# ChicyChen/LOCO-Edit

Measured on AMD Instinct MI355X. Metric: edit-directions/sec (top-5 PMP-Jacobian SVD @256^2) + vT cos-sim vs ref, higher is better.
Workload: dtype bf16x3 (split-bf16 MFMA operands, fp32 accumulate + fp32 storage); 1 GPU; CelebA-HQ DDPM 256x256 top-5 local basis (l_eye-sized mask, L=2400), t=0.6T, 12 power iterations, one GPU; multi_gpu_form=single, probes_total=5, probes_per_gpu=5, kept=5, n_iter=12, mask_L=2400, weights=synthetic seed 0, streams=2

## Files before the change

### include/loco_hip_diag.h

```cpp
#ifndef LOCO_HIP_DIAG_H
#define LOCO_HIP_DIAG_H
#include "loco_hip.h"
#ifdef __cplusplus
extern "C" {
#endif

int  loco_bench_conv(loco_ctx* ctx, int32_t cin, int32_t cout, int32_t H, int32_t W, int32_t B, int32_t mode,
                     int32_t taps, int32_t tile, int32_t iters, float* ms_avg, void* stream);

typedef struct loco_conv_desc {
    int32_t struct_size;
    int32_t Cin, Cout, Hin, Win, B, taps;
    int32_t stride, upsample, zins, mode, cpg;
    int32_t transposed, accumulate, in_arena, pad;
    int32_t Cin2, cot_cpg;
    float   res_scale;
    int32_t reserved;
    const float *weight, *bias;
    const float *in, *bias2, *res;
    const float *prim, *sc, *sh, *mr, *gamma, *tst, *tc;
    const float *in2, *w2, *bias2nd;
    const float *cot_d, *cot_prim, *cot_sc, *cot_sh, *cot_mr, *cot_tc;
    float* out;
} loco_conv_desc;
int  loco_debug_conv(loco_ctx* ctx, const loco_conv_desc* desc, char* plan, int64_t cap, void* stream);

int64_t loco_debug_tensor(loco_ctx* ctx, const char* name, float* dst, int64_t cap, void* stream);

#ifdef __cplusplus
}
#endif
#endif
```

### loco-edit_amd/csrc/conv_bf16.hip

```cpp
#include "kernels.h"
#include <cstdio>
#include <cstdlib>

namespace loco {

enum : int { PR_BF16X3 = 0, PR_F16 = 1 };
template <int PR, int TAPS, int MODE> void launch_tile_b(const ConvArgs& a, hipStream_t st);
template <int PR, int MODE> void launch_kcat_b(const ConvArgs& a, hipStream_t st);
template <int PR, int MODE> void launch_pair_b(const ConvArgs& a, hipStream_t st);
void launch_conv_gemm(const ConvArgs& a, hipStream_t st);

template <int PR>
static void launch_lowp(const ConvArgs& a, int taps, hipStream_t st) {
#ifdef LOCO_DIAG
    if (a.cot_d && (taps != 1 || a.gemm || a.nsplit > 1 || a.Cin2 > 0 || (a.Cout % conv_bf16_tile_couts(a)) != 0 || a.st_kind == ST_TAN || a.st_kind == ST_COT)) {
        fprintf(stderr, "loco: ConvArgs::cot_d on a launch whose epilogue has no norm-cotangent term (taps %d, gemm %d, nsplit %d, Cout %d, st_kind %d)\n",
                taps, a.gemm, a.nsplit, a.Cout, a.st_kind);
        abort();
    }
#endif
    if constexpr (PR == PR_BF16X3) {
        if (taps == 1 && a.gemm) { launch_conv_gemm(a, st); return; }
    }
    if (taps == 9 && a.Cin2 > 0) {
        if (a.mode == CM_GN_SILU) launch_kcat_b<PR, CM_GN_SILU>(a, st);
        else if (a.mode == CM_GN_GELU) launch_kcat_b<PR, CM_GN_GELU>(a, st);
        else launch_kcat_b<PR, CM_TAN_SILU>(a, st);
        return;
    }
    if constexpr (PR == PR_BF16X3) {
        if (taps == 9 && a.pair) {
            switch (a.mode) {
                case CM_NONE: launch_pair_b<PR, CM_NONE>(a, st); break;
                case CM_GN_SILU: launch_pair_b<PR, CM_GN_SILU>(a, st); break;
                case CM_TAN_SILU: launch_pair_b<PR, CM_TAN_SILU>(a, st); break;
                default: launch_pair_b<PR, CM_COT_SILU>(a, st); break;
            }
            return;
        }
    }
    if (taps == 9) {
        switch (a.mode) {
            case CM_NONE: launch_tile_b<PR, 9, CM_NONE>(a, st); break;
            case CM_GN_SILU: launch_tile_b<PR, 9, CM_GN_SILU>(a, st); break;
            case CM_GN_GELU: launch_tile_b<PR, 9, CM_GN_GELU>(a, st); break;
            case CM_TAN_SILU: launch_tile_b<PR, 9, CM_TAN_SILU>(a, st); break;
            case CM_COT_SILU: launch_tile_b<PR, 9, CM_COT_SILU>(a, st); break;
            default: launch_tile_b<PR, 9, CM_GN>(a, st); break;
        }
    } else {
        switch (a.mode) {
            case CM_NONE: launch_tile_b<PR, 1, CM_NONE>(a, st); break;
            default: launch_tile_b<PR, 1, CM_GN>(a, st); break;
        }
    }
}
void launch_conv_bf16x3(const ConvArgs& a, int taps, hipStream_t st) { launch_lowp<PR_BF16X3>(a, taps, st); }
void launch_conv_f16(const ConvArgs& a, int taps, hipStream_t st) { launch_lowp<PR_F16>(a, taps, st); }

}
```

### loco-edit_amd/csrc/conv_bf16_kernel.h

```cpp
#pragma once
#include "kernels.h"
#include <cstdlib>
#include <type_traits>

namespace loco {


typedef float f32x16 __attribute__((ext_vector_type(16)));
typedef float f32x4 __attribute__((ext_vector_type(4)));
typedef f32x4 f32x4_u __attribute__((aligned(4)));
typedef float f32x2 __attribute__((ext_vector_type(2)));
typedef f32x2 f32x2_u __attribute__((aligned(4)));
typedef __bf16 bf16x8 __attribute__((ext_vector_type(8)));
typedef _Float16 f16x8 __attribute__((ext_vector_type(8)));
typedef short s16x8 __attribute__((ext_vector_type(8)));

enum : int { PR_BF16X3 = 0, PR_F16 = 1 };

constexpr int BKC = 16;
constexpr bool LIVE_MASK = true;
constexpr bool EARLY_W = true;
constexpr int NDUMMY = 8;

__device__ __forceinline__ float sigmoidf2_(float y) { return __builtin_amdgcn_rcpf(1.0f + __expf(-y)); }
// ... 257 lines not shown
            const int gl = lane & (LW - 1);
            if (gl < (1 << STEPS)) {
                int base = 0;
#pragma unroll
                for (int sb = 0; sb < STEPS; ++sb) base += ((gl >> sb) & 1) * (NV >> (sb + 1));
                const int ntile = (a.Hout * a.Wout) / NT;
                float* const sp = a.st_part + (long)b * a.Cout * ntile * 2;
#pragma unroll
                for (int i = 0; i < LEFT; ++i) {
                    const int idx = base + i, hq = idx >> 1;
                    const int h = hq / NTASK, q = hq - h * NTASK;
                    const int row = (q * NTHR + tid) / NQ;
                    const int co = co0 + ((row >> 5) * TM + h) * 32 + (row & 31);
                    sp[((long)co * ntile + tile_id) * 2 + (idx & 1)] = av[i];
                }
            }
        }
    }
}
template <int WM, int WN, int TM, int TN>
__device__ __forceinline__ void conv_lowp_epilogue_direct(const ConvArgs& a, f32x16 (&acc)[TM][TN], const int co0, const int oy0,
                                                          const int ox0, const int TW, const int b, const int split) {
    const int lane = threadIdx.x & 63, wave = threadIdx.x >> 6;
    const int l31 = lane & 31, khalf = lane >> 5, wm = wave / WN, wn = wave % WN;
    const long out_plane = (long)a.Hout * a.Wout;
    const bool full_co = false;
#pragma unroll
    for (int j = 0; j < TN; ++j) {
        int p = (wn * TN + j) * 32 + l31;
        int ty = p / TW, tx = p - ty * TW;
        int oy = oy0 + ty, ox = ox0 + tx;
        const unsigned pix = (unsigned)(oy * a.Wout + ox);
#pragma unroll
        for (int i = 0; i < TM; ++i) {
            const int cob = co0 + (wm * TM + i) * 32 + 4 * khalf;
            if (a.nsplit > 1) {
                float* pb = a.partial + (((long)split * a.B + b) * a.Cout) * out_plane;
#pragma unroll
                for (int r = 0; r < 16; ++r) {
                    int co = cob + (r & 3) + 8 * (r >> 2);
                    if (full_co || co < a.Cout) pb[(long)co * out_plane + pix] = acc[i][j][r];
                }
            } else {
                float* ob = a.out + (long)b * a.out_bs;
                const float* rb = a.res ? a.res + (long)b * a.res_bs : nullptr;
                const float* b2 = a.bias2 ? a.bias2 + (long)b * a.bias2_bs : nullptr;
                if (rb || a.accumulate) {
                    float rv[16];
#pragma unroll
                    for (int r = 0; r < 16; ++r) {
                        int co = cob + (r & 3) + 8 * (r >> 2);
                        const bool ok = full_co || co < a.Cout;
                        const long off = (long)(ok ? co : a.Cout - 1) * out_plane + pix;
                        float t = 0.f;
                        if (rb) t = a.res_scale * rb[off];
                        if (a.accumulate) t += ob[off];
                        rv[r] = t;
                    }
#pragma unroll
                    for (int r = 0; r < 16; ++r) {
                        int co = cob + (r & 3) + 8 * (r >> 2);
                        if (!(full_co || co < a.Cout)) continue;
                        float v = acc[i][j][r] + rv[r];
                        if (a.bias) v += a.bias[co];
                        if (b2) v += b2[co];
                        __builtin_nontemporal_store(v, &ob[(long)co * out_plane + pix]);
                    }
                } else {
#pragma unroll
                    for (int r = 0; r < 16; ++r) {
                        int co = cob + (r & 3) + 8 * (r >> 2);
                        if (!(full_co || co < a.Cout)) continue;
                        float v = acc[i][j][r];
                        if (a.bias) v += a.bias[co];
                        if (b2) v += b2[co];
                        __builtin_nontemporal_store(v, &ob[(long)co * out_plane + pix]);
                    }
                }
            }
        }
    }
}

template <int PR, int TAPS, int WM, int WN, int TM, int TN, int MODE, int STG, int PHASE = 0>
__device__ __forceinline__ void conv_lowp_body(const ConvArgs& a, f32x16 (&acc)[TM][TN]) {
    constexpr int NTHR = WM * WN * 64;
    constexpr int HP = halo_pitch<PR>();
    constexpr int RB = rec_bytes<PR>();
    constexpr int NPC = RB / 16;
    constexpr int MT = WM * TM * 32;
    constexpr int NT = WN * TN * 32;
    constexpr int KS = (TAPS == 9) ? 3 : 1;
    constexpr int NTS = KS;
    constexpr int NROW = (TAPS == 9) ? 3 : 1;
    constexpr bool NEEDP = (MODE == CM_TAN_SILU || MODE == CM_COT_SILU);
    constexpr bool GEN = (STG == 1 || STG == 2);
    constexpr int NITEM = GEN ? (2 * max_halo(NT, TAPS, STG == 2) + NTHR - 1) / NTHR : 1;
    constexpr int WTOT = NTS * MT * NPC;
    constexpr int NWV = (WTOT + NTHR - 1) / NTHR;
    constexpr bool XPF = (TAPS == 9 && STG != 2);
    constexpr int NWB = XPF ? 3 : 2;
    constexpr bool DEEP1 = (TAPS == 1 && STG == 1 && !NEEDP);
    constexpr int DEEP_D = 4;

    extern __shared__ __attribute__((aligned(16))) unsigned char smem_b[];
#ifdef LOCO_DUAL_STAMP
#define LP_STAMP(i) do { if (threadIdx.x == 0 && PHASE == 0) reinterpret_cast<unsigned long long*>(a.partial)[blockIdx.x * 8 + (i)] = __builtin_amdgcn_s_memtime(); } while (0)
#else
#define LP_STAMP(i) do { } while (0)
#endif
    LP_STAMP(0);
    constexpr int WBYTES = NTS * MT * RB;
    unsigned char* const Wsb = smem_b;
    unsigned char* Hsb;
    unsigned char* Ws = smem_b;
    unsigned char* Hs = smem_b;

    const int tid = threadIdx.x;
    const int lane = tid & 63;
    const int wave = tid >> 6;
    const int l31 = lane & 31;
    const int khalf = lane >> 5;
    const int wm = wave / WN, wn = wave % WN;

    const int S = a.stride;
    const int TW = (TAPS == 1 && PHASE == 0 && a.stride == 1 && !a.upsample && !a.zins && (a.Wout & (a.Wout - 1)) == 0)
                       ? (a.Wout < NT ? a.Wout : NT) : (a.Wout < 32 ? a.Wout : 32);
    const int TH = NT / TW;
    const int tiles_x = a.Wout / TW;
    int tile_id, cot_id, zid;
    {
        const int ntile = (a.Hout * a.Wout) / NT, ncot = (a.Cout + MT - 1) / MT, Z = a.B * a.nsplit;
        const int NTC = ntile * ncot, L = blockIdx.x;
        int T = 0;
        if ((ntile & 7) == 0) {
            int q = L >> 3, q2, t8;
            idivmod_small(q, ncot, q2, cot_id);
            idivmod_small(q2, Z, t8, zid);
            tile_id = t8 * 8 + (L & 7);
        } else {
            if ((NTC & 7) == 0) { int q = L >> 3, t8; idivmod_small(q, Z, t8, zid); T = t8 * 8 + (L & 7); }
            else idivmod_small(L, Z, T, zid);
            idivmod_small(T, ntile, cot_id, tile_id);
        }
        tile_id = __builtin_amdgcn_readfirstlane(tile_id);
        cot_id = __builtin_amdgcn_readfirstlane(cot_id);
        zid = __builtin_amdgcn_readfirstlane(zid);
    }
    int ty0_, tx0_;
    idivmod_small(tile_id, tiles_x, ty0_, tx0_);
    const int oy0 = __builtin_amdgcn_readfirstlane(ty0_ * TH);
    const int ox0 = __builtin_amdgcn_readfirstlane(tx0_ * TW);
    const int co0 = cot_id * MT;
    int zb_, zs_;
    idivmod_small(zid, a.nsplit, zb_, zs_);
    const int b = __builtin_amdgcn_readfirstlane(zb_);
    const int split = __builtin_amdgcn_readfirstlane(zs_);

    if constexpr (XPF && PHASE != 2 && EARLY_W) {
        const int nchunks_ = (a.Cin + BKC - 1) / BKC;
        const int cps_ = __builtin_amdgcn_readfirstlane((nchunks_ + a.nsplit - 1) / a.nsplit);
        const int cbeg_ = split * cps_;
        const int cend_ = (cbeg_ + cps_ < nchunks_) ? cbeg_ + cps_ : nchunks_;
        if (cend_ > cbeg_) {
            typedef __attribute__((address_space(3))) unsigned char lds_u8_;
            typedef const __attribute__((address_space(1))) unsigned char glb_u8_;
            const int wpitch_ = (a.Cout + 31) & ~31;
            const unsigned char* wbase0 = reinterpret_cast<const unsigned char*>(a.wb) +
                                          (unsigned)(cbeg_ * TAPS) * ((unsigned)wpitch_ * (unsigned)RB);
#pragma unroll
            for (int st_ = 0; st_ < 2; ++st_)
#pragma unroll
                for (int i = 0; i < NWV; ++i) {
                    int e = tid + i * NTHR;
                    if (e >= WTOT) e = WTOT - 1;
                    const int tap = e / (MT * NPC), rem = e - tap * (MT * NPC);
                    int rec = co0 + rem / NPC;
                    if (rec >= wpitch_) rec = wpitch_ - 1;
                    const unsigned rel = (unsigned)(((st_ * NTS + tap) * wpitch_ + rec) * NPC + (rem % NPC)) * 16u;
                    const int e0 = wave * 64 + i * NTHR;
                    if ((WTOT % NTHR) == 0 || e0 < WTOT)
                        __builtin_amdgcn_global_load_lds((glb_u8_*)(wbase0 + rel), (lds_u8_*)(smem_b + st_ * WBYTES + e0 * 16), 16, 0, 0);
                }
        }
    }
    const int halo_w = (TW - 1) * S + KS;
    const int halo_h = (TH - 1) * S + KS;
    const int halo_sz = halo_h * halo_w;
    const int HBYTES = (halo_sz + NDUMMY) * HP;
    Hsb = smem_b + NWB * WBYTES;

    const int LH = (a.upsample || a.zins) ? a.Hin * 2 : a.Hin;
    const int LW = (a.upsample || a.zins) ? a.Win * 2 : a.Win;
    const long in_plane = (long)a.Hin * a.Win;

    int ipos[NITEM], ioct[NITEM];
    unsigned ivoff[NITEM];
    bool ival[NITEM];
#pragma unroll
    for (int i = 0; i < NITEM; ++i) {
        int it = tid + i * NTHR;
        int oct, pos;
        idivmod_small(it, halo_sz, oct, pos);
        int off = -1;
        if (it < 2 * halo_sz) {
            int hy, hx;
            idivmod_small(pos, halo_w, hy, hx);
            int Y = oy0 * S - a.pad + hy, X = ox0 * S - a.pad + hx;
            if (Y >= 0 && Y < LH && X >= 0 && X < LW) {
                if (a.upsample) off = (Y >> 1) * a.Win + (X >> 1);
                else if (a.zins) off = ((Y | X) & 1) ? -1 : (Y >> 1) * a.Win + (X >> 1);
                else off = Y * a.Win + X;
            }
        } else {
            pos = -1; oct = 0;
        }
        ipos[i] = pos; ioct[i] = oct;
        ival[i] = off >= 0;
        ivoff[i] = (unsigned)(oct * 8 * (int)in_plane + (off >= 0 ? off : 0));
    }

    const int nseg = (halo_w + 3) >> 2;
    int v_q4 = 0, v_pos0 = -1, v_voff = 0, v_cnt = 0;
    unsigned v_pm = 0;
    int v_rec[4] = {0, 0, 0, 0};
    unsigned v_goff = 0;
    if constexpr (!GEN) {
        const int per_q = halo_h * nseg;
        const int nsg4 = (nseg + 3) >> 2, nhy2 = (halo_h + 1) >> 1;
        bool have = false;
        int hy = 0, sg = 0;
        if (32 * nsg4 * nhy2 <= NTHR) {
            const int hi = tid >> 5;
            v_q4 = (tid >> 3) & 3;
            int hq_, hr_;
            idivmod_small(hi, nsg4, hq_, hr_);
            sg = hr_ * 4 + (tid & 3);
            hy = hq_ * 2 + ((tid >> 2) & 1);
            have = hi < nsg4 * nhy2 && sg < nseg && hy < halo_h;
            if (!have) v_q4 = 0;
        } else if (tid < 4 * per_q) {
            int rem;
            idivmod_small(tid, per_q, v_q4, rem);
            idivmod_small(rem, nseg, hy, sg);
            have = true;
        }
        if (have) {
            int Y = oy0 - a.pad + hy, X0 = ox0 - a.pad + 4 * sg;
            bool rowok = (Y >= 0 && Y < a.Hin);
            v_pos0 = hy * halo_w + 4 * sg;
            v_cnt = halo_w - 4 * sg < 4 ? halo_w - 4 * sg : 4;
            v_voff = rowok ? Y * a.Win + X0 : 0;
#pragma unroll
            for (int pxi = 0; pxi < 4; ++pxi)
                if (rowok && X0 + pxi >= 0 && X0 + pxi < a.Win && pxi < v_cnt) v_pm |= 1u << pxi;
        }
#pragma unroll
        for (int pxi = 0; pxi < 4; ++pxi)
            v_rec[pxi] = (v_pos0 >= 0 && pxi < v_cnt) ? v_pos0 + pxi : halo_sz + (tid & (NDUMMY - 1));
        v_goff = (unsigned)(((long)v_q4 * 4 * in_plane + v_voff + 16) * 4);
    }

    int hoff[TN];
#pragma unroll
    for (int j = 0; j < TN; ++j) {
        int p = (wn * TN + j) * 32 + l31;
        int ty, tx;
        idivmod_small(p, TW, ty, tx);
        hoff[j] = ty * S * halo_w + tx * S;
    }
    int hbyte[TN];
#pragma unroll
    for (int j = 0; j < TN; ++j) hbyte[j] = hrec_off<PR>(hoff[j], khalf);
    int aoff_hi[TM], aoff_lo[TM];
#pragma unroll
    for (int i = 0; i < TM; ++i) {
        int p = (wm * TM + i) * 32 + l31;
        aoff_hi[i] = rec_off<PR>(p, khalf);
        aoff_lo[i] = PR == PR_F16 ? 0 : rec_off<PR>(p, 2 + khalf);
    }

    if constexpr (PHASE != 2) {
#pragma unroll
        for (int i = 0; i < TM; ++i)
#pragma unroll
            for (int j = 0; j < TN; ++j)
#pragma unroll
                for (int r = 0; r < 16; ++r) acc[i][j][r] = 0.0f;
    }

    const int nchunks = (a.Cin + BKC - 1) / BKC;
    const int cps = __builtin_amdgcn_readfirstlane((nchunks + a.nsplit - 1) / a.nsplit);
    const int cbeg = split * cps;
    const int cend = (cbeg + cps < nchunks) ? cbeg + cps : nchunks;

    const float* inb = a.in + (long)b * a.in_bs;
    const float2* sxb = NEEDP ? a.sx : nullptr;
    const float* scb = (MODE == CM_GN_SILU || MODE == CM_GN || MODE == CM_GN_GELU) ? a.sc + (long)b * a.scsh_bs : nullptr;
    const float* shb = (MODE == CM_GN_SILU || MODE == CM_GN || MODE == CM_GN_GELU) ? a.sh + (long)b * a.scsh_bs : nullptr;
    const int wpitch = (a.Cout + 31) & ~31;
    const uint4* wg = reinterpret_cast<const uint4*>(a.wb);

    float hv[NITEM][8];
    float2 pv[NEEDP ? NITEM : 1][8];
    float cA[(MODE == CM_NONE) ? 1 : 16], cB[(MODE == CM_NONE) ? 1 : 16];
    const float* tcb = NEEDP ? a.tc + (long)b * a.tc_bs : nullptr;

    constexpr int NPART = (!GEN && NROW == 3) ? 2 : 1;
    constexpr int KP = 4 / NPART;
    struct HaloRegs {
        f32x4 dq[GEN ? 1 : KP];
        f32x4 sq[(!GEN && NEEDP) ? KP : 1][2];
        f32x4 cq[(!GEN && MODE != CM_NONE) ? (KP == 4 ? 2 : 1) : 1];
    };
    auto cq_a = [&](const HaloRegs& R, int kk) -> float {
        if constexpr (GEN || MODE == CM_NONE) return 0.f;
        else if constexpr (NEEDP) { if constexpr (KP == 4) return R.cq[kk >> 1][(kk & 1) * 2]; else return R.cq[0][kk * 2]; }
        else return R.cq[0][kk];
    };
    auto cq_b = [&](const HaloRegs& R, int kk) -> float {
        if constexpr (GEN || MODE == CM_NONE) return 0.f;
        else if constexpr (NEEDP) { if constexpr (KP == 4) return R.cq[kk >> 1][(kk & 1) * 2 + 1]; else return R.cq[0][kk * 2 + 1]; }
        else if constexpr (KP == 4) return R.cq[1][kk];
        else return R.cq[0][2 + kk];
    };
    HaloRegs hr;
    bool pf_live = true, dma_live = true;
#ifdef LOCO_DUAL_STAMP
    const bool wi_halo = (a.no_deep & 2) != 0, wi_dma = (a.no_deep & 4) != 0, wi_novalu = (a.no_deep & 8) != 0;
#endif
    auto prefetch_hv = [&](HaloRegs& R, int chunk, int part) {
        const unsigned cb = (unsigned)chunk * ((unsigned)(BKC * 4) * (unsigned)in_plane);
        const char* pk = reinterpret_cast<const char*>(inb - 16) + cb;
        const char* sk = reinterpret_cast<const char*>(reinterpret_cast<const float*>(sxb) - 32) + 2u * cb;
        const unsigned pl = (unsigned)in_plane * 4u;
#pragma unroll
        for (int kk = 0; kk < KP; ++kk) {
#ifdef LOCO_DUAL_STAMP
            const unsigned po = (pf_live && !wi_halo) ? v_goff + (unsigned)(part * KP + kk) * pl : 64u;
#else
            const unsigned po = pf_live ? v_goff + (unsigned)(part * KP + kk) * pl : 64u;
#endif
            R.dq[kk] = *reinterpret_cast<const f32x4_u*>(pk + po);
            if constexpr (NEEDP) {
                R.sq[kk][0] = *reinterpret_cast<const f32x4_u*>(sk + 2u * po);
                R.sq[kk][1] = *reinterpret_cast<const f32x4_u*>(sk + 2u * po + 16);
            }
        }
        const int c0 = chunk * BKC + v_q4 * 4 + part * KP;
        if constexpr (MODE != CM_NONE) {
            if constexpr (NEEDP) {
                R.cq[0] = *reinterpret_cast<const f32x4_u*>(tcb + 2 * c0);
                if constexpr (KP == 4) R.cq[1] = *reinterpret_cast<const f32x4_u*>(tcb + 2 * c0 + 4);
            } else if constexpr (KP == 4) {
                R.cq[0] = *reinterpret_cast<const f32x4_u*>(scb + c0);
                R.cq[1] = *reinterpret_cast<const f32x4_u*>(shb + c0);
            } else {
                const f32x2 sa = *reinterpret_cast<const f32x2_u*>(scb + c0), sb = *reinterpret_cast<const f32x2_u*>(shb + c0);
                R.cq[0] = f32x4{sa[0], sa[1], sb[0], sb[1]};
            }
        }
    };
    auto stage_hv = [&](const HaloRegs& R, int part) {
#ifdef LOCO_DUAL_STAMP
        if (wi_novalu) return;
#endif
        const int oct = v_q4 >> 1, half = v_q4 & 1;
#pragma unroll
        for (int pxi = 0; pxi < 4; ++pxi) {
            float r[KP];
#pragma unroll
            for (int kk = 0; kk < KP; ++kk) {
                float d = R.dq[kk][pxi];
                float v = d;
                if constexpr (MODE == CM_GN_SILU) {
                    float y = fmaf(cq_a(R, kk), d, cq_b(R, kk));
                    v = y * sigmoidf2_(y);
                } else if constexpr (MODE == CM_GN_GELU) {
                    v = act_fwd(fmaf(cq_a(R, kk), d, cq_b(R, kk)), ACT_GELU);
                } else if constexpr (MODE == CM_GN) {
                    v = fmaf(cq_a(R, kk), d, cq_b(R, kk));
                } else if constexpr (NEEDP) {
                    const float Sv = R.sq[kk][pxi >> 1][(pxi & 1) * 2], xh = R.sq[kk][pxi >> 1][(pxi & 1) * 2 + 1];
                    if constexpr (MODE == CM_TAN_SILU) v = Sv * fmaf(-xh, cq_b(R, kk), d - cq_a(R, kk));
                    else v = fmaf(-xh, cq_b(R, kk), fmaf(Sv, d, -cq_a(R, kk)));
                }
                r[kk] = ((v_pm >> pxi) & 1u) ? v : 0.0f;
            }
            unsigned char* dst = Hs + hrec_off<PR>(v_rec[pxi], oct) + half * 8 + part * (KP * 2);
            if constexpr (KP == 4) {
                uint2 h, l;
                cvt2<PR>(r[0], r[1], h.x, l.x);
                cvt2<PR>(r[2], r[3], h.y, l.y);
                *reinterpret_cast<uint2*>(dst) = h;
                if constexpr (PR == PR_BF16X3) *reinterpret_cast<uint2*>(dst + 32) = l;
            } else {
                unsigned h, l;
                cvt2<PR>(r[0], r[1], h, l);
                *reinterpret_cast<unsigned*>(dst) = h;
                if constexpr (PR == PR_BF16X3) *reinterpret_cast<unsigned*>(dst + 32) = l;
            }
        }
    };
    auto load_consts = [&](int chunk) {
        const int c0 = chunk * BKC;
        if constexpr (MODE != CM_NONE) {
#pragma unroll
            for (int kk = 0; kk < 16; ++kk) {
                int c = c0 + kk < a.Cin ? c0 + kk : a.Cin - 1;
                if constexpr (NEEDP) { cA[kk] = tcb[2 * c]; cB[kk] = tcb[2 * c + 1]; }
                else { cA[kk] = scb[c]; cB[kk] = shb[c]; }
            }
        }
    };
    auto load_regs = [&](float (&hvd)[NITEM][8], int chunk) {
        const int c0 = chunk * BKC;
        if (c0 + BKC <= a.Cin) {
            if constexpr (TAPS == 9 && !NEEDP) {
                const unsigned lm = pf_live ? 0xffffffffu : 0u;
                const long pb4 = in_plane * 4;
                const unsigned char* pk = reinterpret_cast<const unsigned char*>(inb) + (long)c0 * pb4;
#pragma unroll
                for (int k = 0; k < 8; ++k) {
#pragma unroll
                    for (int i = 0; i < NITEM; ++i) hvd[i][k] = *reinterpret_cast<const float*>(pk + ((ivoff[i] * 4u) & lm));
                    pk += pb4;
                }
            } else {
#pragma unroll
            for (int k = 0; k < 8; ++k) {
                const float* pk = inb + (long)(c0 + k) * in_plane;
                const float2* sk = NEEDP ? sxb + (long)(c0 + k) * in_plane : nullptr;
#pragma unroll
                for (int i = 0; i < NITEM; ++i) {
                    hvd[i][k] = pk[pf_live ? ivoff[i] : 0u];
                    if constexpr (NEEDP) pv[i][k] = sk[pf_live ? ivoff[i] : 0u];
                }
            }
            }
        } else {
#pragma unroll
            for (int i = 0; i < NITEM; ++i) {
#pragma unroll
                for (int k = 0; k < 8; ++k) {
                    int c = c0 + ioct[i] * 8 + k;
                    int cc = c < a.Cin ? c : a.Cin - 1;
                    unsigned vo = ivoff[i] - (unsigned)(ioct[i] * 8 * (int)in_plane);
                    float v = inb[(long)cc * in_plane + vo];
                    hvd[i][k] = c < a.Cin ? v : 0.0f;
                    if constexpr (NEEDP) {
                        float2 pp = sxb[(long)cc * in_plane + vo];
                        pv[i][k] = c < a.Cin ? pp : make_float2(0.f, 0.f);
                    }
                }
            }
        }
    };
    auto prefetch_h = [&](int chunk, int part) {
        if constexpr (!GEN) { prefetch_hv(hr, chunk, part); return; }
        load_consts(chunk);
        load_regs(hv, chunk);
    };
    unsigned wrel[NWV];
#pragma unroll
    for (int i = 0; i < NWV; ++i) {
        int e = tid + i * NTHR;
        if (e >= WTOT) e = WTOT - 1;
        int tap = e / (MT * NPC), rem = e - tap * (MT * NPC);
        int rec = co0 + rem / NPC;
        if (rec >= wpitch) rec = wpitch - 1;
        wrel[i] = (unsigned)((tap * wpitch + rec) * NPC + (rem % NPC)) * 16u;
    }
    typedef __attribute__((address_space(3))) unsigned char lds_u8;
    typedef const __attribute__((address_space(1))) unsigned char glb_u8;
    auto dma_w = [&](int chunk, int row, unsigned char* Wdst) {
        const unsigned char* wbase = reinterpret_cast<const unsigned char*>(wg) +
                                     (unsigned)(chunk * TAPS + row * NTS) * ((unsigned)wpitch * (unsigned)RB);
#pragma unroll
        for (int i = 0; i < NWV; ++i) {
            const int e0 = (wave * 64 + i * NTHR);
            if ((WTOT % NTHR) == 0 || e0 < WTOT)
#ifdef LOCO_DUAL_STAMP
                __builtin_amdgcn_global_load_lds((glb_u8*)(wbase + ((dma_live && !wi_dma) ? wrel[i] : 0u)), (lds_u8*)(Wdst + e0 * 16), 16, 0, 0);
#else
                __builtin_amdgcn_global_load_lds((glb_u8*)(wbase + (dma_live ? wrel[i] : 0u)), (lds_u8*)(Wdst + e0 * 16), 16, 0, 0);
#endif
        }
    };
    auto stage_regs = [&](const float (&hvs)[NITEM][8], int chunk, unsigned char* Hd, auto whole_tag) {
        constexpr bool WHOLE = decltype(whole_tag)::value;
        const int c0 = chunk * BKC;
#pragma unroll
        for (int i = 0; i < NITEM; ++i) {
            if (ipos[i] < 0) continue;
            float v[8];
#pragma unroll
            for (int k = 0; k < 8; ++k) {
                int c = c0 + ioct[i] * 8 + k;
                float r = 0.0f;
                if (ival[i] && (WHOLE || c < a.Cin)) {
                    float d = hvs[i][k];
                    if constexpr (MODE == CM_NONE) {
                        r = d;
                    } else {
                        const float ca = ioct[i] ? cA[8 + k] : cA[k];
                        const float cb = ioct[i] ? cB[8 + k] : cB[k];
                        if constexpr (MODE == CM_GN_SILU) {
                            float y = fmaf(ca, d, cb);
                            r = y * sigmoidf2_(y);
                        } else if constexpr (MODE == CM_GN_GELU) {
                            r = act_fwd(fmaf(ca, d, cb), ACT_GELU);
                        } else if constexpr (MODE == CM_GN) {
                            r = fmaf(ca, d, cb);
                        } else {
                            float Sv = pv[i][k].x, xh = pv[i][k].y;
                            if constexpr (MODE == CM_TAN_SILU) r = Sv * fmaf(-xh, cb, d - ca);
                            else r = fmaf(-xh, cb, fmaf(Sv, d, -ca));
                        }
                    }
                }
                v[k] = r;
            }
            uint4 hi, lo;
            split8<PR>(v, hi, lo);
            *reinterpret_cast<uint4*>(Hd + hrec_off<PR>(ipos[i], ioct[i])) = hi;
            if constexpr (PR == PR_BF16X3) *reinterpret_cast<uint4*>(Hd + hrec_off<PR>(ipos[i], 2 + ioct[i])) = lo;
        }
    };
    auto stage_h = [&](int chunk, int part) {
        if constexpr (!GEN) { stage_hv(hr, part); return; }
        stage_regs(hv, chunk, Hs, std::false_type{});
    };

    constexpr int NLO = PR == PR_BF16X3 ? 1 : 0;
    struct Frag { s16x8 ah[TM], al[NLO ? TM : 1], bh[TN], bl[NLO ? TN : 1]; };
    auto load_frag = [&](Frag& f, int row, int tp) {
        const int tapoff = (TAPS == 9) ? row * halo_w + tp : 0;
#pragma unroll
        for (int i = 0; i < TM; ++i) {
            f.ah[i] = *reinterpret_cast<const s16x8*>(Ws + tp * MT * RB + aoff_hi[i]);
#if defined(LOCO_WI_NOLO)
            if constexpr (NLO) f.al[i] = f.ah[i];
#else
            if constexpr (NLO) f.al[i] = *reinterpret_cast<const s16x8*>(Ws + tp * MT * RB + aoff_lo[i]);
#endif
        }
#pragma unroll
        for (int j = 0; j < TN; ++j) {
            const unsigned char* hp = Hs + tapoff * HP + hbyte[j];
            f.bh[j] = *reinterpret_cast<const s16x8*>(hp);
#if defined(LOCO_WI_NOLO)
            if constexpr (NLO) f.bl[j] = f.bh[j];
#else
            if constexpr (NLO) f.bl[j] = *reinterpret_cast<const s16x8*>(hp + 32);
#endif
        }
    };
    auto mma_frag = [&](const Frag& f) {
#pragma unroll
        for (int i = 0; i < TM; ++i)
#pragma unroll
            for (int j = 0; j < TN; ++j) {
                if constexpr (PR == PR_F16) {
                    acc[i][j] = __builtin_amdgcn_mfma_f32_32x32x16_f16(__builtin_bit_cast(f16x8, f.ah[i]),
                                                                       __builtin_bit_cast(f16x8, f.bh[j]), acc[i][j], 0, 0, 0);
                } else {
                    const bf16x8 ah = __builtin_bit_cast(bf16x8, f.ah[i]), al = __builtin_bit_cast(bf16x8, f.al[i]);
                    const bf16x8 bh = __builtin_bit_cast(bf16x8, f.bh[j]), bl = __builtin_bit_cast(bf16x8, f.bl[j]);
                    acc[i][j] = __builtin_amdgcn_mfma_f32_32x32x16_bf16(al, bh, acc[i][j], 0, 0, 0);
                    acc[i][j] = __builtin_amdgcn_mfma_f32_32x32x16_bf16(ah, bl, acc[i][j], 0, 0, 0);
                    acc[i][j] = __builtin_amdgcn_mfma_f32_32x32x16_bf16(ah, bh, acc[i][j], 0, 0, 0);
                }
            }
    };

    auto mma_one = [&](const Frag& f, int i, int j) {
        if constexpr (PR == PR_F16) {
            acc[i][j] = __builtin_amdgcn_mfma_f32_32x32x16_f16(__builtin_bit_cast(f16x8, f.ah[i]),
                                                               __builtin_bit_cast(f16x8, f.bh[j]), acc[i][j], 0, 0, 0);
        } else {
            const bf16x8 ah = __builtin_bit_cast(bf16x8, f.ah[i]), al = __builtin_bit_cast(bf16x8, f.al[i]);
            const bf16x8 bh = __builtin_bit_cast(bf16x8, f.bh[j]), bl = __builtin_bit_cast(bf16x8, f.bl[j]);
#if defined(LOCO_WI_MFMA16)
            {
                f32x4 q0 = {acc[i][j][0], acc[i][j][1], acc[i][j][2], acc[i][j][3]}, q1 = {acc[i][j][4], acc[i][j][5], acc[i][j][6], acc[i][j][7]};
                f32x4 q2 = {acc[i][j][8], acc[i][j][9], acc[i][j][10], acc[i][j][11]}, q3 = {acc[i][j][12], acc[i][j][13], acc[i][j][14], acc[i][j][15]};
                q0 = __builtin_amdgcn_mfma_f32_16x16x32_bf16(al, bh, q0, 0, 0, 0);
                q1 = __builtin_amdgcn_mfma_f32_16x16x32_bf16(al, bh, q1, 0, 0, 0);
                q2 = __builtin_amdgcn_mfma_f32_16x16x32_bf16(ah, bl, q2, 0, 0, 0);
                q3 = __builtin_amdgcn_mfma_f32_16x16x32_bf16(ah, bl, q3, 0, 0, 0);
                q0 = __builtin_amdgcn_mfma_f32_16x16x32_bf16(ah, bh, q0, 0, 0, 0);
                q1 = __builtin_amdgcn_mfma_f32_16x16x32_bf16(ah, bh, q1, 0, 0, 0);
#pragma unroll
                for (int r = 0; r < 4; ++r) { acc[i][j][r] = q0[r]; acc[i][j][4 + r] = q1[r]; acc[i][j][8 + r] = q2[r]; acc[i][j][12 + r] = q3[r]; }
                return;
            }
#elif defined(LOCO_WI_2MFMA)
            acc[i][j] = __builtin_amdgcn_mfma_f32_32x32x16_bf16(ah, bl, acc[i][j], 0, 0, 0);
            acc[i][j] = __builtin_amdgcn_mfma_f32_32x32x16_bf16(ah, bh, acc[i][j], 0, 0, 0);
            (void)al;
            return;
#endif
            acc[i][j] = __builtin_amdgcn_mfma_f32_32x32x16_bf16(al, bh, acc[i][j], 0, 0, 0);
            acc[i][j] = __builtin_amdgcn_mfma_f32_32x32x16_bf16(ah, bl, acc[i][j], 0, 0, 0);
            acc[i][j] = __builtin_amdgcn_mfma_f32_32x32x16_bf16(ah, bh, acc[i][j], 0, 0, 0);
        }
    };
    auto mma_frag_head = [&](const Frag& f) { mma_one(f, 0, 0); };
    auto mma_frag_tail = [&](const Frag& f) {
#pragma unroll
        for (int i = 0; i < TM; ++i)
#pragma unroll
            for (int j = 0; j < TN; ++j)
                if (i + j > 0) mma_one(f, i, j);
    };

    const int nch = cend - cbeg;
    const int clast = cend - 1;
    auto cclamp = [&](int c) { return __builtin_amdgcn_readfirstlane(c < clast ? c : clast); };
    auto vres = [&](int x) -> int {
// ... 120 lines not shown
            const bool live = LIVE_MASK ? (chunk_raw <= clast) : true;
            const int chunk = cclamp(chunk_raw);
            const int c0 = chunk * BKC;
            const unsigned lm = live ? 0xffffffffu : 0u;
            const unsigned char* pk = reinterpret_cast<const unsigned char*>(inb) + (long)c0 * plane_bytes;
#pragma unroll
            for (int k = 0; k < 8; ++k) {
#pragma unroll
                for (int i = 0; i < NITEM; ++i) hvr[sl][i][k] = *reinterpret_cast<const float*>(pk + (ivoffb[i] & lm));
                pk += plane_bytes;
            }
            const unsigned char* wbase = wgb + (unsigned)(chunk * TAPS) * ((unsigned)wpitch * (unsigned)RB);
#pragma unroll
            for (int i = 0; i < NWV; ++i) wr[sl][i] = *reinterpret_cast<const f32x4*>(wbase + (wrel[i] & lm));
        };
        auto commit = [&](auto stag, int chunk, unsigned char* Hd, unsigned char* Wd) {
            constexpr int sl = decltype(stag)::value;
            if constexpr (MODE != CM_NONE) load_consts(chunk);
            stage_regs(hvr[sl], chunk, Hd, std::true_type{});
#pragma unroll
            for (int i = 0; i < NWV; ++i)
                if ((WTOT % NTHR) == 0 || tid + i * NTHR < WTOT)
                    *reinterpret_cast<f32x4*>(Wd + (tid + i * NTHR) * 16) = wr[sl][i];
        };
        using S0 = std::integral_constant<int, 0>; using S1 = std::integral_constant<int, 1>;
        using S2 = std::integral_constant<int, 2>; using S3 = std::integral_constant<int, 3>;
        static_assert(D == 4, "ring slots are spelled out below");
        if (nch > 0) {
            issue(S0{}, cbeg);
            issue(S1{}, cbeg + 1);
            issue(S2{}, cbeg + 2);
            issue(S3{}, cbeg + 3);
            commit(S0{}, cbeg, Hsb, Wsb);
            issue(S0{}, cbeg + 4);
            stage_end();
        }
        auto body = [&](auto stag, const int ci) {
            const int chunk = cbeg + ci;
            unsigned char* const Wcur = Wsb + (ci & 1) * WBYTES;
            unsigned char* const Wnxt = Wsb + ((ci + 1) & 1) * WBYTES;
            unsigned char* const Hcur = Hsb + (ci & 1) * HBYTES;
            unsigned char* const Hnxt = Hsb + ((ci + 1) & 1) * HBYTES;
            Ws = Wcur; Hs = Hcur;
            Frag f0;
            load_frag(f0, 0, 0);
            __builtin_amdgcn_sched_barrier(0);
            mma_frag(f0);
            commit(stag, cclamp(chunk + 1), Hnxt, Wnxt);
            issue(stag, chunk + 1 + D);
            stage_end();
        };
        int ci = 0;
        for (; ci + D <= nch; ci += D) {
            body(S1{}, ci); body(S2{}, ci + 1); body(S3{}, ci + 2); body(S0{}, ci + 3);
        }
        if (ci < nch) body(S1{}, ci);
        if (ci + 1 < nch) body(S2{}, ci + 1);
        if (ci + 2 < nch) body(S3{}, ci + 2);
      }
    }
    if (!deep_done) {
    if (nch > 0) {
        dma_w(cbeg, 0, Wsb);
        Hs = Hsb;
        if constexpr (!GEN && NPART == 2) {
            HaloRegs hr2;
            prefetch_hv(hr, cbeg, 0);
            prefetch_hv(hr2, cbeg, 1);
            stage_hv(hr, 0);
            stage_hv(hr2, 1);
        } else {
#pragma unroll
            for (int part = 0; part < NPART; ++part) {
                prefetch_h(cbeg, part);
                stage_h(cbeg, part);
            }
        }
        asm volatile("s_waitcnt vmcnt(0)" ::: "memory");
        if (NROW == 1 || NPART == 2) prefetch_h(cclamp(cbeg + 1), 0);
        stage_end();
    }
    for (int ci = 0; ci < nch; ++ci) {
        const int chunk = cbeg + ci;
#pragma unroll
        for (int row = 0; row < NROW; ++row) {
            const int s_ = ci * NROW + row;
            unsigned char* const Wcur = Wsb + (s_ & 1) * WBYTES;
            unsigned char* const Wnxt = Wsb + ((s_ + 1) & 1) * WBYTES;
            unsigned char* const Hcur = Hsb + (ci & 1) * HBYTES;
            unsigned char* const Hnxt = Hsb + ((ci + 1) & 1) * HBYTES;
            constexpr bool one = (NROW == 1);
            const int st_part = one ? 0 : (NPART == 2 ? (row == 0 ? 0 : row == 1 ? 1 : -1) : (row == 2 ? 0 : -1));
            const int ld_part = one ? 0 : (NPART == 2 ? (row == 0 ? 1 : row == 1 ? 0 : -1) : (row == 0 ? 0 : -1));
            const int ld_chunk = one ? chunk + 2 : ((NPART == 2 && row == 1) ? chunk + 2 : chunk + 1);
            constexpr bool MIDLOAD = !GEN;
            constexpr int NLD = KP + (NEEDP ? 2 * KP + 1 : (MODE != CM_NONE ? 2 : 0));
            {
                const int r1 = (row + 1) % NROW, dc = (row + 1) / NROW;
                dma_live = LIVE_MASK ? (chunk + dc <= clast) : true;
                dma_w(cclamp(chunk + dc), r1, Wnxt);
                dma_live = true;
            }
            Ws = Wcur; Hs = Hcur;
            Frag f0, f1;
            load_frag(f0, row, 0);
            if (NTS > 1) load_frag(f1, row, 1);
            __builtin_amdgcn_sched_barrier(0);
            mma_frag(f0);
            __builtin_amdgcn_sched_barrier(0);
            if (NTS > 2) load_frag(f0, row, 2);
            __builtin_amdgcn_sched_barrier(0);
            if (NTS > 1) mma_frag(f1);
            if (st_part >= 0) { Hs = Hnxt; stage_h(cclamp(chunk + 1), st_part); Hs = Hcur; }
            if (MIDLOAD && ld_part >= 0) { pf_live = LIVE_MASK ? (ld_chunk <= clast) : true; prefetch_h(cclamp(ld_chunk), ld_part); pf_live = true; }
            if (NTS > 2) mma_frag(f0);
            __builtin_amdgcn_sched_barrier(0);
            if (MIDLOAD && ld_part >= 0) {
                asm volatile("s_waitcnt vmcnt(%0)" :: "n"(NLD) : "memory");
            } else {
                asm volatile("s_waitcnt vmcnt(0)" ::: "memory");
                if (!MIDLOAD && ld_part >= 0) { pf_live = LIVE_MASK ? (ld_chunk <= clast) : true; prefetch_h(cclamp(ld_chunk), ld_part); pf_live = true; }
            }
            stage_end();
        }
    }
    }

    }

    if constexpr (PHASE == 1) {
        asm volatile("s_waitcnt lgkmcnt(0)" ::: "memory");
        __builtin_amdgcn_s_barrier();
        return;
    }
    LP_STAMP(3);
    conv_lowp_epilogue<WM, WN, TM, TN, (TAPS == 1 && PHASE == 0) ? (EPI_COT1 | EPI_STATS) : EPI_STATS>(a, acc, smem_b, co0, oy0, ox0, TW, tile_id, b, split);
    LP_STAMP(4);
#undef LP_STAMP
}

constexpr int lowp_min_waves(int taps, int nthr) { return (taps == 1 && nthr <= 256) ? 2 : 1; }
template <int TAPS, int WM, int WN, int TM, int TN, int MODE, int STG>
__global__ __launch_bounds__(WM * WN * 64, lowp_min_waves(TAPS, WM * WN * 64)) void conv_mfma_bf16x3(ConvArgs a) {
    f32x16 acc[TM][TN];
    conv_lowp_body<PR_BF16X3, TAPS, WM, WN, TM, TN, MODE, STG>(a, acc);
}
template <int TAPS, int WM, int WN, int TM, int TN, int MODE, int STG>
__global__ __launch_bounds__(WM * WN * 64, lowp_min_waves(TAPS, WM * WN * 64)) void conv_mfma_f16(ConvArgs a) {
    f32x16 acc[TM][TN];
    conv_lowp_body<PR_F16, TAPS, WM, WN, TM, TN, MODE, STG>(a, acc);
}

template <int PR, int WM, int WN, int TM, int TN, int MODE>
__device__ __forceinline__ void conv_lowp_kcat(const ConvArgs& a) {
    f32x16 acc[TM][TN];
    conv_lowp_body<PR, 9, WM, WN, TM, TN, MODE, 0, 1>(a, acc);
    ConvArgs a2 = a;
    a2.in = a.in2; a2.in_bs = a.in2_bs; a2.Cin = a.Cin2; a2.wb = a.wb2; a2.mode = CM_NONE; a2.pad = 0; a2.in_padded = a.in2_padded;
    conv_lowp_body<PR, 1, WM, WN, TM, TN, CM_NONE, 1, 2>(a2, acc);
}
template <int WM, int WN, int TM, int TN, int MODE>
__global__ __launch_bounds__(WM * WN * 64) void conv_kcat_bf16x3(ConvArgs a) { conv_lowp_kcat<PR_BF16X3, WM, WN, TM, TN, MODE>(a); }
template <int WM, int WN, int TM, int TN, int MODE>
__global__ __launch_bounds__(WM * WN * 64) void conv_kcat_f16(ConvArgs a) { conv_lowp_kcat<PR_F16, WM, WN, TM, TN, MODE>(a); }

template <int PR, int TAPS, int WM, int WN, int TM, int TN, int MODE, int STG>
static void launch_one_b2(const ConvArgs& a, hipStream_t st) {
    constexpr int MT = WM * TM * 32, NT = WN * TN * 32;
    constexpr int KS = (TAPS == 9) ? 3 : 1;
    int TW = a.Wout < 32 ? a.Wout : 32;
    int TH = NT / TW;
    int halo_w = (TW - 1) * a.stride + KS, halo_h = (TH - 1) * a.stride + KS;
    const int nwb = (TAPS == 9 && STG != 2) ? 3 : 2;
    size_t lds = (size_t)nwb * KS * MT * rec_bytes<PR>() + 2 * ((size_t)halo_w * halo_h + NDUMMY) * halo_pitch<PR>();
    const size_t stage_bytes = (size_t)WM * 32 * NT * 4;
    if (lds < stage_bytes) lds = stage_bytes;
    dim3 grid(((a.Hout * a.Wout) / NT) * ((a.Cout + MT - 1) / MT) * a.B * a.nsplit);
    void (*kern)(ConvArgs);
    if constexpr (PR == PR_F16) kern = &conv_mfma_f16<TAPS, WM, WN, TM, TN, MODE, STG>;
    else kern = &conv_mfma_bf16x3<TAPS, WM, WN, TM, TN, MODE, STG>;
    if (lds > 64 * 1024) {
        static DeviceOnce once;
        if (first_on_device(once)) {
            (void)hipFuncSetAttribute(reinterpret_cast<const void*>(kern), hipFuncAttributeMaxDynamicSharedMemorySize,
                                      160 * 1024);
        }
    }
    hipLaunchKernelGGL(kern, grid, dim3(WM * WN * 64), lds, st, a);
}

template <int PR, int TAPS, int WM, int WN, int TM, int TN, int MODE>
static void launch_one_b(const ConvArgs& a, hipStream_t st) {
    const bool general = a.stride != 1 || a.upsample || a.zins || (a.Cin % BKC) != 0 || !a.in_padded;
    if constexpr (MODE == CM_NONE) {
        if (a.stride == 2) launch_one_b2<PR, TAPS, WM, WN, TM, TN, MODE, 2>(a, st);
        else if (TAPS == 9 && !general) launch_one_b2<PR, TAPS, WM, WN, TM, TN, MODE, 0>(a, st);
        else launch_one_b2<PR, TAPS, WM, WN, TM, TN, MODE, 1>(a, st);
        return;
    }
    if constexpr (MODE == CM_GN_SILU || MODE == CM_TAN_SILU || MODE == CM_GN_GELU) {
        if (general) { launch_one_b2<PR, TAPS, WM, WN, TM, TN, MODE, 1>(a, st); return; }
    }
    launch_one_b2<PR, TAPS, WM, WN, TM, TN, MODE, 0>(a, st);
}


template <int PR, int MODE>
void launch_kcat_b(const ConvArgs& a, hipStream_t st) {
    constexpr int WM = 2, WN = 4, TM = 2, TN = 2, MT = 128, NT = 256;
    const int TW = a.Wout < 32 ? a.Wout : 32, TH = NT / TW;
    size_t lds = (size_t)3 * 3 * MT * rec_bytes<PR>() + 2 * ((size_t)(TW + 2) * (TH + 2) + NDUMMY) * halo_pitch<PR>();
    dim3 grid(((a.Hout * a.Wout) / NT) * ((a.Cout + MT - 1) / MT) * a.B * a.nsplit);
    void (*kern)(ConvArgs);
    if constexpr (PR == PR_F16) kern = &conv_kcat_f16<WM, WN, TM, TN, MODE>;
    else kern = &conv_kcat_bf16x3<WM, WN, TM, TN, MODE>;
    static DeviceOnce once;
    if (first_on_device(once))
        (void)hipFuncSetAttribute(reinterpret_cast<const void*>(kern), hipFuncAttributeMaxDynamicSharedMemorySize, 160 * 1024);
    hipLaunchKernelGGL(kern, grid, dim3(WM * WN * 64), lds, st, a);
}

template <int PR, int TAPS, int MODE>
void launch_tile_b(const ConvArgs& a, hipStream_t st) {
    switch (a.tile) {
        case 5:
            launch_one_b<PR, TAPS, 2, 4, 2, 2, MODE>(a, st);
            break;
        case 0: launch_one_b<PR, TAPS, 2, 2, 2, 2, MODE>(a, st); break;
        case 1: launch_one_b<PR, TAPS, 4, 1, 1, 2, MODE>(a, st); break;
        case 2: launch_one_b<PR, TAPS, 1, 4, 1, 1, MODE>(a, st); break;
        default: launch_one_b<PR, TAPS, 2, 2, 1, 1, MODE>(a, st); break;
    }
}


}
```

### loco-edit_amd/csrc/conv_plan.hip

```cpp
#include "kernels.h"
#include <cstdio>
#include <cstdlib>

namespace loco {

constexpr int BKC = 16;
constexpr int BKF = 8;

static const int kMT[6] = {128, 128, 32, 64, 128, 128}, kNT[6] = {128, 64, 128, 64, 256, 256};

static int env_int(const char* name, int dflt) {
    const char* e = getenv(name);
    return e ? atoi(e) : dflt;
}
static int pick_tile(int Cout, int HW) {
    if (HW >= 128) return Cout > 32 ? 0 : 2;
    return Cout > 64 ? 1 : 3;
}

static int conv_pick_nsplit(int Cin, int Cout, int Hout, int Wout, int B) {
    const int t = pick_tile(Cout, Hout * Wout);
    long blocks = (long)((Hout * Wout) / kNT[t]) * ((Cout + kMT[t] - 1) / kMT[t]) * B;
    int nchunks = (Cin + BKF - 1) / BKF;
    if (blocks >= 384 || nchunks < 8) return 1;
    int want = (int)((512 + blocks - 1) / blocks);
    int maxs = nchunks / 4;
    if (want > maxs) want = maxs;
    if (want > 32) want = 32;
    return want < 1 ? 1 : want;
}

static int conv_bf16_pick_tile(int Cout, int HW, int B, int tile_override) {
    if (B <= 1 && HW <= 1024 && HW >= 64 && (Cout % 64) == 0) return 3;
    int t = pick_tile(Cout, HW);
    if (t == 0 && HW >= 256) {
        if (tile_override >= 0) return tile_override;
        return 5;
    }
    return t;
}

constexpr int kTile0MaxHW = 65536;

static int bf16_tile_of(const ConvArgs& a, int tile_override = -1) {
    int tile = conv_bf16_pick_tile(a.Cout, a.Hout * a.Wout, a.B, tile_override);
    if (tile == 4) tile = 5;
    if (tile == 5 && a.taps == 1 && !a.gemm && a.B >= 2 && a.Hout * a.Wout <= kTile0MaxHW) return 0;
    if (a.stride == 2 && tile == 5) tile = 0;
    return tile;
}
static int tile_for(const ConvArgs& a, int prec, int tile_override) {
    return prec ? bf16_tile_of(a, tile_override) : pick_tile(a.Cout, a.Hout * a.Wout);
}
static int conv_bf16_tile_pixels(const ConvArgs& a) { return a.gemm ? 256 : kNT[a.tile]; }
int conv_bf16_tile_couts(const ConvArgs& a) { return a.gemm ? 64 * a.gemm_tm : kMT[a.tile]; }

static int conv_bf16_pick_nsplit(int Cin, int Cout, int Hout, int Wout, int B, int chip_share, int taps, int lanes) {
    const int HW = Hout * Wout;
    int t = conv_bf16_pick_tile(Cout, HW, B, -1);
    if (t == 4) t = 5;
    if (taps == 1 && t == 5 && B >= 2 && HW <= kTile0MaxHW) t = 0;
    long blocks = (long)(HW / kNT[t]) * ((Cout + kMT[t] - 1) / kMT[t]) * B;
    int nchunks = (Cin + BKC - 1) / BKC;
    int target = chip_share > 1 ? 256 / chip_share : (lanes == 2 ? 240 : 256);
    if (target < 32) target = 32;
    if (blocks >= target / 2 || nchunks < 8) return 1;
    int want = (int)(target / blocks);
    int maxs = nchunks / 4;
    if (want > maxs) want = maxs;
    if (want > 32) want = 32;
    return want < 1 ? 1 : want;
}

static bool conv_lowp_can_kcat(const ConvArgs& a) {
    static const bool on = env_int("LOCO_KCAT", 1) != 0;
    return on && a.Cin2 > 0 && a.nsplit == 1 && bf16_tile_of(a) == 5 && a.stride == 1 && !a.upsample && !a.zins && a.pad == 1 &&
           (a.Cin % BKC) == 0 && (a.Cin2 % BKC) == 0 && a.in_padded &&
           (a.mode == CM_GN_SILU || a.mode == CM_GN_GELU || a.mode == CM_TAN_SILU);
}
static bool conv_lowp_can_fuse_stats(const ConvArgs& a) {
    return a.nsplit <= 1 && !a.gemm && (a.Cout % conv_bf16_tile_couts(a)) == 0;
}

static bool conv_pair_ok(const ConvArgs& a) {
    static const bool on = env_int("LOCO_CONV_PAIR", 1) != 0;
    if (!on || a.Hout * a.Wout < 16384 || a.taps != 9 || a.Cin2 > 0 || a.nsplit != 1 || a.stride != 1 || a.upsample || a.zins ||
        a.pad != 1 || !a.in_padded || (a.Cin % (2 * BKC)) != 0 || (a.Cout % 128) != 0 || (a.Wout % 32) != 0 || (a.Hout % 8) != 0)
        return false;
    if (!(a.mode == CM_NONE || a.mode == CM_GN_SILU || a.mode == CM_TAN_SILU || a.mode == CM_COT_SILU)) return false;
    return a.tile == 5;
}

static ConvArgs conv_shift_batch(const ConvArgs& a, int nb) {
    ConvArgs t = a;
    t.B = a.B - nb;
    t.in += (long)nb * a.in_bs; t.out += (long)nb * a.out_bs;
    if (t.prim) t.prim += (long)nb * a.prim_bs;
    if (t.bias2) t.bias2 += (long)nb * a.bias2_bs;
    if (t.res) t.res += (long)nb * a.res_bs;
    if (t.sc) { t.sc += (long)nb * a.scsh_bs; t.sh += (long)nb * a.scsh_bs; }
    if (t.mr) t.mr += (long)nb * a.mr_bs;
    if (t.tst) t.tst += (long)nb * a.tst_bs;
    if (t.tc) t.tc += (long)nb * a.tc_bs;
    if (t.in2) t.in2 += (long)nb * a.in2_bs;
    if (t.cot_d) { t.cot_d += (long)nb * a.cot_d_bs; t.cot_tc += (long)nb * a.cot_tc_bs; }
    if (t.st_part) t.st_part += (long)nb * a.Cout * ((a.Hout * a.Wout) / conv_bf16_tile_pixels(a)) * 2;
    return t;
}

static void conv_gemm_plan(ConvArgs& a) {
    static const bool on = env_int("LOCO_CONV_GEMM", 1) != 0;
    a.gemm = 0;
    const long HW = (long)a.Hout * a.Wout;
    if (!on || a.stride != 1 || a.upsample || a.zins || (a.Cin % BKC) != 0 || a.Cin < 320 || (HW % 256) != 0 || (a.Wout % 16) != 0 ||
        a.Cout < 128 || !a.partial || a.Cin2 > 0 || !(a.mode == CM_NONE || a.mode == CM_GN) || a.cot_d)
        return;
    {
        const int TW = a.Wout < 32 ? a.Wout : 32;
        if ((256 % TW) != 0 || (a.Wout % TW) != 0 || (a.Hout % (256 / TW)) != 0) return;
    }
    static const int all_shapes = env_int("LOCO_GEMM_ALL", 0);
    if (!all_shapes && !(a.Cout >= 640 && (a.Cout >= 4 * a.Cin || a.Cin >= 2560))) return;
    const int pad256 = (a.Cout + 255) / 256 * 256;
    const int tm = (pad256 * 10 <= a.Cout * 11) ? 4 : 2;
    const int mt = 64 * tm;
    const long tiles = (HW / 256) * ((a.Cout + mt - 1) / mt) * a.B;
    const size_t rec_floats = (size_t)a.B * a.Cin * HW;
    int ns = 1;
    if (tiles < 192) {
        const int nchunks = a.Cin / BKC;
        ns = (int)((256 + tiles - 1) / tiles);
        if (ns > 8) ns = 8;
        while (ns > 1 && nchunks / ns < 8) --ns;
        while (ns > 1 && (size_t)ns * a.B * a.Cout * HW + rec_floats > a.partial_floats) --ns;
    }
    if ((ns > 1 ? (size_t)ns * a.B * a.Cout * HW : 0) + rec_floats > a.partial_floats) return;
    a.gemm = 1; a.gemm_tm = tm; a.nsplit = ns;
}

void conv_plan_family(ConvArgs& a, int prec) {
    if (prec == 1 && a.taps == 1) conv_gemm_plan(a);
}

void conv_plan_tile_pair(ConvArgs& a, int prec, int tile_override) {
    a.tile = tile_for(a, prec, tile_override);
    a.pair = prec == 1 && conv_pair_ok(a);
}

static bool short_tail(long per_probe, int B) {
    const long total = per_probe * B, r = total % 256;
    return total > 256 && r > 0 && r <= 160;
}

static int tail_split(const ConvArgs& a, size_t partial_floats, int* split) {
    const long per_probe = (long)((a.Hout * a.Wout) / conv_bf16_tile_pixels(a)) * ((a.Cout + 127) / 128);
    const long r = per_probe * a.B % 256;
    if (!short_tail(per_probe, a.B) || per_probe <= 0 || r % per_probe != 0 || r / per_probe >= a.B) return 0;
    int s = (int)(256 / r);
    if (s > 4) s = 4;
    const int nchunks = (a.Cin + 15) / 16;
    while (s > 1 && nchunks / s < 4) --s;
    const size_t one = (size_t)(r / per_probe) * a.Cout * a.Hout * a.Wout;
    while (s > 1 && (size_t)s * one > partial_floats) --s;
    *split = s;
    return s > 1 ? (int)(r / per_probe) : 0;
}

static int stats_route(const ConvEnv& e, const StatAsk* q, bool want, ConvArgs& x, int s0, int B, int* keep_ntile) {
    if (!q || q->kind == ST_NONE) return SR_NONE;
    const int alone = q->norm ? SR_ALONE : SR_NONE;
    if (!want) return alone;
    if (x.nsplit > 1) return !q->norm ? SR_NONE : ((x.Hout * x.Wout) % 4 == 0 ? SR_SPLITK : SR_ALONE);
    const int ntile = (x.Hout * x.Wout) / conv_bf16_tile_pixels(x);
    const size_t need = (size_t)x.B * x.Cout * ntile * 2;
    const int epi = q->norm ? SR_EPI : SR_KEEP;
    const bool kept = q->keep && s0 == 0 && x.B == B && need <= q->keep_floats;
    if (q->kind == ST_FWD && conv_lowp_can_fuse_stats(x) && (kept || (q->norm && need <= e.stpart_floats))) {
        x.st_part = kept ? q->keep : e.stpart; x.st_kind = ST_FWD;
        if (kept) *keep_ntile = ntile;
        return epi;
    }
    const bool cot_cache = q->kind == ST_COT && q->norm && q->sx;
    if ((q->kind == ST_TAN || cot_cache) && e.fuse_lin && !x.cot_d && conv_lowp_can_fuse_stats(x)) {
        const size_t lane_off = (size_t)e.lane_s0 * (q->keep_floats / e.max_batch);
        const bool keptl = q->kind == ST_TAN && q->keep && s0 == 0 && x.B == B && lane_off + need <= q->keep_floats;
        if (keptl || (q->norm && need <= e.stpart_floats)) {
            x.st_part = keptl ? q->keep + lane_off : e.stpart; x.st_kind = q->kind; x.st_x = q->prim;
            if (q->kind == ST_COT) x.st_sx = q->sx;
            if (keptl) *keep_ntile = ntile;
            return epi;
        }
    }
    return alone;
}

static ConvLaunch plan_launch(const ConvEnv& e, const StatAsk* q, bool want, const ConvArgs& x, int s0, int B, int* keep_ntile) {
    ConvLaunch l;
    l.args = x;
    l.s0 = s0;
    l.args.tile = tile_for(x, e.prec, -1);
    l.stats = stats_route(e, q, want, l.args, s0, B, keep_ntile);
    if (l.stats == SR_EPI || l.stats == SR_KEEP) l.ntile = (x.Hout * x.Wout) / conv_bf16_tile_pixels(l.args);
    conv_plan_tile_pair(l.args, e.prec, -1);
    return l;
}

ConvPlan plan_conv(const ConvEnv& e, const ConvArgs& a0, int taps, const StatAsk* q, const ConvArgs* sc) {
    ConvPlan p;
    ConvArgs a = a0;
    a.taps = taps;
    a.gemm = 0;
    if (sc) {
        ConvArgs t = a;
        t.nsplit = e.prec >= 1 ? conv_bf16_pick_nsplit(a.Cin, a.Cout, a.Hout, a.Wout, a.B, e.chip_share, 9, e.lanes) : 2;
        t.in2 = sc->in; t.in2_bs = sc->in_bs; t.Cin2 = sc->Cin;
        const long per_probe = (long)((a.Hout * a.Wout) / 256) * ((a.Cout + 127) / 128);
        if (e.prec >= 1 && taps == 9 && !short_tail(per_probe, a.B) && !a.bias2 && conv_lowp_can_kcat(t)) {
            a.in2 = sc->in; a.in2_bs = sc->in_bs; a.Cin2 = sc->Cin; a.in2_padded = sc->in_padded;
            a.wb2 = e.prec == 2 ? sc->wh : sc->wb;
            a.bias2 = sc->bias; a.bias2_bs = 0;
            a.res = nullptr;
        } else {
            p.sc_first = true;
            a.res = sc->out; a.res_bs = sc->out_bs;
        }
    }
    if (e.prec == 2) a.wb = a.wh;
    a.no_deep = e.deep1 ? 0 : 1;
    a.nsplit = e.prec >= 1 ? conv_bf16_pick_nsplit(a.Cin, a.Cout, a.Hout, a.Wout, a.B, e.chip_share, taps, e.lanes)
                           : conv_pick_nsplit(a.Cin, a.Cout, a.Hout, a.Wout, a.B);
    if (a.cot_d) {
        ConvArgs t = a;
        t.tile = bf16_tile_of(t);
        const long per_probe = (long)((a.Hout * a.Wout) / conv_bf16_tile_pixels(t)) * ((a.Cout + 127) / 128);
        p.cot = e.prec >= 1 && taps == 1 && a.nsplit == 1 && !short_tail(per_probe, a.B) && conv_lowp_can_fuse_stats(t);
        if (!p.cot) { a.cot_d = nullptr; a.cot_d_bs = 0; a.cot_sx = nullptr; a.cot_tc = nullptr; a.cot_tc_bs = 0; }
    }
    while (a.nsplit > 1 && (size_t)a.nsplit * a.B * a.Cout * a.Hout * a.Wout > e.partial_floats) a.nsplit >>= 1;
    if (a.nsplit < 1) a.nsplit = 1;
    a.partial = e.partial;
    a.partial_floats = e.partial_floats;
    conv_plan_family(a, e.prec);
    a.tile = tile_for(a, e.prec, -1);
    int split = 1;
    const int tail = e.prec >= 1 && a.nsplit == 1 && a.B >= 2 && !a.gemm ? tail_split(a, e.partial_floats, &split) : 0;
    const bool want = q && q->kind != ST_NONE && e.prec >= 1 && e.fuse_stats;
    if (!tail) {
        p.l[0] = plan_launch(e, q, want, a, 0, a.B, &p.keep_ntile);
        return p;
    }
    const bool per_part = want && q->norm && (q->kind == ST_FWD || (e.fuse_lin && (a.Hout * a.Wout) % 4 == 0));
    p.stats_all = !per_part && q && q->kind != ST_NONE && q->norm;
    const StatAsk* ql = per_part ? q : nullptr;
    const int nb = a.B - tail;
    ConvArgs m = a, t = conv_shift_batch(a, nb);
    m.B = nb;
    t.nsplit = split;
    p.nl = 2;
    p.l[0] = plan_launch(e, ql, want, m, 0, a.B, &p.keep_ntile);
    p.l[1] = plan_launch(e, ql, want, t, nb, a.B, &p.keep_ntile);
    return p;
}

const char* conv_variant_name(const ConvArgs& a, int taps, int prec) {
    static const char* tiles[6] = {"2,2,2,2", "4,1,1,2", "1,4,1,1", "2,2,1,1", "2,2,2,4", "2,4,2,2"};
    static char names[3][2][6][6][56];
    static char others[3][3][6][40];
    const int mode = (a.mode < 0 || a.mode > 5) ? 2 : a.mode;
    const char* other = nullptr;
    int k = 0, v = mode;
    if (prec && taps == 9 && a.Cin2 > 0) other = prec == 1 ? "conv_kcat_bf16x3<2,4,2,2,%d>" : "conv_kcat_f16<2,4,2,2,%d>";
    else if (prec == 1 && taps == 1 && a.gemm) { k = 1; other = "conv_gemm_bf16x3<%d>"; v = a.gemm_tm; }
    else if (prec == 1 && taps == 9 && a.pair) { k = 2; other = "conv_pair_bf16x3<%d>"; }
    if (other) {
        char* n = others[k][prec][v];
        if (!n[0]) snprintf(n, 40, other, v);
        return n;
    }
    int t = a.tile;
    if (t < 0 || t > 5) t = 0;
    int m = mode;
    if (taps != 9 && m != CM_NONE) m = CM_GN;
    if (!prec && m == CM_GN_GELU) m = CM_GN_SILU;
    char* n = names[prec][taps == 9 ? 0 : 1][t][m];
    static const char* kn[3] = {"conv_mfma_f32", "conv_mfma_bf16x3", "conv_mfma_f16"};
    if (!n[0]) snprintf(n, 56, "%s<%d,%s,%d>", kn[prec], taps, tiles[t], m);
    return n;
}

}
```

### loco-edit_amd/csrc/engine.hip

```cpp
#include <hip/hip_runtime.h>

#include <algorithm>
#include <array>
#include <cmath>
#include <cstdio>
#include <cstdlib>
#include <cstring>
#include <map>
#include <memory>
#include <thread>
#include <atomic>
#include <string>
#include <vector>

#include "../../include/loco_hip.h"
#ifdef LOCO_DIAG
#include "../../include/loco_hip_diag.h"
#endif
#include "kernels.h"
#include "program.h"
#ifdef LOCO_DIAG
#include "conv_plan_text.h"
#endif

using namespace loco;


#define HIPCHK(ctx, call)                                                                    \
    do {                                                                                     \
        hipError_t e_ = (call);                                                              \
        if (e_ != hipSuccess) {                                                              \
            (ctx)->err = std::string(#call) + ": " + hipGetErrorString(e_);                  \
            return -1;                                                                       \
        }                                                                                    \
    } while (0)

namespace {

struct ConvP {
    float* wf = nullptr;
    float* wd = nullptr;
    float* wbf = nullptr;
    float* wbd = nullptr;
    float* whf = nullptr;
    float* whd = nullptr;
    float* bias = nullptr;
    int cin = 0, cout = 0, taps = 0;
};
struct NormW { float* gamma = nullptr; float* beta = nullptr; };

struct OpWeights {
    ConvP c1, c2, nin, qkvc, proj, conv;
    ConvP xqc, xproj;
    ConvP pj_in, to_out1, to_out2, ff1, ff2, pj_out;
    NormW g1, g2, gx;
    float *xkw = nullptr, *xkb = nullptr, *xvw = nullptr, *xvb = nullptr;
    float *xng = nullptr, *xnb = nullptr;
    float *lng[3] = {nullptr, nullptr, nullptr}, *lnb[3] = {nullptr, nullptr, nullptr};
    long tproj_off = 0;
};
struct Weights {
    std::vector<OpWeights> op;
    float *freq = nullptr, *td0w = nullptr, *td0b = nullptr, *td1w = nullptr, *td1b = nullptr;
    float* tcw = nullptr;
    float *tp_w = nullptr, *tp_b = nullptr;
    long tproj_total = 0;
    double flops = 0.0;
};

struct Tens : TensPlan {
    float* keep = nullptr; size_t keep_floats = 0; int keep_ntile = 0;
};
struct NormP : NormPlan, NormW {
    bool ready = false;
};
struct Op : OpPlan, OpWeights {
    NormP n1, n2, nx;
    float *xK = nullptr, *xV = nullptr;
};

struct HostParam { std::vector<float> data; std::vector<int64_t> shape; bool loaded = false; };

}


struct loco_ctx {
    loco_unet_cfg cfg;
    std::string err;
    std::map<std::string, HostParam> params;
    bool finalized = false;

    std::shared_ptr<const Program> prog;
    std::shared_ptr<Weights> wts;
    std::vector<Tens> tens;
    std::vector<Op> ops;


    float *arenaP = nullptr, *arenaT = nullptr;
    float *statsP = nullptr, *statsT = nullptr;
    double* red = nullptr;
    bool fuse_cot = true;
    float *stpart = nullptr, *stpart2 = nullptr;
    size_t stpart_floats = 0;
    bool fuse_stats = true;
    bool fuse_xattn = true;
    bool deep1 = true;
    bool flash_attn = true;
    float* attn_delta = nullptr;
    float* partial = nullptr;
    size_t partial_floats = 0;
    const float* bench_out = nullptr; int64_t bench_out_count = 0;
#ifdef LOCO_DIAG
    std::string* plan_log = nullptr;
#endif
    float *tact = nullptr, *tproj = nullptr;
    float* eps_buf = nullptr;
    float* gx0 = nullptr;
    float* ge = nullptr;
    float* tmpA = nullptr;
    double *G = nullptr, *Q = nullptr, *W = nullptr, *gscratch = nullptr;
    float* alphas = nullptr;
    float* ctx_colbias = nullptr;
    bool has_ctx = false;
    float* cond_add = nullptr;
    float* ctx_norm = nullptr;
    bool has_cond = false;
    float* cond_in = nullptr;
    bool has_tcond = false;
// ... 58 lines not shown
    *p = reinterpret_cast<T*>(q);
    c->owned.push_back(reinterpret_cast<float*>(q));
    c->bytes += count * sizeof(T);
    return 0;
}

inline float eps_of(const loco_ctx* c, const NormP& n) { return n.eps > 0.f ? n.eps : c->cfg.gn_eps; }


int upload(loco_ctx* c, float** dst, const std::vector<float>& h) {
    if (dalloc(c, dst, h.size() ? h.size() : 1)) return -1;
    HIPCHK(c, hipMemcpy(*dst, h.data(), h.size() * sizeof(float), hipMemcpyHostToDevice));
    return 0;
}

static inline uint16_t f2bf(float f) {
    uint32_t u; std::memcpy(&u, &f, 4);
    u += 0x7FFFu + ((u >> 16) & 1u);
    return (uint16_t)(u >> 16);
}
static inline float bf2f(uint16_t h) {
    uint32_t u = (uint32_t)h << 16; float f; std::memcpy(&f, &u, 4); return f;
}
template <typename F>
static void parallel_for(int n, size_t work, F fn) {
    unsigned nt = std::thread::hardware_concurrency();
    if (nt > 16) nt = 16;
    if ((int)nt > n) nt = (unsigned)n;
    if (nt <= 1 || work < ((size_t)1 << 18)) { for (int i = 0; i < n; ++i) fn(i); return; }
    std::atomic<int> next{0};
    std::vector<std::thread> th;
    for (unsigned t = 0; t < nt; ++t)
        th.emplace_back([&]() { int i; while ((i = next.fetch_add(1)) < n) fn(i); });
    for (auto& t : th) t.join();
}

template <typename F>
static std::vector<float> build_records(int nin, int nout, int taps, F get) {
    int nch = (nin + 15) / 16, noutP = (nout + 31) & ~31;
    std::vector<uint16_t> rec((size_t)nch * taps * noutP * 32, 0);
    parallel_for(nch, (size_t)nin * nout * taps, [&](int ck) {
        for (int t = 0; t < taps; ++t)
            for (int o = 0; o < nout; ++o) {
                uint16_t* r = rec.data() + (((size_t)ck * taps + t) * noutP + o) * 32;
                int sw = (o >> 2) & 3;
                for (int k = 0; k < 16; ++k) {
                    int i = ck * 16 + k;
                    float v = (i < nin) ? get(o, i, t) : 0.f;
                    uint16_t h = f2bf(v);
                    uint16_t l = f2bf(v - bf2f(h));
                    int qh = (k >> 3) ^ sw, ql = (2 + (k >> 3)) ^ sw;
                    r[qh * 8 + (k & 7)] = h;
                    r[ql * 8 + (k & 7)] = l;
                }
            }
    });
    std::vector<float> out(rec.size() / 2);
    std::memcpy(out.data(), rec.data(), rec.size() * 2);
    return out;
}

template <typename F>
static std::vector<float> build_records_f16(int nin, int nout, int taps, F get) {
    int nch = (nin + 15) / 16, noutP = (nout + 31) & ~31;
    std::vector<_Float16> rec((size_t)nch * taps * noutP * 16, (_Float16)0.f);
    parallel_for(nch, (size_t)nin * nout * taps, [&](int ck) {
        for (int t = 0; t < taps; ++t)
            for (int o = 0; o < nout; ++o) {
                _Float16* r = rec.data() + (((size_t)ck * taps + t) * noutP + o) * 16;
                int sw = (o >> 3) & 1;
                for (int k = 0; k < 16; ++k) {
                    int i = ck * 16 + k;
                    float v = (i < nin) ? get(o, i, t) : 0.f;
                    r[((k >> 3) ^ sw) * 8 + (k & 7)] = (_Float16)v;
                }
            }
    });
    std::vector<float> out(rec.size() / 2);
    std::memcpy(out.data(), rec.data(), rec.size() * 2);
    return out;
}

int make_conv(loco_ctx* c, const std::vector<const HostParam*>& ws, const std::vector<const HostParam*>& bs,
              ConvP* out, int row_limit = -1) {
    int cin = (int)ws[0]->shape[1], k = ws[0]->shape.size() > 2 ? (int)ws[0]->shape[2] : 1;
    int taps = ws[0]->shape.size() == 4 ? k * k : k;
    int cout = 0;
    for (auto* w : ws) cout += (int)w->shape[0];
    if (row_limit > 0 && ws.size() == 1 && row_limit < cout) cout = row_limit;
    int coutP = (cout + 31) & ~31, cinP = (cin + 31) & ~31;
    std::vector<float> wf((size_t)cin * taps * coutP, 0.f), wd((size_t)cout * taps * cinP, 0.f), bias(cout);
    int co0 = 0;
    for (size_t wi = 0; wi < ws.size(); ++wi) {
        const HostParam* w = ws[wi];
        int co_n = (int)w->shape[0];
        if (co_n > cout - co0) co_n = cout - co0;
        parallel_for(co_n, (size_t)co_n * cin * taps, [&](int co) {
            for (int ci = 0; ci < cin; ++ci)
                for (int t = 0; t < taps; ++t)
                    wd[((size_t)(co0 + co) * taps + (taps - 1 - t)) * cinP + ci] = w->data[((size_t)co * cin + ci) * taps + t];
        });
        parallel_for(cin, (size_t)co_n * cin * taps, [&](int ci) {
            for (int t = 0; t < taps; ++t)
                for (int co = 0; co < co_n; ++co)
                    wf[((size_t)ci * taps + t) * coutP + co0 + co] = w->data[((size_t)co * cin + ci) * taps + t];
        });
        for (int co = 0; co < co_n; ++co) bias[co0 + co] = bs[wi]->data[co];
        co0 += co_n;
    }
    out->cin = cin; out->cout = cout; out->taps = taps;
    if (upload(c, &out->wf, wf) || upload(c, &out->wd, wd) || upload(c, &out->bias, bias)) return -1;
    auto fwd = [&](int o, int i, int t) { return wf[((size_t)i * taps + t) * coutP + o]; };
    auto dgr = [&](int o, int i, int t) { return wd[((size_t)i * taps + t) * cinP + o]; };
    std::vector<float> rf = build_records(cin, cout, taps, fwd);
    std::vector<float> rd = build_records(cout, cin, taps, dgr);
    if (upload(c, &out->wbf, rf) || upload(c, &out->wbd, rd)) return -1;
    std::vector<float> hf = build_records_f16(cin, cout, taps, fwd);
    std::vector<float> hd = build_records_f16(cout, cin, taps, dgr);
    if (upload(c, &out->whf, hf) || upload(c, &out->whd, hd)) return -1;
    return 0;
}
int make_conv1(loco_ctx* c, const std::string& name, ConvP* out, int row_limit = -1) {
    return make_conv(c, {&c->params[name + ".weight"]}, {&c->params[name + ".bias"]}, out, row_limit);
}
int make_conv1_scaled(loco_ctx* c, const std::string& name, ConvP* out, float s) {
    if (s == 1.f) return make_conv1(c, name, out);
    HostParam w = c->params[name + ".weight"], b = c->params[name + ".bias"];
    for (float& v : w.data) v *= s;
    for (float& v : b.data) v *= s;
    return make_conv(c, {&w}, {&b}, out);
}
int make_norm(loco_ctx* c, const std::string& name, NormW* n) {
    if (upload(c, &n->gamma, c->params[name + ".weight"].data)) return -1;
    if (upload(c, &n->beta, c->params[name + ".bias"].data)) return -1;
    return 0;
}

int bind_weights(loco_ctx* c) {
    const Weights& W = *c->wts;
    for (size_t i = 0; i < c->ops.size(); ++i) {
        Op& v = c->ops[i];
        static_cast<OpWeights&>(v) = W.op[i];
        static_cast<NormW&>(v.n1) = v.g1; static_cast<NormW&>(v.n2) = v.g2; static_cast<NormW&>(v.nx) = v.gx;
    }
    if (dalloc(c, &c->tact, (size_t)c->cfg.ch * 4) || dalloc(c, &c->tproj, (size_t)(W.tproj_total > 0 ? W.tproj_total : 1))) return -1;
    c->finalized = true;
    return 0;
}

int finalize_params(loco_ctx* c) {
    if (c->finalized) return 0;
    for (const ParamDecl& d : c->prog->params)
        if (!c->params[d.name].loaded) { c->err = "parameter not loaded: " + d.name; return -1; }
    Weights& W = *c->wts;
    const loco_unet_cfg& cfg = c->cfg;
    int temb_ch = cfg.ch * 4;
    const bool adm = cfg.arch == 1;
    const std::string te0 = adm ? "time_embed.0" : "temb.dense.0", te1 = adm ? "time_embed.2" : "temb.dense.1";
    if (cfg.arch < 2) {
        if (upload(c, &W.td0w, c->params[te0 + ".weight"].data)) return -1;
        if (upload(c, &W.td0b, c->params[te0 + ".bias"].data)) return -1;
        if (upload(c, &W.td1w, c->params[te1 + ".weight"].data)) return -1;
        if (upload(c, &W.td1b, c->params[te1 + ".bias"].data)) return -1;
        if (cfg.time_cond_proj_dim > 0 && upload(c, &W.tcw, c->params["time_embed.cond_proj.weight"].data)) return -1;
    }
    {
        int half = cfg.ch / 2;
        std::vector<float> f(half);
        for (int i = 0; i < half; ++i) {
            float x;
            if (adm) x = ((float)(-std::log(10000.0)) * (float)i) / (float)half;
            else x = (float)i * (float)(-(std::log(10000.0) / (double)(half - 1)));
            f[i] = (float)std::exp((double)x);
        }
        if (upload(c, &W.freq, f)) return -1;
    }
    std::vector<float> tpw, tpb;
    for (size_t oi = 0; oi < W.op.size(); ++oi) {
        const OpPlan& op = c->prog->ops[oi];
        OpWeights& ow = W.op[oi];
        switch (op.kind) {
            case OP_CONV_IN: case OP_CONV: if (make_conv1(c, op.pn_conv, &ow.conv)) return -1; break;
            case OP_RES: {
                if (make_norm(c, op.pn_n1, &ow.g1) || make_norm(c, op.pn_n2, &ow.g2)) return -1;
                if (make_conv1(c, op.pn_c1, &ow.c1) || make_conv1_scaled(c, op.pn_c2, &ow.c2, c->prog->res_scale)) return -1;
                if (op.has_nin && make_conv1_scaled(c, op.pn_skip, &ow.nin, c->prog->res_scale)) return -1;
                if (!op.has_temb) break;
                ow.tproj_off = (long)tpb.size();
                auto& w = c->params[op.pn_emb + ".weight"].data;
                auto& b = c->params[op.pn_emb + ".bias"].data;
                tpw.insert(tpw.end(), w.begin(), w.end());
                tpb.insert(tpb.end(), b.begin(), b.end());
                break;
            }
            case OP_ATTN: {
                if (make_norm(c, op.pn_n1, &ow.g1)) return -1;
                if (adm) {
                    if (make_conv1(c, op.pn_qkv, &ow.qkvc)) return -1;
                } else if (make_conv(c, {&c->params[op.name + ".q.weight"], &c->params[op.name + ".k.weight"],
                                         &c->params[op.name + ".v.weight"]},
                                     {&c->params[op.name + ".q.bias"], &c->params[op.name + ".k.bias"],
                                      &c->params[op.name + ".v.bias"]}, &ow.qkvc)) return -1;
                if (make_conv1(c, op.pn_proj, &ow.proj)) return -1;
                if (op.added_kv) {
                    const int C = c->tens[op.in].C, NH = op.heads, CH = C / NH, D = c->cfg.context_dim;
                    const HostParam& w = c->params[op.name + ".encoder_kv.weight"];
                    const HostParam& b = c->params[op.name + ".encoder_kv.bias"];
                    std::vector<float> kw((size_t)C * D), vw((size_t)C * D), kb(C), vb(C);
                    for (int h = 0; h < NH; ++h)
                        for (int i = 0; i < CH; ++i) {
                            const size_t rk = (size_t)h * 2 * CH + i, rv = rk + CH, r = (size_t)h * CH + i;
                            std::copy(w.data.begin() + rk * D, w.data.begin() + (rk + 1) * D, kw.begin() + r * D);
                            std::copy(w.data.begin() + rv * D, w.data.begin() + (rv + 1) * D, vw.begin() + r * D);
                            kb[r] = b.data[rk]; vb[r] = b.data[rv];
                        }
                    if (upload(c, &ow.xkw, kw) || upload(c, &ow.xkb, kb) || upload(c, &ow.xvw, vw) || upload(c, &ow.xvb, vb) ||
                        upload(c, &ow.xng, c->params[op.name + ".norm_encoder.weight"].data) ||
                        upload(c, &ow.xnb, c->params[op.name + ".norm_encoder.bias"].data)) return -1;
                }
                if (op.has_x) {
                    const std::string x = op.name + ".xattn";
                    if (make_norm(c, x + ".norm", &ow.gx) || make_conv1(c, x + ".q", &ow.xqc) ||
                        make_conv1(c, x + ".proj_out", &ow.xproj)) return -1;
                    if (upload(c, &ow.xkw, c->params[x + ".k.weight"].data) || upload(c, &ow.xkb, c->params[x + ".k.bias"].data) ||
                        upload(c, &ow.xvw, c->params[x + ".v.weight"].data) || upload(c, &ow.xvb, c->params[x + ".v.bias"].data))
                        return -1;
                }
                break;
            }
            case OP_DOWN: case OP_UP: if (make_conv1(c, op.pn_conv, &ow.conv)) return -1; break;
            case OP_XFMR: {
                const int C = c->tens[op.in].C, NH = op.heads, CH = C / NH;
                const std::string b = op.name + ".transformer_blocks.0";
                HostParam zb; zb.shape = {8 * C}; zb.data.assign((size_t)8 * C, 0.f);
                auto nobias = [&](const std::string& w, ConvP* out) { return make_conv(c, {&c->params[w + ".weight"]}, {&zb}, out); };
                if (make_norm(c, op.pn_n1, &ow.g1) || make_conv1(c, op.name + ".proj_in", &ow.pj_in) ||
                    make_conv1(c, op.name + ".proj_out", &ow.pj_out)) return -1;
                const char* lnn[3] = {".norm1", ".norm2", ".norm3"};
                for (int i = 0; i < 3; ++i)
                    if (upload(c, &ow.lng[i], c->params[b + lnn[i] + ".weight"].data) ||
                        upload(c, &ow.lnb[i], c->params[b + lnn[i] + ".bias"].data)) return -1;
                {
                    HostParam w; w.shape = {3 * C, C}; w.data.resize((size_t)3 * C * C);
                    const char* nm[3] = {".attn1.to_q.weight", ".attn1.to_k.weight", ".attn1.to_v.weight"};
                    for (int which = 0; which < 3; ++which) {
                        const std::vector<float>& src = c->params[b + nm[which]].data;
                        for (int h = 0; h < NH; ++h)
                            for (int j = 0; j < CH; ++j)
                                std::memcpy(&w.data[((size_t)(h * 3 + which) * CH + j) * C], &src[(size_t)(h * CH + j) * C], (size_t)C * 4);
                    }
                    if (make_conv(c, {&w}, {&zb}, &ow.qkvc)) return -1;
                }
                if (make_conv1(c, b + ".attn1.to_out.0", &ow.to_out1) || nobias(b + ".attn2.to_q", &ow.xqc) ||
                    make_conv1(c, b + ".attn2.to_out.0", &ow.to_out2) || make_conv1(c, b + ".ff.net.0.proj", &ow.ff1) ||
                    make_conv1(c, b + ".ff.net.2", &ow.ff2)) return -1;
                std::vector<float> z0((size_t)C, 0.f);
                if (upload(c, &ow.xkw, c->params[b + ".attn2.to_k.weight"].data) || upload(c, &ow.xkb, z0) ||
                    upload(c, &ow.xvw, c->params[b + ".attn2.to_v.weight"].data) || upload(c, &ow.xvb, z0)) return -1;
                break;
            }
            case OP_OUT:
                if (make_norm(c, op.pn_n1, &ow.g1) || make_conv1(c, op.pn_conv, &ow.conv, cfg.out_ch)) return -1;
                break;
        }
    }
    W.tproj_total = (long)tpb.size();
    if (upload(c, &W.tp_w, tpw) || upload(c, &W.tp_b, tpb)) return -1;
    double fl = 0.0;
    for (size_t oi = 0; oi < W.op.size(); ++oi) {
        const OpPlan& op = c->prog->ops[oi];
        const OpWeights& ow = W.op[oi];
        auto convf = [&](const ConvP& p, int H, int W) { fl += 2.0 * p.cin * p.cout * p.taps * (double)H * W; };
        const Tens& to = c->tens[op.out];
        switch (op.kind) {
            case OP_CONV_IN: case OP_CONV: case OP_DOWN: case OP_UP: case OP_OUT: convf(ow.conv, to.H, to.W); break;
            case OP_RES:
                convf(ow.c1, to.H, to.W); convf(ow.c2, to.H, to.W);
                if (op.has_nin) convf(ow.nin, to.H, to.W);
                break;
            case OP_XFMR: {
                for (const ConvP* p : {&ow.pj_in, &ow.qkvc, &ow.to_out1, &ow.xqc, &ow.to_out2, &ow.ff1, &ow.ff2, &ow.pj_out}) convf(*p, to.H, to.W);
                double T = (double)to.H * to.W;
                fl += 2.0 * 2.0 * T * T * to.C + 2.0 * 2.0 * T * c->cfg.context_len * to.C;
                break;
            }
            case OP_ATTN: {
                convf(ow.qkvc, to.H, to.W); convf(ow.proj, to.H, to.W);
                double T = (double)to.H * to.W;
                fl += 2.0 * 2.0 * T * T * to.C;
                if (op.has_x) {
                    convf(ow.xqc, to.H, to.W); convf(ow.xproj, to.H, to.W);
                    fl += 2.0 * 2.0 * T * c->cfg.context_len * to.C;
                }
                break;
            }
        }
    }
    W.flops = fl;
    for (auto& kv : c->params) { std::vector<float>().swap(kv.second.data); }
    return bind_weights(c);
}

struct Pass {
    loco_ctx* c;
    hipStream_t st;
    int B;
    float* arena;
    float* stats;
    float* T(int id) const { return arena + c->tens[id].off; }
    long bs() const { return c->prog->per_sample; }
};

static void drop_graphs(loco_ctx* c) {
// ... 29 lines not shown
}

void conv_defaults(ConvArgs& a) {
    std::memset(&a, 0, sizeof(a));
    a.stride = 1; a.pad = 1; a.nsplit = 1; a.mode = CM_NONE; a.res_scale = 1.f;
}

struct NS { float *sc, *sh, *mr, *tst, *tc; };
NS nstats(const loco_ctx* c, float* base, const NormP& n) {
    NS s;
    s.sc = base + n.soff; s.sh = s.sc + n.C; s.mr = s.sh + n.C; s.tst = s.mr + 2 * c->cfg.gn_groups;
    s.tc = s.tst + 2 * c->cfg.gn_groups;
    return s;
}

struct StatReq {
    int kind = ST_NONE;
    NormP* n = nullptr;
    float* stats = nullptr;
    const float* prim = nullptr;
    const float* ss_scale = nullptr; const float* ss_shift = nullptr;
    float* keep = nullptr; size_t keep_floats = 0; int* keep_ntile = nullptr;
};

void stats_standalone(loco_ctx* c, const StatReq& rq, const float* x, long xbs, int B, int HW, int s0, hipStream_t st) {
    const NormP& n = *rq.n;
    const long SB = c->prog->stats_per_sample;
    const int G = c->cfg.gn_groups;
    if (rq.kind == ST_FWD) {
        NS s = nstats(c, rq.stats + (long)s0 * SB, n);
        launch_gn_stats(x, xbs, B, n.C, HW, G, eps_of(c, n), n.gamma, n.beta, s.mr, s.sc, s.sh, SB, c->red, st, rq.ss_scale,
                        rq.ss_shift);
    } else {
        NS sp = nstats(c, c->statsP, n);
        NS stt = nstats(c, rq.stats + (long)s0 * SB, n);
        launch_gn_tstats(x, xbs, rq.prim, 0, B, n.C, HW, G, sp.sc, sp.sh, sp.mr, 0, 0, rq.kind == ST_TAN ? 0 : 1, stt.tst,
                         stt.tc, SB, c->red, st, c->cfg.act);
    }
}

bool run_conv(loco_ctx* c, const ConvArgs& a0, int taps, hipStream_t st, const StatReq* rq = nullptr,
              const ConvArgs* second = nullptr) {
    const size_t span = (size_t)c->cfg.max_batch * c->prog->per_sample;
    auto padded = [&](const float* p) { return (p >= c->arenaP && p < c->arenaP + span) || (p >= c->arenaT && p < c->arenaT + span); };
    ConvArgs a = a0, sc;
    a.act = c->cfg.act;
    if (a.mode == CM_GN_SILU && c->cfg.act == ACT_GELU) a.mode = CM_GN_GELU;
    a.in_padded = padded(a.in);
    if (second) { sc = *second; sc.in_padded = padded(sc.in); }
    ConvEnv e;
    e.prec = c->prec; e.chip_share = c->chip_share; e.lanes = c->lanes_active; e.lane_s0 = c->lane_s0;
    e.partial = c->partial; e.partial_floats = c->partial_floats; e.stpart = c->stpart; e.stpart_floats = c->stpart_floats;
    e.fuse_stats = c->fuse_stats; e.fuse_lin = c->fuse_lin; e.deep1 = c->deep1; e.max_batch = c->cfg.max_batch;
    StatAsk q;
    if (rq) {
        q.kind = rq->kind; q.norm = rq->n != nullptr; q.prim = rq->prim; q.keep = rq->keep; q.keep_floats = rq->keep_floats;
        if (rq->n && rq->n->sx_off >= 0 && c->sxcache) q.sx = c->sxcache + rq->n->sx_off;
    }
    const ConvPlan p = plan_conv(e, a, taps, rq ? &q : nullptr, second ? &sc : nullptr);
    if (p.sc_first) run_conv(c, *second, 1, st);
#ifdef LOCO_DIAG
    if (c->plan_log) conv_plan_text(p, taps, c->prec, *c->plan_log);
#endif
    if (rq && rq->kind != ST_NONE && rq->n) rq->n->ready = true;
    if (rq && rq->keep_ntile) *rq->keep_ntile = p.keep_ntile;
    const int HWo = a.Hout * a.Wout, Gn = c->cfg.gn_groups;
    const long SBs = c->prog->stats_per_sample;
    auto timed = [&](const char* name, double flops, const ConvArgs& y, auto&& launch) {
        loco_ctx::ProfRec r;
        if (c->prof_on) {
            r.name = name; r.flops = flops;
            r.cin = y.Cin; r.cout = y.Cout; r.h = y.Hout; r.b = y.B; r.ns = y.nsplit; r.mode = y.mode; r.taps = taps;
            r.e0 = c->next_event(); r.e1 = c->next_event();
            (void)hipEventRecord(r.e0, st);
        }
        launch();
        if (c->prof_on) { (void)hipEventRecord(r.e1, st); c->prof.push_back(r); }
    };
    for (int li = 0; li < p.nl; ++li) {
        const ConvLaunch& l = p.l[li];
        const ConvArgs& x = l.args;
        double flops = 2.0 * (x.Cin * taps + x.Cin2) * x.Cout * (double)x.Hout * x.Wout * x.B;
        if (x.zins) flops *= 0.25;
        timed(c->prof_on ? conv_variant_name(x, taps, c->prec) : nullptr, flops, x, [&] {
            if (c->prec == 1) launch_conv_bf16x3(x, taps, st);
            else if (c->prec == 2) launch_conv_f16(x, taps, st);
            else launch_conv(x, taps, st);
        });
        if (x.nsplit > 1) {
            timed("conv_splitk_reduce", 0.0, x, [&] {
                if (l.stats != SR_SPLITK) { launch_conv_splitk_reduce(x, st); return; }
                const NormP& n = *rq->n;
                NS sp = nstats(c, c->statsP, n);
                NS so = nstats(c, rq->stats + (long)l.s0 * SBs, n);
                launch_conv_splitk_reduce_stats(x, rq->kind, Gn, eps_of(c, n), n.gamma, n.beta, so.mr, so.sc, so.sh, SBs, rq->ss_scale,
                                                rq->ss_shift, rq->prim, sp.sc, sp.sh, sp.mr, so.tst, so.tc, SBs, c->red, st);
            });
        }
        if (l.stats == SR_ALONE) stats_standalone(c, *rq, x.out, x.out_bs, x.B, HWo, l.s0, st);
        if (l.stats == SR_EPI) {
            const NormP& n = *rq->n;
            NS so = nstats(c, rq->stats + (long)l.s0 * SBs, n);
            if (rq->kind != ST_FWD) {
                NS sp = nstats(c, c->statsP, n);
                launch_gn_lin_fused_finalize(rq->kind, x.st_part, n.C, l.ntile, nullptr, 0, x.B, n.C, HWo, Gn, sp.mr, so.tst, so.tc,
                                             SBs, st);
            } else {
                launch_gn_fused_finalize(x.st_part, l.ntile, x.B, n.C, HWo, Gn, eps_of(c, n), n.gamma, n.beta, so.mr, so.sc, so.sh,
                                         SBs, rq->ss_scale, rq->ss_shift, st);
            }
        }
    }
    if (p.stats_all) stats_standalone(c, *rq, a.out, a.out_bs, a.B, HWo, 0, st);
    return p.cot;
}

inline void setw(ConvArgs& a, const ConvP& p, bool dgrad) {
    a.w = dgrad ? p.wd : p.wf;
    a.wb = dgrad ? (const void*)p.wbd : (const void*)p.wbf;
    a.wh = dgrad ? (const void*)p.whd : (const void*)p.whf;
}

NormP* consumer_norm(loco_ctx* c, int tid) {
    const Tens& t = c->tens[tid];
    if (t.cons_op < 0) return nullptr;
    Op& op = c->ops[t.cons_op];
    return t.cons_norm == 2 ? &op.nx : &op.n1;
}
StatReq req_fwd(NormP* n, float* stats, const float* ss_scale = nullptr, const float* ss_shift = nullptr) {
    StatReq r;
    if (n) { r.kind = ST_FWD; r.n = n; r.stats = stats; r.ss_scale = ss_scale; r.ss_shift = ss_shift; }
    return r;
}
StatReq req_lin(loco_ctx* c, int kind, NormP* n, const float* prim) {
    StatReq r;
    if (n) { r.kind = kind; r.n = n; r.stats = c->statsT; r.prim = prim; }
    return r;
}
void clear_ready(loco_ctx* c) {
    for (auto& op : c->ops) op.n1.ready = op.n2.ready = op.nx.ready = false;
    for (auto& t : c->tens) t.keep_ntile = 0;
}
StatReq req_fwd_of(loco_ctx* c, int tid, float* stats) {
    StatReq r = req_fwd(consumer_norm(c, tid), stats);
    Tens& t = c->tens[tid];
    if (t.cat_of >= 0 && t.keep) {
        r.kind = ST_FWD; r.stats = stats;
        r.keep = t.keep; r.keep_floats = t.keep_floats; r.keep_ntile = &t.keep_ntile;
    }
    return r;
}
bool cat_fused_stats(loco_ctx* c, const NormP& n, int tid, float* stats, int B, hipStream_t st) {
    const Tens& q = c->tens[tid];
    if (q.cat_a < 0 || c->prec < 1 || !c->fuse_stats) return false;
    const Tens& A = c->tens[q.cat_a];
    const Tens& Bt = c->tens[q.cat_b];
    if (A.keep_ntile <= 0 || Bt.keep_ntile <= 0) return false;
    NS s = nstats(c, stats, n);
    launch_gn_fused_finalize_cat(A.keep, A.C, A.keep_ntile, Bt.keep, Bt.keep_ntile, B, q.C, q.H * q.W, c->cfg.gn_groups,
                                 eps_of(c, n), n.gamma, n.beta, s.mr, s.sc, s.sh, c->prog->stats_per_sample, st);
    return true;
}

bool cat_fused_tstats(loco_ctx* c, const NormP& n, int tid, int B, hipStream_t st) {
    const Tens& q = c->tens[tid];
    if (q.cat_a < 0 || c->prec < 1 || !c->fuse_stats || !c->fuse_lin) return false;
    const Tens& A = c->tens[q.cat_a];
    const Tens& Bt = c->tens[q.cat_b];
    if (A.keep_ntile <= 0 || Bt.keep_ntile <= 0) return false;
    NS sp = nstats(c, c->statsP, n);
    NS stt = nstats(c, c->statsT, n);
    const size_t MB = c->cfg.max_batch;
    launch_gn_lin_fused_finalize(ST_TAN, A.keep + c->lane_s0 * (A.keep_floats / MB), A.C, A.keep_ntile,
                                 Bt.keep + c->lane_s0 * (Bt.keep_floats / MB), Bt.keep_ntile, B, q.C, q.H * q.W,
                                 c->cfg.gn_groups, sp.mr, stt.tst, stt.tc, c->prog->stats_per_sample, st);
    return true;
}

void gn_forward_stats(const Pass& p, const NormP& n, const float* x, long xbs, int HW) {
    NS s = nstats(p.c, p.stats, n);
    launch_gn_stats(x, xbs, p.B, n.C, HW, p.c->cfg.gn_groups, eps_of(p.c, n), n.gamma, n.beta, s.mr, s.sc, s.sh,
                    p.c->prog->stats_per_sample, p.c->red, p.st);
}


struct XA {
    loco_ctx* c; const Op* op; hipStream_t st; int B; int C, T, NH, CH, Lp;
    float scale;
};
XA xa_of(loco_ctx* c, const Op& op, int B, hipStream_t st) {
    XA x; x.c = c; x.op = &op; x.st = st; x.B = B;
    const Tens& t = c->tens[op.in];
    x.C = t.C; x.T = t.H * t.W; x.NH = op.heads; x.CH = x.C / x.NH; x.Lp = c->prog->ctx_Lp;
    x.scale = 1.0f / std::sqrt((float)x.CH);
    return x;
}
void xa_scores(const XA& x, const float* X, long x_bs, const float* K, float* S, long s_bs, float alpha, bool mask) {
    GemmArgs g; std::memset(&g, 0, sizeof(g));
    g.A = X; g.sam = 1; g.sak = x.T; g.sab = x_bs; g.sah = (long)x.CH * x.T;
    g.Bm = K; g.sbk = x.Lp; g.sbn = 1; g.sbb = 0; g.sbh = (long)x.CH * x.Lp;
    g.C = S; g.scm = x.Lp; g.scn = 1; g.scb = s_bs; g.sch = (long)x.T * x.Lp;
    g.M = x.T; g.N = x.Lp; g.K = x.CH; g.batch = x.B; g.batch2 = x.NH; g.alpha = alpha; g.beta = 0.f;
    g.colbias = mask ? x.c->ctx_colbias : nullptr;
// ... 519 lines not shown
                lin1x1(c, op.xqc, false, XT_(X_A2), PS, C, XT_(X_XQ), PS, C, H, W, B, nullptr, 0, false, st);
                xa_linear(xa, XT_(X_XQ), op.xK, op.xV, XP(X_XS), XT_(X_XS), XT_(X_XO));
                lin1x1(c, op.to_out2, false, XT_(X_XO), PS, C, XT_(X_H2), PS, C, H, W, B, XT_(X_H1), PS, false, st);
                launch_ln_tan(XT_(X_H2), PS, XP(X_H2), XP(X_LN3), B, C, T, op.lng[2], XT_(X_A3), PS, st);
                lin1x1(c, op.ff1, false, XT_(X_A3), PS, C, XT_(X_F), PS, 8 * C, H, W, B, nullptr, 0, false, st);
                launch_geglu(1, XT_(X_F), PS, XP(X_F), B, 4L * C * T, XT_(X_GG), PS, st);
                lin1x1(c, op.ff2, false, XT_(X_GG), PS, 4 * C, XT_(X_H3), PS, C, H, W, B, XT_(X_H2), PS, false, st);
                const StatReq rq = next_tan(op.out);
                lin1x1(c, op.pj_out, false, XT_(X_H3), PS, C, TT(op.out), PS, C, H, W, B, TT(op.in), PS, false, st, &rq);
                break;
            }
            case OP_DOWN: case OP_UP: {
                const Tens& ti = c->tens[op.in];
                ConvArgs a; conv_defaults(a);
                a.in = TT(op.in); a.in_bs = PS; a.Cin = ti.C; a.Hin = ti.H; a.Win = ti.W;
                setw(a, op.conv, false);
                if (op.kind == OP_DOWN) { a.stride = 2; a.pad = op.sym_down ? 1 : 0; } else { a.upsample = 1; }
                a.out = TT(op.out); a.out_bs = PS; a.Cout = to.C; a.Hout = to.H; a.Wout = to.W; a.B = B;
                const StatReq rq = next_tan(op.out);
                run_conv(c, a, 9, st, &rq);
                break;
            }
            case OP_OUT: {
                const Tens& ti = c->tens[op.in];
                if (!op.n1.ready) tangent_stats(c, op.n1, TT(op.in), PS, TP(op.in), ti.H * ti.W, B, st);
                op.n1.ready = false;
                ConvArgs a; conv_defaults(a);
                a.in = TT(op.in); a.in_bs = PS; a.Cin = ti.C; a.Hin = ti.H; a.Win = ti.W;
                setw(a, op.conv, false);
                set_tan(c, a, op.n1, TP(op.in));
                a.out = TT(op.out); a.out_bs = PS; a.Cout = to.C; a.Hout = to.H; a.Wout = to.W; a.B = B;
                run_conv(c, a, 9, st);
                break;
            }
        }
    }
    return 0;
}

void cot_stats(loco_ctx* c, const NormP& n, const float* d, long dbs, const float* x, int HW, int B, int kind,
               hipStream_t st) {
    NS sp = nstats(c, c->statsP, n);
    NS stt = nstats(c, c->statsT, n);
    launch_gn_tstats(d, dbs, x, 0, B, n.C, HW, c->cfg.gn_groups, sp.sc, sp.sh, sp.mr, 0, 0, kind, stt.tst,
                     stt.tc, c->prog->stats_per_sample, c->red, st, c->cfg.act);
}

int cotangent_pass(loco_ctx* c, const float* ge, const float* gx0, float* Aout, int B, hipStream_t st) {
    const loco_unet_cfg& cfg = c->cfg;
    const long PS = c->prog->per_sample;
    const int G = cfg.gn_groups;
    auto TP = [&](int id) { return c->arenaP + c->tens[id].off; };
    auto TG = [&](int id) { return c->arenaT + c->tens[id].off; };
    auto GO = [&](const Op& o) -> const float* { return o.out == c->prog->eps_t ? ge : TG(o.out); };
    auto GOS = [&](const Op& o) -> long { return o.out == c->prog->eps_t ? (long)c->prog->n_out : PS; };
    clear_ready(c);
    for (int oi = (int)c->ops.size() - 1; oi >= 0; --oi) {
        Op& op = c->ops[oi];
        const Tens& to = c->tens[op.out];
        const int HW = to.H * to.W;
        switch (op.kind) {
            case OP_OUT: {
                const Tens& ti = c->tens[op.in];
                ConvArgs a; conv_defaults(a);
                a.in = GO(op); a.in_bs = GOS(op); a.Cin = to.C; a.Hin = to.H; a.Win = to.W;
                setw(a, op.conv, true);
                a.out = TG(op.a1); a.out_bs = PS; a.Cout = ti.C; a.Hout = ti.H; a.Wout = ti.W; a.B = B;
                {
                    const StatReq rq = req_lin(c, ST_COT, &op.n1, TP(op.in));
                    run_conv(c, a, 9, st, &rq);
                    op.n1.ready = false;
                }
                NS sp = nstats(c, c->statsP, op.n1);
                NS stt = nstats(c, c->statsT, op.n1);
                launch_gn_apply(2, TG(op.a1), PS, TP(op.in), 0, nullptr, 0, TG(op.in), PS, 0, B, ti.C, ti.H * ti.W, G,
                                sp.sc, sp.sh, sp.mr, 0, 0, stt.tst, c->prog->stats_per_sample, st, cfg.act);
                break;
            }
            case OP_UP: {
                const Tens& ti = c->tens[op.in];
                ConvArgs a; conv_defaults(a);
                a.in = TG(op.out); a.in_bs = PS; a.Cin = to.C; a.Hin = to.H; a.Win = to.W;
                setw(a, op.conv, true);
                a.out = TG(op.up); a.out_bs = PS; a.Cout = ti.C; a.Hout = to.H; a.Wout = to.W; a.B = B;
                run_conv(c, a, 9, st);
                launch_pool2x2_sum(TG(op.up), PS, TG(op.in), PS, 0, B, ti.C, ti.H, ti.W, st);
                break;
            }
            case OP_DOWN: {
                const Tens& ti = c->tens[op.in];
                ConvArgs a; conv_defaults(a);
                a.in = TG(op.out); a.in_bs = PS; a.Cin = to.C; a.Hin = to.H; a.Win = to.W;
                setw(a, op.conv, true); a.zins = 1; a.pad = op.sym_down ? 1 : 2; a.accumulate = op.in_is_skip ? 1 : 0;
                a.out = TG(op.in); a.out_bs = PS; a.Cout = ti.C; a.Hout = ti.H; a.Wout = ti.W; a.B = B;
                run_conv(c, a, 9, st);
                break;
            }
            case OP_RES: {
                const Tens& ti = c->tens[op.in];
                const int HWi = ti.H * ti.W;
                ConvArgs a; conv_defaults(a);
                a.in = TG(op.out); a.in_bs = PS; a.Cin = to.C; a.Hin = to.H; a.Win = to.W;
                setw(a, op.c2, true);
                a.out = TG(op.h1); a.out_bs = PS; a.Cout = to.C; a.Hout = to.H; a.Wout = to.W; a.B = B;
                {
                    const StatReq rq2 = req_lin(c, ST_COT, &op.n2, TP(op.h1));
                    run_conv(c, a, 9, st, &rq2);
                    op.n2.ready = false;
                }
                ConvArgs b; conv_defaults(b);
                b.in = TG(op.h1); b.in_bs = PS; b.Cin = to.C; b.Hin = to.H; b.Win = to.W;
                setw(b, op.c1, true);
                set_tan(c, b, op.n2, TP(op.h1));
                b.mode = CM_COT_SILU;
                b.out_bs = PS; b.Cout = ti.C; b.Hout = to.H; b.Wout = to.W; b.B = B;
                if (op.updown == 0) {
                    b.out = TG(op.a1);
                    const StatReq rq1 = req_lin(c, ST_COT, &op.n1, TP(op.in));
                    run_conv(c, b, 9, st, &rq1);
                } else if (op.updown == 1) {
                    b.out = TG(op.ap);
                    run_conv(c, b, 9, st);
                    launch_upsample2x(TG(op.ap), PS, TG(op.a1), PS, 0, 0.25f, B, ti.C, to.H, to.W, st);
                } else {
                    b.out = TG(op.xu);
                    run_conv(c, b, 9, st);
                    launch_pool2x2_sum(TG(op.xu), PS, TG(op.a1), PS, 0, B, ti.C, ti.H, ti.W, st);
                }
                if (!op.n1.ready) cot_stats(c, op.n1, TG(op.a1), PS, TP(op.in), HWi, B, 1, st);
                op.n1.ready = false;
                NS sp = nstats(c, c->statsP, op.n1);
                NS stt = nstats(c, c->statsT, op.n1);
                int acc = op.in_is_skip ? 1 : 0;
                const float* gsk = TG(op.out);
                bool cot_in_epilogue = false;
                if (op.has_nin) {
                    ConvArgs n; conv_defaults(n);
                    n.in = TG(op.out); n.in_bs = PS; n.Cin = to.C; n.Hin = to.H; n.Win = to.W;
                    setw(n, op.nin, true); n.pad = 0;
                    n.Cout = ti.C; n.Hout = to.H; n.Wout = to.W; n.B = B; n.out_bs = PS;
                    n.out = TG(op.in); n.accumulate = acc;
                    if (op.updown == 0 && c->prec >= 1 && c->fuse_cot && op.n1.sx_off >= 0 && c->sxcache) {
                        n.cot_d = TG(op.a1); n.cot_d_bs = PS; n.cot_sx = c->sxcache + op.n1.sx_off;
                        n.cot_tc = stt.tc; n.cot_tc_bs = c->prog->stats_per_sample;
                    }
                    cot_in_epilogue = run_conv(c, n, 1, st);
                    gsk = nullptr;
                }
                if (op.updown == 0) {
                    if (cot_in_epilogue) {  }
                    else if (op.has_nin)
                        launch_gn_apply(2, TG(op.a1), PS, TP(op.in), 0, nullptr, 0, TG(op.in), PS, 1, B, ti.C, HWi, G,
                                        sp.sc, sp.sh, sp.mr, 0, 0, stt.tst, c->prog->stats_per_sample, st, cfg.act);
                    else
                        launch_gn_apply(2, TG(op.a1), PS, TP(op.in), 0, gsk, PS, TG(op.in), PS, acc, B, ti.C, HWi, G,
                                        sp.sc, sp.sh, sp.mr, 0, 0, stt.tst, c->prog->stats_per_sample, st, cfg.act, c->prog->res_scale);
                } else {
                    launch_gn_apply(2, TG(op.a1), PS, TP(op.in), 0, nullptr, 0, TG(op.in), PS, acc, B, ti.C, HWi, G,
                                    sp.sc, sp.sh, sp.mr, 0, 0, stt.tst, c->prog->stats_per_sample, st, cfg.act);
                    if (op.updown == 1) launch_upsample2x(gsk, PS, TG(op.in), PS, 1, 0.25f * c->prog->res_scale, B, ti.C, to.H, to.W, st);
                    else launch_pool2x2_sum(gsk, PS, TG(op.in), PS, 1, B, ti.C, ti.H, ti.W, st, c->prog->res_scale);
                }
                break;
            }
            case OP_ATTN: {
                const int C = to.C;
                const int so = op.has_x ? op.xmid : op.out;
                if (op.has_x) {
                    const XA x = xa_of(c, op, B, st);
// ... 717 lines not shown
                       int32_t rule, float* m_out, uint8_t* mask_out, void* stream) {
    if (!c) return -2;
    if (!eps_a || !eps_b || !mask_out || B < 1 || C < 1 || HW < 1) { c->err = "diffedit_mask: bad arguments"; return -2; }
    if (rule != 0 && rule != 1) { c->err = "diffedit_mask: rule is 0 (reference) or 1 (intended)"; return -2; }
    float* ws = reinterpret_cast<float*>(c->gscratch);
    const size_t cap = 2 * ((((size_t)c->prog->n_in + 255) / 256) * 64 * 64 + 4096);
    float* m = m_out;
    if (!m) {
        if (1024 + (size_t)HW > cap) { c->err = "diffedit_mask: map larger than the reduction workspace; pass m_out"; return -2; }
        m = ws + 1024;
    }
    hipStream_t st = (hipStream_t)stream;
    launch_diffedit_mask(eps_a, eps_b, scale, B, C, (long)HW, rule, m, mask_out, ws, ws + 768, st);
    HIPCHK(c, hipGetLastError());
    float status[3] = {0.f, 0.f, 0.f};
    HIPCHK(c, hipMemcpyAsync(status, ws + 768, sizeof(status), hipMemcpyDeviceToHost, st));
    HIPCHK(c, hipStreamSynchronize(st));
    if (status[0] == 1.f) {
        c->err = "diffedit_mask: constant map (max == min = " + std::to_string(status[1]) + "): the two noise predictions do not differ";
        return -4;
    }
    if (status[0] != 0.f) { c->err = "diffedit_mask: non-finite map"; return -5; }
    return 0;
}

int loco_cfg_masked_step(loco_ctx* c, const float* x, const float* eps_for, const float* eps_edit, const float* eps_null,
                         float g, float at, float at_next, const uint8_t* mask, int32_t B, int64_t n, float* x_next,
                         void* stream) {
    if (!c) return -2;
    if (!x || !eps_for || !eps_edit || !eps_null || !mask || !x_next || B < 1 || n < 1) {
        c->err = "cfg_masked_step: bad arguments";
        return -2;
    }
    float s1, s2, s3, ce, cn;
    sched_coeffs(at, at_next, 0.f, &s1, &s2, &s3, &ce, &cn);
    launch_cfg_masked_step(x, eps_for, eps_edit, eps_null, mask, x_next, B, (long)n, g, s2, s1, s3, ce, (hipStream_t)stream);
    HIPCHK(c, hipGetLastError());
    return 0;
}

int loco_lcm_step(loco_ctx* c, const float* x, const float* eps, float at, float at_prev, float c_skip, float c_out,
                  const float* noise, int64_t count, float* x_prev, float* denoised, void* stream) {
    if (!c) return -2;
    if (!x || !eps || count < 1 || (!x_prev && !denoised)) { c->err = "lcm_step: bad arguments"; return -2; }
    if (!(at > 0.f && at <= 1.f) || !(at_prev >= 0.f && at_prev <= 1.f)) { c->err = "lcm_step: alpha-bar outside (0, 1]"; return -2; }
    launch_lcm_step(x, eps, noise, x_prev, denoised, (long)count, std::sqrt(at), std::sqrt(1.0f - at), std::sqrt(at_prev),
                    std::sqrt(1.0f - at_prev), c_skip, c_out, (hipStream_t)stream);
    HIPCHK(c, hipGetLastError());
    return 0;
}

#ifdef LOCO_DIAG
}
__global__ void diag_fill_records(unsigned char* rec, long nrec, int wpitch, unsigned seed, float scale) {
    const long r = (long)blockIdx.x * 256 + threadIdx.x;
    if (r >= nrec) return;
    const int idx = (int)(r % wpitch);
    unsigned short hi[16], lo[16];
    for (int k = 0; k < 16; ++k) {
        unsigned h = (unsigned)(r * 16 + k) * 2654435761u + seed * 40503u;
        h ^= h >> 15; h *= 2246822519u; h ^= h >> 13; h *= 3266489917u; h ^= h >> 16;
        const float v = scale * ((float)(h & 0xffffff) * (1.0f / 8388608.0f) - 1.0f);
        const __bf16 hb = (__bf16)v;
        const __bf16 lb = (__bf16)(v - (float)hb);
        hi[k] = __builtin_bit_cast(unsigned short, hb);
        lo[k] = __builtin_bit_cast(unsigned short, lb);
    }
    const int sw = (idx >> 2) & 3;
    unsigned short* base = reinterpret_cast<unsigned short*>(rec + r * 64);
    for (int k = 0; k < 8; ++k) {
        base[((0 ^ sw) << 3) + k] = hi[k];
        base[((1 ^ sw) << 3) + k] = hi[8 + k];
        base[((2 ^ sw) << 3) + k] = lo[k];
        base[((3 ^ sw) << 3) + k] = lo[8 + k];
    }
}
extern "C" {
int loco_bench_conv(loco_ctx* c, int32_t cin, int32_t cout, int32_t H, int32_t W, int32_t B, int32_t mode,
                    int32_t taps, int32_t tile, int32_t iters, float* ms_avg, void* stream) {
    if (!c) return -2;
    if (finalize_params(c)) return -3;
    hipStream_t st = (hipStream_t)stream;
    const long HW = (long)H * W;
    const long in_e = (long)cin * HW, out_e = (long)cout * HW;
    if ((in_e + out_e) * B > (long)c->cfg.max_batch * c->prog->per_sample || 2 * in_e > (long)c->prog->per_sample ||
        in_e > c->prog->sx_total) { c->err = "bench_conv: shape exceeds the arenas"; return -2; }
    float* in = c->arenaT;
    float* out = c->arenaT + in_e * B;
    const int bz = getenv("LOCO_BENCH_ZERO") ? atoi(getenv("LOCO_BENCH_ZERO")) : 0;
    const float zs = (bz & 1) ? 0.0f : 1.0f, zw = (bz & 2) ? 0.0f : 1.0f;
    launch_fill_random(in, in_e * B, 1u, zs, st);
    launch_fill_random(c->arenaP, in_e, 2u, zs, st);
    launch_fill_random(reinterpret_cast<float*>(c->sxcache), 2 * in_e, 3u, zs, st);
    launch_fill_random(c->statsP, c->prog->stats_per_sample, 4u, 1.0f, st);
    launch_fill_random(c->statsT, c->prog->stats_per_sample * B, 5u, 0.01f, st);
    size_t wfl = (size_t)((cin + 15) / 16) * 16 * taps * ((cout + 31) & ~31);
    if (wfl * 2 > c->partial_floats) { c->err = "bench_conv: weights exceed workspace"; return -2; }
    float* wf = c->partial + c->partial_floats - wfl * 2;
    launch_fill_random(wf, (long)wfl * 2, 6u, 0.05f * zw, st);
    if (c->prec == 1) {
        const long nrec = (long)((cin + 15) / 16) * taps * ((cout + 31) & ~31);
        hipLaunchKernelGGL(diag_fill_records, dim3((unsigned)((nrec + 255) / 256)), dim3(256), 0, st,
                           reinterpret_cast<unsigned char*>(wf), nrec, (cout + 31) & ~31, 7u, 0.05f * zw);
    }
    ConvArgs a; conv_defaults(a);
    a.in = in; a.in_bs = in_e; a.Cin = cin; a.Hin = H; a.Win = W;
    a.prim = c->arenaP; a.prim_bs = 0; a.sx = c->sxcache;
    a.w = wf; a.wb = wf; a.wh = wf;
    a.out = out; a.out_bs = out_e; a.Cout = cout; a.Hout = H; a.Wout = W; a.B = B;
    a.mode = mode; a.pad = taps == 9 ? 1 : 0; a.in_padded = 1; a.taps = taps;
    a.sc = c->statsP; a.sh = c->statsP + cin; a.scsh_bs = 0; a.mr = c->statsP + 2 * cin; a.mr_bs = 0;
    a.gamma_ = c->statsP; a.tst = c->statsT; a.tst_bs = c->prog->stats_per_sample; a.cpg = cin / c->cfg.gn_groups;
    a.tc = c->statsT + 64; a.tc_bs = c->prog->stats_per_sample;
    if (a.cpg < 1) a.cpg = 1;
    a.nsplit = 1; a.partial = c->partial;
    a.partial_floats = c->partial_floats - wfl * 2;
    if (getenv("LOCO_BENCH_COT") && atoi(getenv("LOCO_BENCH_COT")) && taps == 1) {
        if ((in_e + 2 * out_e) * B > (long)c->cfg.max_batch * c->prog->per_sample || out_e > c->prog->sx_total ||
            2L * cout > c->prog->stats_per_sample) { c->err = "bench_conv: cot operands exceed the arenas"; return -2; }
        launch_fill_random(out + out_e * B, out_e * B, 8u, zs, st);
        if (out_e > in_e) launch_fill_random(reinterpret_cast<float*>(c->sxcache), 2 * out_e, 3u, zs, st);
        a.cot_d = out + out_e * B; a.cot_d_bs = out_e; a.cot_sx = c->sxcache; a.cot_tc = c->statsT; a.cot_tc_bs = c->prog->stats_per_sample;
    }
    if (getenv("LOCO_BENCH_ACC") && atoi(getenv("LOCO_BENCH_ACC"))) a.accumulate = 1;
    conv_plan_family(a, c->prec);
    if (const char* e = getenv("LOCO_DUAL_WHATIF")) a.no_deep = atoi(e);
    conv_plan_tile_pair(a, c->prec, tile);
    auto run = [&]() {
        if (c->prec == 1) launch_conv_bf16x3(a, taps, st);
        else if (c->prec == 2) launch_conv_f16(a, taps, st);
        else launch_conv(a, taps, st);
        launch_conv_splitk_reduce(a, st);
    };
    run();
    HIPCHK(c, hipEventRecord(c->ev0, st));
    for (int i = 0; i < iters; ++i) run();
    HIPCHK(c, hipEventRecord(c->ev1, st));
    HIPCHK(c, hipEventSynchronize(c->ev1));
    c->bench_out = out; c->bench_out_count = (int64_t)out_e * B;
    float ms = 0.f;
    HIPCHK(c, hipEventElapsedTime(&ms, c->ev0, c->ev1));
    *ms_avg = ms / iters;
    HIPCHK(c, hipGetLastError());
    return 0;
}

}
__global__ void diag_scale_tc(const float* tc, const float* mr, int C, int cpg, long n, int by_rstd, float* out) {
    const long i = (long)blockIdx.x * 256 + threadIdx.x;
    if (i >= n) return;
    const float f = by_rstd ? mr[2 * (int)((i % C) / cpg) + 1] : 1.0f;
    out[2 * i] = f * tc[2 * i];
    out[2 * i + 1] = f * tc[2 * i + 1];
}
extern "C" {
int loco_debug_conv(loco_ctx* c, const loco_conv_desc* d, char* plan, int64_t cap, void* stream) {
    if (!c) return -2;
    if (!d || d->struct_size != (int32_t)sizeof(loco_conv_desc)) { c->err = "debug_conv: descriptor size mismatch"; return -2; }
    if (finalize_params(c)) return -3;
    hipStream_t st = (hipStream_t)stream;
    const int taps = d->taps, k = taps == 9 ? 3 : 1, B = d->B;
    if ((taps != 9 && taps != 1) || d->Cin < 1 || d->Cout < 1 || d->Hin < 1 || d->Win < 1 || B < 1 || (d->stride != 1 && d->stride != 2) ||
        d->mode < CM_NONE || d->mode > CM_GN_GELU || (d->upsample && d->zins) || (d->stride == 2 && (d->upsample || d->zins)) ||
        !d->weight || !d->in || !d->out) { c->err = "debug_conv: bad descriptor"; return -2; }
    if (d->stride == 2 && ((d->Hin | d->Win) & 1)) { c->err = "debug_conv: stride 2 needs an even map"; return -2; }
    const bool lin = d->mode == CM_TAN_SILU || d->mode == CM_COT_SILU;
    if (d->mode != CM_NONE && (!d->sc || !d->sh)) { c->err = "debug_conv: the prologue modes need sc / sh"; return -2; }
    if (lin && (!d->prim || !d->mr || !d->gamma || !d->tst || !d->tc || d->cpg < 1 || d->Cin % d->cpg)) {
        c->err = "debug_conv: modes 3 / 4 need prim, mr, gamma, tst, tc and cpg"; return -2;
    }
    if (d->Cin2 > 0 && (!d->in2 || !d->w2)) { c->err = "debug_conv: the second operator needs in2 and w2"; return -2; }
    if (d->Cin2 > 0 && (d->res || d->accumulate || taps != 9)) {
        c->err = "debug_conv: the second operator goes with a 3x3 conv without res / accumulate"; return -2;
    }
    if (d->cot_d && (!d->cot_prim || !d->cot_sc || !d->cot_sh || !d->cot_mr || !d->cot_tc || d->cot_cpg < 1 || d->Cout % d->cot_cpg)) {
        c->err = "debug_conv: the norm-cotangent term needs cot_prim, cot_sc, cot_sh, cot_mr, cot_tc and cot_cpg"; return -2;
    }
    const int Hout = d->stride == 2 ? d->Hin / 2 : (d->upsample || d->zins) ? 2 * d->Hin : d->Hin;
    const int Wout = d->stride == 2 ? d->Win / 2 : (d->upsample || d->zins) ? 2 * d->Win : d->Win;
    {
        auto pow2 = [](int v) { return v >= 8 && (v & (v - 1)) == 0; };
        if (!((pow2(Hout) && pow2(Wout)) || (Wout % 32 == 0 && Hout % 8 == 0 && ((long)Hout * Wout) % 256 == 0))) {
            c->err = "debug_conv: output map outside the tile geometry of the conv kernels"; return -2;
        }
    }
    const long in_e = (long)d->Cin * d->Hin * d->Win, out_e = (long)d->Cout * Hout * Wout, in2_e = (long)d->Cin2 * Hout * Wout;
    if ((in_e | out_e | in2_e) & 3) { c->err = "debug_conv: planes must be whole 16-byte units"; return -2; }
    auto up64 = [](long v) { return (v + 63) & ~63L; };
    const long offT_in2 = d->in_arena ? up64(in_e * B) : 0, offT_cot = offT_in2 + up64(in2_e * B);
    const long needT = offT_cot + (d->cot_d ? out_e * B : 0);
    const long sx_cot = lin ? up64(in_e) : 0, need_sx = sx_cot + (d->cot_d ? out_e : 0);
    if (needT > (long)c->cfg.max_batch * c->prog->per_sample || (lin && in_e > (long)c->cfg.max_batch * c->prog->per_sample) ||
        need_sx > c->prog->sx_total) { c->err = "debug_conv: shape exceeds the arenas"; return -2; }
    const int G = lin ? d->Cin / d->cpg : 0;
    const long tbs = up64(2L * G) + up64(2L * d->Cin);
    const long small_n = (lin ? (long)B * tbs : 0) + (d->cot_d ? (long)B * up64(2L * d->Cout) : 0) + 64;
    const size_t owned0 = c->owned.size();
    const size_t bytes0 = c->bytes;
    auto release = [&]() {
        (void)hipStreamSynchronize(st);
        while (c->owned.size() > owned0) { (void)hipFree(c->owned.back()); c->owned.pop_back(); }
        c->bytes = bytes0;
    };
    auto host_param = [&](const float* p, std::vector<int64_t> shape) {
        HostParam h; h.shape = shape; h.loaded = true;
        size_t n = 1; for (int64_t s : shape) n *= (size_t)s;
        if (p) h.data.assign(p, p + n); else h.data.assign(n, 0.f);
        return h;
    };
    const int m_out = d->transposed ? d->Cin : d->Cout, m_in = d->transposed ? d->Cout : d->Cin;
    HostParam w = host_param(d->weight, {m_out, m_in, k, k}), wb0 = host_param(nullptr, {m_out});
    HostParam w2 = host_param(d->Cin2 > 0 ? d->w2 : nullptr, {d->Cout, d->Cin2 > 0 ? d->Cin2 : 1, 1, 1}), wb2 = host_param(nullptr, {d->Cout});
    ConvP cp, cp2;
    float *bias_d = nullptr, *bias2nd_d = nullptr, *small = nullptr;
    int rc = make_conv(c, {&w}, {&wb0}, &cp);
    if (!rc && d->Cin2 > 0) rc = make_conv(c, {&w2}, {&wb2}, &cp2);
    if (!rc && d->bias) rc = upload(c, &bias_d, std::vector<float>(d->bias, d->bias + d->Cout));
    if (!rc && d->Cin2 > 0 && d->bias2nd) rc = upload(c, &bias2nd_d, std::vector<float>(d->bias2nd, d->bias2nd + d->Cout));
    if (!rc) rc = dalloc(c, &small, (size_t)small_n);
    if (rc) { release(); return -1; }
    auto copy = [&](float* dst, const float* src, long n) {
        return hipMemcpyAsync(dst, src, (size_t)n * sizeof(float), hipMemcpyDeviceToDevice, st);
    };
    hipError_t he = hipSuccess;
    ConvArgs a; conv_defaults(a);
    if (d->in_arena) { he = copy(c->arenaT, d->in, in_e * B); a.in = c->arenaT; } else a.in = d->in;
    a.in_bs = in_e; a.Cin = d->Cin; a.Hin = d->Hin; a.Win = d->Win;
    setw(a, cp, d->transposed != 0);
    a.bias = bias_d;
    a.out = d->out; a.out_bs = out_e; a.Cout = d->Cout; a.Hout = Hout; a.Wout = Wout; a.B = B;
    a.bias2 = d->bias2; a.bias2_bs = d->Cout;
    a.res = d->res; a.res_bs = out_e; a.res_scale = d->res_scale;
    a.mode = d->mode; a.stride = d->stride; a.upsample = d->upsample; a.zins = d->zins; a.accumulate = d->accumulate;
    a.pad = d->pad >= 0 ? d->pad : taps == 1 ? 0 : d->zins ? 2 : d->stride == 2 ? 0 : 1;
    a.sc = d->sc; a.sh = d->sh; a.scsh_bs = 0; a.cpg = d->cpg;
    if (lin) {
        if (he == hipSuccess) he = copy(c->arenaP, d->prim, in_e);
        a.prim = c->arenaP; a.prim_bs = 0;
        a.mr = d->mr; a.mr_bs = 0; a.gamma_ = d->gamma;
        for (int b = 0; b < B && he == hipSuccess; ++b) he = copy(small + b * tbs, d->tst + (long)b * 2 * G, 2L * G);
        a.tst = small; a.tst_bs = tbs;
        for (int b = 0; b < B; ++b)
            hipLaunchKernelGGL(diag_scale_tc, dim3((unsigned)((d->Cin + 255) / 256)), dim3(256), 0, st, d->tc + (long)b * 2 * d->Cin, d->mr,
                               d->Cin, d->cpg, (long)d->Cin, d->mode == CM_COT_SILU ? 1 : 0, small + b * tbs + up64(2L * G));
        a.tc = small + up64(2L * G); a.tc_bs = tbs;
        launch_gn_cache(c->arenaP, d->Cin, d->Hin * d->Win, d->cpg, d->sc, d->sh, d->mr, c->sxcache, st, ACT_SILU);
        a.sx = c->sxcache;
    }
    ConvArgs n2; conv_defaults(n2);
    if (d->Cin2 > 0) {
        float* in2 = c->arenaT + offT_in2;
        if (he == hipSuccess) he = copy(in2, d->in2, in2_e * B);
        n2.in = in2; n2.in_bs = in2_e; n2.Cin = d->Cin2; n2.Hin = Hout; n2.Win = Wout;
        setw(n2, cp2, false); n2.bias = bias2nd_d; n2.pad = 0;
        n2.out = d->out; n2.out_bs = out_e; n2.Cout = d->Cout; n2.Hout = Hout; n2.Wout = Wout; n2.B = B;
        a.res = d->out; a.res_bs = out_e;
    }
    if (d->cot_d) {
        float* cd = c->arenaT + offT_cot;
        float* ctc = small + (lin ? (long)B * tbs : 0);
        const long cbs = up64(2L * d->Cout);
        if (he == hipSuccess) he = copy(cd, d->cot_d, out_e * B);
        for (int b = 0; b < B; ++b)
            hipLaunchKernelGGL(diag_scale_tc, dim3((unsigned)((d->Cout + 255) / 256)), dim3(256), 0, st, d->cot_tc + (long)b * 2 * d->Cout,
                               d->cot_mr, d->Cout, d->cot_cpg, (long)d->Cout, 1, ctc + b * cbs);
        launch_gn_cache(d->cot_prim, d->Cout, Hout * Wout, d->cot_cpg, d->cot_sc, d->cot_sh, d->cot_mr, c->sxcache + sx_cot, st, ACT_SILU);
        a.cot_d = cd; a.cot_d_bs = out_e; a.cot_sx = c->sxcache + sx_cot; a.cot_tc = ctc; a.cot_tc_bs = cbs;
    }
    if (he != hipSuccess) { c->err = std::string("debug_conv: ") + hipGetErrorString(he); release(); return -1; }
    std::string text;
    const int act0 = c->cfg.act;
    if (d->mode == CM_GN_GELU) c->cfg.act = ACT_GELU;
    c->plan_log = &text;
    const bool rode = run_conv(c, a, taps, st, nullptr, d->Cin2 > 0 ? &n2 : nullptr);
    c->plan_log = nullptr;
    c->cfg.act = act0;
    he = hipGetLastError();
    release();
    if (he == hipSuccess) he = hipGetLastError();
    if (he != hipSuccess) { c->err = std::string("debug_conv: ") + hipGetErrorString(he); return -1; }
    if (plan && cap > 0) {
        if ((int64_t)text.size() + 1 > cap) { c->err = "debug_conv: plan buffer too small"; return -4; }
        std::memcpy(plan, text.c_str(), text.size() + 1);
    }
    if (d->cot_d && !rode) { c->err = "debug_conv: norm-cotangent term declined"; return 1; }
    return 0;
}

#endif

int loco_set_streams(loco_ctx* c, int32_t n) {
    if (!c || (n != 1 && n != 2)) return -2;
    c->n_streams = n;
    return 0;
}

int loco_set_chip_share(loco_ctx* c, int32_t n) {
    if (!c || n < 1 || n > 8) return -2;
    c->chip_share = n;
    return 0;
}

int loco_set_side_stream(loco_ctx* c, void* stream) {
    if (!c) return -2;
    c->st2_user = (hipStream_t)stream;
    return 0;
}

int loco_profile_enable(loco_ctx* c, int32_t on) {
    if (!c) return -2;
    c->prof_on = on != 0;
    c->prof_shapes = on == 2;
    if (on) { c->prof.clear(); c->ev_used = 0; }
    return 0;
}

int loco_profile_report(loco_ctx* c, char* buf, int64_t cap) {
    if (!c || !buf || cap < 1) return -2;
    HIPCHK(c, hipDeviceSynchronize());
    std::map<std::string, std::array<double, 3>> agg;
    for (auto& r : c->prof) {
        float ms = 0.f;
        if (hipEventElapsedTime(&ms, r.e0, r.e1) != hipSuccess) continue;
        std::string key = r.name;
        if (c->prof_shapes) {
            char sb[96];
            snprintf(sb, sizeof(sb), "|t%d_m%d_ci%d_co%d_h%d_b%d_s%d", r.taps, r.mode, r.cin, r.cout, r.h, r.b, r.ns);
            key += sb;
        }
        auto& a = agg[key];
        a[0] += 1.0; a[1] += ms; a[2] += r.flops;
    }
    std::string out;
    char line[256];
    for (auto& kv : agg) {
        snprintf(line, sizeof(line), "%s %.0f %.6f %.6e\n", kv.first.c_str(), kv.second[0], kv.second[1], kv.second[2]);
        out += line;
    }
    if ((int64_t)out.size() + 1 > cap) { c->err = "profile buffer too small"; return -4; }
    std::memcpy(buf, out.c_str(), out.size() + 1);
    return 0;
}

#ifdef LOCO_DIAG
int64_t loco_debug_tensor(loco_ctx* c, const char* name, float* dst, int64_t cap, void* stream) {
    if (!c) return -2;
    std::string nm(name);
    if (nm == "bench_out") {
        if (!c->bench_out) { c->err = "no loco_bench_conv yet"; return -3; }
        int64_t cnt = cap < c->bench_out_count ? cap : c->bench_out_count;
        HIPCHK(c, hipMemcpyAsync(dst, c->bench_out, (size_t)cnt * sizeof(float), hipMemcpyDeviceToDevice, (hipStream_t)stream));
        return cnt;
    }
    if (nm == "workspace") {
        int64_t cnt = cap < (int64_t)c->partial_floats ? cap : (int64_t)c->partial_floats;
        HIPCHK(c, hipMemcpyAsync(dst, c->partial, (size_t)cnt * sizeof(float), hipMemcpyDeviceToDevice, (hipStream_t)stream));
        return cnt;
    }
    int arena = 0;
// ... 23 lines not shown
```

### loco-edit_amd/csrc/kernels.h

```cpp
#pragma once
#include <hip/hip_runtime.h>
#include <stdint.h>

namespace loco {

struct DeviceOnce { bool seen[64] = {}; };
inline bool first_on_device(DeviceOnce& f) {
    int d = 0;
    (void)hipGetDevice(&d);
    d &= 63;
    if (f.seen[d]) return false;
    f.seen[d] = true;
    return true;
}


enum ConvMode : int {
    CM_NONE = 0,
    CM_GN_SILU = 1,
    CM_GN = 2,
    CM_TAN_SILU = 3,
    CM_COT_SILU = 4,
    CM_GN_GELU = 5,
};
enum ActKind : int { ACT_SILU = 0, ACT_GELU = 1 };
__device__ __forceinline__ float act_fwd(float y, int act) {
    if (act == ACT_GELU) return 0.5f * y * (1.0f + erff(y * 0.70710678118654752f));
    return y * (1.0f / (1.0f + __expf(-y)));
}
__device__ __forceinline__ float act_der(float y, int act) {
    if (act == ACT_GELU) return 0.5f * (1.0f + erff(y * 0.70710678118654752f)) + y * 0.39894228040143268f * __expf(-0.5f * y * y);
    const float sg = 1.0f / (1.0f + __expf(-y));
    return sg * (1.0f + y * (1.0f - sg));
}

enum StatKind : int { ST_NONE = 0, ST_FWD = 1, ST_TAN = 2, ST_COT = 3 };

struct ConvArgs {
    const float* in; long in_bs; int Cin, Hin, Win;
    const float* prim; long prim_bs;
    const float* w;
    const void* wb;
    const void* wh;
    const float2* sx;
    float* out; long out_bs; int Cout, Hout, Wout;
    const float* bias;
    const float* bias2; long bias2_bs;
    const float* res; long res_bs;
    const float* sc; const float* sh; long scsh_bs;
    const float* mr; long mr_bs;
    const float* gamma_;
    const float* tst; long tst_bs;
    const float* tc; long tc_bs;
    int cpg;
    int mode;
    int stride;
    int pad;
    int upsample;
    int zins;
    int in_padded;
    int accumulate;
    int nsplit;
    int taps;
    int no_deep;
    float* partial;
    int B;
    float* st_part; int st_kind;
    const float* st_x; const float2* st_sx;
    const float* in2; long in2_bs; int Cin2; int in2_padded;
    const void* wb2;
    const float* cot_d; long cot_d_bs; const float2* cot_sx; const float* cot_tc; long cot_tc_bs;
    int act;
    float res_scale;
    int gemm, gemm_tm;
    size_t partial_floats;
    int tile, pair;
};

void launch_conv(const ConvArgs& a, int taps, hipStream_t st);
void launch_conv_bf16x3(const ConvArgs& a, int taps, hipStream_t st);
void launch_conv_f16(const ConvArgs& a, int taps, hipStream_t st);
void launch_conv_splitk_reduce(const ConvArgs& a, hipStream_t st);

struct ConvEnv {
    int prec = 1;
    int chip_share = 1;
    int lanes = 1, lane_s0 = 0;
    float* partial = nullptr; size_t partial_floats = 0;
    float* stpart = nullptr; size_t stpart_floats = 0;
    bool fuse_stats = true, fuse_lin = true, deep1 = true;
    int max_batch = 1;
};

struct StatAsk {
    int kind = ST_NONE;
    bool norm = false;
    const float2* sx = nullptr;
    const float* prim = nullptr;
    float* keep = nullptr; size_t keep_floats = 0;
};

enum StatRoute : int {
    SR_NONE = 0,
    SR_EPI = 1,
    SR_SPLITK = 2,
    SR_ALONE = 3,
    SR_KEEP = 4,
};

struct ConvLaunch {
    ConvArgs args;
    int s0 = 0;
    int stats = SR_NONE;
    int ntile = 0;
};

struct ConvPlan {
    bool sc_first = false;
    int nl = 1;
    ConvLaunch l[2];
    bool stats_all = false;
    int keep_ntile = 0;
    bool cot = false;
};

ConvPlan plan_conv(const ConvEnv& env, const ConvArgs& a, int taps, const StatAsk* ask, const ConvArgs* shortcut);
void conv_plan_family(ConvArgs& a, int prec);
void conv_plan_tile_pair(ConvArgs& a, int prec, int tile_override);

int conv_bf16_tile_couts(const ConvArgs& a);
const char* conv_variant_name(const ConvArgs& a, int taps, int prec);

void launch_fill_random(float* p, long count, unsigned seed, float scale, hipStream_t st);
void launch_gn_cache(const float* x, int C, int HW, int cpg, const float* sc, const float* sh, const float* mr,
                     float2* sx, hipStream_t st, int act = 0);

struct GemmArgs {
    const float* A; long sam, sak, sab;
    const float* Bm; long sbk, sbn, sbb;
    float* C; long scm, scn, scb;
    const float* bias;
    const float* colbias;
    const float* R; long srb;
    int M, N, K, batch;
    float alpha, beta;
    int batch2; long sah, sbh, sch;
    const float* A2; long sab2; const float* Bm2; long sbb2;
};
void launch_gemm(const GemmArgs& g, hipStream_t st);
enum GemmAct : int { GEMM_ACT_NONE = 0, GEMM_ACT_QUICK_GELU = 1, GEMM_ACT_GELU = 2 };
void launch_gemm_fixed(const GemmArgs& g, int act, hipStream_t st);
void launch_gemm_bf16x3(const GemmArgs& g, hipStream_t st);
bool gemm_prefers_bf16x3(const GemmArgs& g);
bool gemm_rec_eligible(const GemmArgs& g);
size_t gemm_rec_ws_bytes(const GemmArgs& g);
void launch_gemm_rec(const GemmArgs& g, unsigned char* ws, hipStream_t st);

struct AttnFlashArgs {
    int T, NH, B, CH; float scale;
    const float *q, *k, *v; long hs;
    const float* P;
    const float* o;
    const float *dq, *dk, *dv; long bs_d;
    float* out; long bs_out;
    const float* go; long bs_go;
    float *gq, *gk, *gv; long bs_g;
    float* delta;
    int Lt; const float *kt, *vt;
    unsigned char* ws; size_t ws_bytes;
};
size_t attn_flash_ws_bytes(const AttnFlashArgs& a);
bool attn_flash_supported(int T, int CH);
bool attn_flash_text_supported(int T, int CH, int Lt);
void launch_attn_flash_tangent(const AttnFlashArgs& a, hipStream_t st);
void launch_attn_flash_cotangent(const AttnFlashArgs& a, hipStream_t st);

void launch_ln_fwd(const float* x, long xbs, int B, int C, int T, const float* gamma, const float* beta, float eps, float* y,
                   long ybs, float* stats, long sbs, hipStream_t st);
void launch_ln_tan(const float* dx, long dbs, const float* xprim, const float* sprim, int B, int C, int T, const float* gamma,
                   float* dy, long ybs, hipStream_t st);
void launch_ln_cot(const float* gy, long gbs, const float* xprim, const float* sprim, int B, int C, int T, const float* gamma,
                   const float* base, long base_bs, float* gx, long xbs, hipStream_t st);
struct XAttnArgs {
    int T, NH, B, CH, L, Lp, fwd;
    float alpha;
    const float* X; long x_bs;
    const float* K1; const float* K2;
    float* P; long p_bs;
    float* O; long o_bs;
};
bool xattn_fused_supported(int T, int CH, int L, int Lp);
void launch_xattn_fused(const XAttnArgs& a, hipStream_t st);
void launch_geglu(int kind, const float* in, long in_bs, const float* fprim, int B, long n4, float* out, long out_bs,
                  hipStream_t st);

void launch_gn_stats(const float* x, long bs, int B, int C, int HW, int G, float eps,
                     const float* gamma, const float* beta,
                     float* mr, float* sc, float* sh, long stats_bs, double* scratch, hipStream_t st,
                     const float* ss_scale = nullptr, const float* ss_shift = nullptr);
void launch_gn_fused_finalize_cat(const float* partA, int C1, int ntA, const float* partB, int ntB, int B, int C, int HW, int G,
                                  float eps, const float* gamma, const float* beta, float* mr, float* sc, float* sh,
                                  long stats_bs, hipStream_t st);
void launch_gn_fused_finalize(const float* part, int ntile, int B, int C, int HW, int G, float eps, const float* gamma,
                              const float* beta, float* mr, float* sc, float* sh, long stats_bs, const float* ss_scale,
                              const float* ss_shift, hipStream_t st);
// ... 86 lines not shown
```

### loco-edit_amd/hip.py

```python
from __future__ import annotations

import ctypes as C
import os
from typing import Dict, Optional

import numpy as np
import torch

from .config import UNetConfig

_LIB_PATH = os.environ.get("LOCO_HIP_LIB") or os.path.join(os.path.dirname(os.path.abspath(__file__)), "libloco_hip.so")
_lib = None

DIAG_SYMBOLS = ["loco_bench_conv", "loco_debug_conv", "loco_debug_tensor"]

SYMBOLS = [
    "loco_version", "loco_device_count", "loco_create", "loco_fork", "loco_destroy", "loco_last_error",
    "loco_load_param", "loco_params_missing", "loco_unet_forward", "loco_ddim_step", "loco_sched_step",
    "loco_pmp_primal", "loco_pmp_set_second_mask", "loco_pmp_jvp", "loco_pmp_vjp", "loco_orthonormalize", "loco_qr_rows",
    "loco_convergence", "loco_convergence_rows", "loco_null_project", "loco_edit_axpy", "loco_mask_gather", "loco_mask_count",
    "loco_unet_flops", "loco_workspace_bytes", "loco_clock_stamp", "loco_set_side_stream", "loco_timer_start", "loco_timer_stop",
    "loco_profile_enable", "loco_profile_report", "loco_set_precision", "loco_get_precision", "loco_set_streams", "loco_set_chip_share",
    "loco_set_cond", "loco_set_context", "loco_lincomb", "loco_masked_axpby", "loco_latent_sample",
    "loco_text_create", "loco_text_load_param", "loco_text_params_missing", "loco_text_encode", "loco_text_last_error",
    "loco_text_destroy", "loco_t5_create", "loco_text_encode_masked",
    "loco_diffedit_mask", "loco_cfg_masked_step", "loco_set_time_cond", "loco_lcm_step",
    "loco_sam_create", "loco_sam_load_param", "loco_sam_params_missing", "loco_sam_encode", "loco_sam_profile",
    "loco_sam_profile_read", "loco_sam_last_error", "loco_sam_destroy",
    "loco_samdec_create", "loco_samdec_load_param", "loco_samdec_params_missing", "loco_samdec_set_image", "loco_samdec_predict",
    "loco_samdec_score", "loco_samdec_binarize", "loco_samdec_last_error", "loco_samdec_destroy",
    "loco_clipvis_create", "loco_clipvis_load_param", "loco_clipvis_params_missing", "loco_clipvis_preprocess",
    "loco_clipvis_encode", "loco_clipvis_last_error", "loco_clipvis_destroy",
    "loco_quality_create", "loco_quality_load_param", "loco_quality_params_missing", "loco_quality_lpips", "loco_quality_ssim",
    "loco_quality_masked_mse", "loco_quality_last_error", "loco_quality_destroy",
]

DIFFEDIT_RULES = {"reference": 0, "intended": 1}


class LocoCfg(C.Structure):
    _fields_ = [
        ("struct_size", C.c_int32), ("resolution", C.c_int32), ("in_channels", C.c_int32), ("out_ch", C.c_int32), ("ch", C.c_int32),
        ("num_levels", C.c_int32), ("ch_mult", C.c_int32 * 8), ("num_res_blocks", C.c_int32),
        ("num_attn_res", C.c_int32), ("attn_resolutions", C.c_int32 * 8), ("gn_groups", C.c_int32),
        ("gn_eps", C.c_float), ("max_batch", C.c_int32),
        ("arch", C.c_int32), ("num_head_channels", C.c_int32), ("learn_sigma", C.c_int32),
        ("context_dim", C.c_int32), ("context_len", C.c_int32),
        ("scale_shift_norm", C.c_int32), ("resblock_updown", C.c_int32), ("num_heads", C.c_int32),
        ("transformer_depth", C.c_int32),
        ("act", C.c_int32), ("res_scale", C.c_float), ("added_kv", C.c_int32),
        ("time_cond_proj_dim", C.c_int32),
    ]


class LocoConvDesc(C.Structure):
    _PTRS = ("weight", "bias", "in", "bias2", "res", "prim", "sc", "sh", "mr", "gamma", "tst", "tc", "in2", "w2", "bias2nd",
             "cot_d", "cot_prim", "cot_sc", "cot_sh", "cot_mr", "cot_tc", "out")
    _HOST = ("weight", "bias", "w2", "bias2nd")
    _fields_ = ([("struct_size", C.c_int32)] +
                [(k, C.c_int32) for k in ("Cin", "Cout", "Hin", "Win", "B", "taps", "stride", "upsample", "zins", "mode", "cpg",
                                          "transposed", "accumulate", "in_arena", "pad", "Cin2", "cot_cpg")] +
                [("res_scale", C.c_float), ("reserved", C.c_int32)] + [(k, C.c_void_p) for k in _PTRS])


class LocoTextCfg(C.Structure):
    _fields_ = [("vocab", C.c_int32), ("width", C.c_int32), ("layers", C.c_int32), ("heads", C.c_int32), ("ffn", C.c_int32),
                ("positions", C.c_int32), ("act", C.c_int32), ("ln_eps", C.c_float)]


class LocoT5Cfg(C.Structure):
    _fields_ = [("vocab", C.c_int32), ("d_model", C.c_int32), ("d_kv", C.c_int32), ("heads", C.c_int32), ("d_ff", C.c_int32),
                ("layers", C.c_int32), ("positions", C.c_int32), ("buckets", C.c_int32), ("max_distance", C.c_int32),
                ("act", C.c_int32), ("ln_eps", C.c_float)]


SAM_MAX_GLOBAL = 16


class LocoSamCfg(C.Structure):
    _fields_ = [("image_size", C.c_int32), ("patch_size", C.c_int32), ("width", C.c_int32), ("depth", C.c_int32),
                ("heads", C.c_int32), ("mlp_dim", C.c_int32), ("window_size", C.c_int32), ("num_global", C.c_int32),
                ("global_attn", C.c_int32 * SAM_MAX_GLOBAL), ("out_channels", C.c_int32), ("ln_eps", C.c_float)]


class LocoSamDecCfg(C.Structure):
    _fields_ = [("grid", C.c_int32), ("image_size", C.c_int32), ("hidden", C.c_int32), ("layers", C.c_int32), ("heads", C.c_int32),
                ("mlp_dim", C.c_int32), ("attention_downsample_rate", C.c_int32), ("num_multimask_outputs", C.c_int32),
                ("iou_head_depth", C.c_int32), ("iou_head_hidden_dim", C.c_int32), ("layer_norm_eps", C.c_float),
                ("hidden_act", C.c_int32), ("max_prompts", C.c_int32)]


class LocoClipVisCfg(C.Structure):
    _fields_ = [("image_size", C.c_int32), ("patch_size", C.c_int32), ("width", C.c_int32), ("layers", C.c_int32),
                ("heads", C.c_int32), ("mlp_dim", C.c_int32), ("projection_dim", C.c_int32), ("act", C.c_int32),
                ("ln_eps", C.c_float), ("image_mean", C.c_float * 3), ("image_std", C.c_float * 3)]


class LocoQualityCfg(C.Structure):
    _fields_ = [("max_h", C.c_int32), ("max_w", C.c_int32), ("ssim_window", C.c_double * 11)]


def library_path() -> str:
    return _LIB_PATH


def load_library():
    global _lib
    if _lib is not None:
        return _lib
    if not os.path.exists(_LIB_PATH):
        raise RuntimeError(
            f"{_LIB_PATH} not found: build it with `python -c 'import __graft_entry__ as g; g.build()'` "
            "(hipcc --offload-arch=gfx950). There is no CPU fallback.")
    lib = C.CDLL(_LIB_PATH)
    vp, i32, i64, f32 = C.c_void_p, C.c_int32, C.c_int64, C.c_float
    lib.loco_version.restype = C.c_char_p
    lib.loco_device_count.restype = C.c_int
    lib.loco_create.argtypes = [C.POINTER(LocoCfg), C.POINTER(vp)]
    if hasattr(lib, "loco_fork"):
        lib.loco_fork.argtypes = [vp, C.c_int32, C.POINTER(vp)]
    lib.loco_destroy.argtypes = [vp]
    lib.loco_destroy.restype = None
    lib.loco_last_error.argtypes = [vp]
    lib.loco_last_error.restype = C.c_char_p
    lib.loco_load_param.argtypes = [vp, C.c_char_p, vp, C.POINTER(i64), i32, i32]
    lib.loco_params_missing.argtypes = [vp]
    lib.loco_unet_forward.argtypes = [vp, vp, f32, i32, vp, vp]
    lib.loco_ddim_step.argtypes = [vp, vp, f32, f32, f32, f32, vp, i32, vp, vp]
    lib.loco_sched_step.argtypes = [vp, vp, vp, f32, f32, f32, vp, i64, vp, vp, vp]
    lib.loco_pmp_primal.argtypes = [vp, vp, f32, f32, vp, i32, vp]
    lib.loco_pmp_set_second_mask.argtypes = [vp, vp, i32, vp]
    lib.loco_pmp_jvp.argtypes = [vp, vp, i32, vp, vp]
    lib.loco_pmp_vjp.argtypes = [vp, vp, i32, vp, vp]
    lib.loco_orthonormalize.argtypes = [vp, vp, i32, i64, vp, vp]
    lib.loco_qr_rows.argtypes = [vp, vp, i32, i64, vp]
    lib.loco_convergence.argtypes = [vp, vp, vp, i64, f32, vp, vp]
    lib.loco_convergence_rows.argtypes = [vp, vp, vp, i32, i64, f32, vp, vp]
    lib.loco_null_project.argtypes = [vp, vp, i32, vp, i32, i64, vp, vp]
    lib.loco_edit_axpy.argtypes = [vp, vp, vp, C.POINTER(f32), i32, i64, vp, vp]
    lib.loco_mask_gather.argtypes = [vp, vp, i32, vp, vp]
    lib.loco_mask_count.argtypes = [vp]
    lib.loco_mask_count.restype = i64
    lib.loco_clock_stamp.argtypes = [vp, vp, vp]
    lib.loco_set_side_stream.argtypes = [vp, vp]
    lib.loco_unet_flops.argtypes = [vp]
# ... 454 lines not shown
                                           _ptr(noise), x.numel(), _ptr(prev), _ptr(den), _stream()), "loco_lcm_step")
        return prev, den

    def version(self) -> str:
        return self.lib.loco_version().decode()

    def clock_stamp(self) -> torch.Tensor:
        out = torch.zeros(2, device=self.device, dtype=torch.int64)
        self._check(self.lib.loco_clock_stamp(self._ctx, _ptr(out), _stream()), "loco_clock_stamp")
        return out

    @staticmethod
    def sclk_mhz(stamp0: torch.Tensor, stamp1: torch.Tensor) -> float:
        d = (stamp1 - stamp0).tolist()
        return 100.0 * d[0] / max(d[1], 1)

    def unet_flops(self) -> float:
        return float(self.lib.loco_unet_flops(self._ctx))

    def workspace_bytes(self) -> int:
        return int(self.lib.loco_workspace_bytes(self._ctx))

    def timer_start(self):
        self._check(self.lib.loco_timer_start(self._ctx, _stream()), "loco_timer_start")

    def timer_stop(self) -> float:
        ms = C.c_float()
        self._check(self.lib.loco_timer_stop(self._ctx, _stream(), C.byref(ms)), "loco_timer_stop")
        return float(ms.value)

    PRECISIONS = {"f32": 0, "bf16x3": 1, "f16": 2}

    def set_precision(self, mode: str):
        self._check(self.lib.loco_set_precision(self._ctx, self.PRECISIONS[mode]), "loco_set_precision")

    def set_streams(self, n: int):
        self._check(self.lib.loco_set_streams(self._ctx, int(n)), "loco_set_streams")

    def set_chip_share(self, n: int):
        self._check(self.lib.loco_set_chip_share(self._ctx, int(n)), "loco_set_chip_share")

    def set_side_stream(self, stream: "Optional[torch.cuda.Stream]"):
        self._side_stream = stream
        ptr = C.c_void_p(stream.cuda_stream) if stream is not None else None
        self._check(self.lib.loco_set_side_stream(self._ctx, ptr), "loco_set_side_stream")

    def set_streams_measured(self, n: int):
        if n == 2:
            from .tloco import BranchStreams
            side = BranchStreams._pick(1, self.device)
            if not side:
                self.set_streams(1)
                return 1
            self.set_side_stream(side[0])
        self.set_streams(n)
        return n

    def get_precision(self) -> str:
        m = self.lib.loco_get_precision(self._ctx)
        return {v: k for k, v in self.PRECISIONS.items()}[m]

    def _need_diag(self, sym):
        if not hasattr(self.lib, sym):
            raise RuntimeError(f"{sym} is a diagnostic of include/loco_hip_diag.h: build `make -C loco-edit_amd/csrc diag` "
                               "and set LOCO_HIP_LIB=<repo>/loco-edit_amd/libloco_hip_diag.so")

    def bench_conv(self, cin, cout, H, W, B, mode, taps=9, tile=-1, iters=20) -> float:
        self._need_diag("loco_bench_conv")
        ms = C.c_float()
        self._check(self.lib.loco_bench_conv(self._ctx, cin, cout, H, W, B, mode, taps, tile, iters, C.byref(ms),
                                             _stream()), "loco_bench_conv")
        return float(ms.value)

    def debug_conv(self, out: torch.Tensor, **desc):
        self._need_diag("loco_debug_conv")
        d = LocoConvDesc()
        d.struct_size = C.sizeof(LocoConvDesc)
        d.stride, d.in_arena, d.pad, d.res_scale = 1, 1, -1, 1.0
        keep = []
        _chk_dev(out)
        d.out = out.data_ptr()
        for k, v in desc.items():
            if k not in LocoConvDesc._PTRS:
                if not hasattr(d, k) or k in ("struct_size", "reserved"):
                    raise TypeError(f"debug_conv: no descriptor field {k!r}")
                setattr(d, k, v)
            elif v is not None:
                if k in LocoConvDesc._HOST:
                    v = v.detach().to("cpu", torch.float32).contiguous()
                else:
                    _chk_dev(v)
                keep.append(v)
                setattr(d, k, v.data_ptr())
        buf = C.create_string_buffer(1 << 12)
        rc = self.lib.loco_debug_conv(self._ctx, C.byref(d), buf, len(buf), _stream())
        if rc not in (0, 1):
            self._check(rc, "loco_debug_conv")
        plan = []
        for line in buf.value.decode().splitlines():
            rec = dict(f.split("=", 1) for f in line.split(" "))
            plan.append({k: (v if k == "kernel" else int(v)) for k, v in rec.items()})
        return plan, rc == 0

    def profile_enable(self, on):
        self._check(self.lib.loco_profile_enable(self._ctx, int(on)), "loco_profile_enable")

    def profile_report(self):
        buf = C.create_string_buffer(1 << 18)
        self._check(self.lib.loco_profile_report(self._ctx, buf, len(buf)), "loco_profile_report")
        out = {}
        for line in buf.value.decode().splitlines():
            name, n, ms, fl = line.rsplit(" ", 3)
            out[name] = dict(launches=int(float(n)), ms=float(ms), flops=float(fl))
        return out

    def debug_tensor(self, name: str, numel: int) -> torch.Tensor:
        self._need_diag("loco_debug_tensor")
        dst = torch.empty(numel, device=self.device, dtype=torch.float32)
        got = self.lib.loco_debug_tensor(self._ctx, name.encode(), _ptr(dst), numel, _stream())
        if got < 0:
            raise RuntimeError(f"loco_debug_tensor({name}) failed: {self.lib.loco_last_error(self._ctx).decode()}")
        return dst[:got]


class _EncoderEngine:
    _prefix = ""
    _label = ""

    def _open(self, device: Optional[torch.device]):
        self.lib = load_library()
        if not torch.cuda.is_available() or self.lib.loco_device_count() < 1:
            raise RuntimeError(f"loco_hip: no HIP device visible; the {self._label} has no CPU fallback")
        self.device = torch.device(device if device is not None else "cuda:0")
        if self.device.index is None:
            self.device = torch.device("cuda", torch.cuda.current_device())
        self._t = C.c_void_p()

    def _fn(self, name):
        return getattr(self.lib, f"{self._prefix}_{name}")

    def _create(self, what, c_cfg, *args):
        rc = getattr(self.lib, what)(C.byref(c_cfg), self.device.index, *args, C.byref(self._t))
        if rc != 0:
            raise RuntimeError(f"{what} failed ({rc}): {self._fn('last_error')(None).decode()}")

    def __del__(self):
        try:
            if getattr(self, "_t", None):
                self._fn("destroy")(self._t)
                self._t = None
        except Exception:
            pass

    def _check(self, rc, what):
        if rc != 0:
            raise RuntimeError(f"{what} failed ({rc}): {self._fn('last_error')(self._t).decode()}")

    def load_params(self, sd: Dict[str, "np.ndarray | torch.Tensor"]):
        if any(isinstance(v, torch.Tensor) and v.is_cuda for v in sd.values()):
            torch.cuda.synchronize()
        for name, v in sd.items():
            t = torch.as_tensor(np.asarray(v) if not isinstance(v, torch.Tensor) else v).detach().to(torch.float32).contiguous()
            if not t.is_cuda:
                t = t.cpu()
            shape = (C.c_int64 * max(t.dim(), 1))(*t.shape)
            self._check(self._fn("load_param")(self._t, name.encode(), C.c_void_p(t.data_ptr()), shape, t.dim()),
                        f"{self._prefix}_load_param({name})")
# ... 282 lines not shown
```

Before: 19.85 edit-directions/s.

## Add polyphase 4-tap conv kernels for upsample and pooled-input 3x3 convs

Adds a polyphase decomposition for 3x3 convolutions that follow a 2x nearest upsample or zero insertion. The weights are folded into four 2x2 sub-kernels with a 4x wider virtual Cout, and a matching epilogue interleaves the phases back into the full-resolution output, including the tangent statistics. A second form folds a stride-2 pooled input into a 4-phase 2x2 conv. This is meant to skip the redundant MACs over replicated or zero pixels, which cuts the 9-tap work to 4 taps, at the cost of new weight folding, extra plan gating and a new epilogue path. It is on by default through LOCO_POLYPHASE.

```diff
diff --git a/include/loco_hip_diag.h b/include/loco_hip_diag.h
--- a/include/loco_hip_diag.h
+++ b/include/loco_hip_diag.h
@@ -15,13 +15,16 @@
     int32_t transposed, accumulate, in_arena, pad;
     int32_t Cin2, cot_cpg;
     float   res_scale;
-    int32_t reserved;
+    int32_t st_cpg;
     const float *weight, *bias;
     const float *in, *bias2, *res;
     const float *prim, *sc, *sh, *mr, *gamma, *tst, *tc;
     const float *in2, *w2, *bias2nd;
     const float *cot_d, *cot_prim, *cot_sc, *cot_sh, *cot_mr, *cot_tc;
     float* out;
+    const float *st_prim, *st_mr;
+    float* st_out;
+    int32_t pool2;
 } loco_conv_desc;
 int  loco_debug_conv(loco_ctx* ctx, const loco_conv_desc* desc, char* plan, int64_t cap, void* stream);
 
diff --git a/loco-edit_amd/csrc/conv_bf16.hip b/loco-edit_amd/csrc/conv_bf16.hip
--- a/loco-edit_amd/csrc/conv_bf16.hip
+++ b/loco-edit_amd/csrc/conv_bf16.hip
@@ -9,6 +9,8 @@
 template <int PR, int MODE> void launch_kcat_b(const ConvArgs& a, hipStream_t st);
 template <int PR, int MODE> void launch_pair_b(const ConvArgs& a, hipStream_t st);
 void launch_conv_gemm(const ConvArgs& a, hipStream_t st);
+template <int PR> void launch_poly_b(const ConvArgs& a, hipStream_t st);
+template <int PR> void launch_poly_in_b(const ConvArgs& a, hipStream_t st);
 
 template <int PR>
 static void launch_lowp(const ConvArgs& a, int taps, hipStream_t st) {
@@ -22,6 +24,8 @@
     if constexpr (PR == PR_BF16X3) {
         if (taps == 1 && a.gemm) { launch_conv_gemm(a, st); return; }
     }
+    if (taps == 9 && a.poly == 2) { launch_poly_in_b<PR>(a, st); return; }
+    if (taps == 9 && a.poly) { launch_poly_b<PR>(a, st); return; }
     if (taps == 9 && a.Cin2 > 0) {
         if (a.mode == CM_GN_SILU) launch_kcat_b<PR, CM_GN_SILU>(a, st);
         else if (a.mode == CM_GN_GELU) launch_kcat_b<PR, CM_GN_GELU>(a, st);
diff --git a/loco-edit_amd/csrc/conv_bf16_inst_p.hip b/loco-edit_amd/csrc/conv_bf16_inst_p.hip
--- /dev/null
+++ b/loco-edit_amd/csrc/conv_bf16_inst_p.hip
@@ -0,0 +1,6 @@
+#include "conv_bf16_kernel.h"
+
+namespace loco {
+template void launch_poly_b<PR_BF16X3>(const ConvArgs&, hipStream_t);
+template void launch_poly_in_b<PR_BF16X3>(const ConvArgs&, hipStream_t);
+}
diff --git a/loco-edit_amd/csrc/conv_bf16_inst_p_f16.hip b/loco-edit_amd/csrc/conv_bf16_inst_p_f16.hip
--- /dev/null
+++ b/loco-edit_amd/csrc/conv_bf16_inst_p_f16.hip
@@ -0,0 +1,6 @@
+#include "conv_bf16_kernel.h"
+
+namespace loco {
+template void launch_poly_b<PR_F16>(const ConvArgs&, hipStream_t);
+template void launch_poly_in_b<PR_F16>(const ConvArgs&, hipStream_t);
+}
diff --git a/loco-edit_amd/csrc/conv_bf16_kernel.h b/loco-edit_amd/csrc/conv_bf16_kernel.h
--- a/loco-edit_amd/csrc/conv_bf16_kernel.h
+++ b/loco-edit_amd/csrc/conv_bf16_kernel.h
@@ -363,6 +363,108 @@
     }
 }
 
+template <int WM, int WN, int TM, int TN>
+__device__ __forceinline__ void conv_lowp_epilogue_poly(const ConvArgs& a, f32x16 (&acc)[TM][TN], unsigned char* smem_b, const int cot_id,
+                                                        const int pa, const int oy0, const int ox0, const int TW, const int tile_id,
+                                                        const int b) {
+    constexpr int NTHR = WM * WN * 64, NT = WN * TN * 32, NQ = NT / 4, RSTEP = NTHR / NQ, NP = 32 / RSTEP;
+    static_assert(WM == 2 && NTHR % NQ == 0 && 32 % RSTEP == 0 && NQ == 64, "polyphase epilogue: a task row is one wave");
+    const int tid = threadIdx.x, lane = tid & 63, wave = tid >> 6;
+    const int l31 = lane & 31, khalf = lane >> 5, wm = wave / WN, wn = wave % WN;
+    const int C = a.Cout >> 2, ncb = C >> 6;
+    const int ch0 = (cot_id - pa * ncb) * 64;
+    const int Wo = 2 * a.Wout;
+    const unsigned out_plane = 4u * (unsigned)(a.Hout * a.Wout);
+    float* const S = reinterpret_cast<float*>(smem_b);
+    float* const ob = a.out + (long)b * a.out_bs;
+    const float* const b2 = a.bias2 ? a.bias2 + (long)b * a.bias2_bs : nullptr;
+    const bool accu = a.accumulate != 0;
+    const bool tan_st = a.st_kind == ST_TAN;
+    const int twsh = 31 - __builtin_clz((unsigned)TW);
+    const int row0 = tid / NQ, quad0 = tid & (NQ - 1);
+    const unsigned pix0 = (unsigned)((2 * (oy0 + ((quad0 * 4) >> twsh)) + pa) * Wo + 2 * (ox0 + ((quad0 * 4) & (TW - 1))));
+    constexpr int NV = 2 * TM * NP;
+    float av[NV];
+#pragma unroll
+    for (int h = 0; h < TM; ++h) {
+        if (h > 0) {
+            asm volatile("s_waitcnt lgkmcnt(0)" ::: "memory");
+            __builtin_amdgcn_s_barrier();
+        }
+#pragma unroll
+        for (int j = 0; j < TN; ++j)
+#pragma unroll
+            for (int r = 0; r < 16; ++r)
+                S[(wm * 32 + (r & 3) + 8 * (r >> 2) + 4 * khalf) * NT + (wn * TN + j) * 32 + l31] = acc[h][j][r];
+        f32x4 xs[NP][2];
+        if (tan_st) {
+#pragma unroll
+            for (int q = 0; q < NP; ++q) {
+                const unsigned o = (unsigned)(ch0 + h * 32 + q * RSTEP + row0) * out_plane + pix0;
+                xs[q][0] = *reinterpret_cast<const f32x4*>(a.st_x + o);
+                xs[q][1] = *reinterpret_cast<const f32x4*>(a.st_x + o + 4);
+            }
+        }
+        asm volatile("s_waitcnt lgkmcnt(0)" ::: "memory");
+        __builtin_amdgcn_s_barrier();
+        f32x4 o0[NP], o1[NP];
+#pragma unroll
+        for (int q = 0; q < NP; ++q) {
+            const f32x4 v0 = *reinterpret_cast<const f32x4*>(&S[(q * RSTEP + row0) * NT + quad0 * 4]);
+            const f32x4 v1 = *reinterpret_cast<const f32x4*>(&S[(32 + q * RSTEP + row0) * NT + quad0 * 4]);
+            o0[q] = f32x4{v0[0], v1[0], v0[1], v1[1]};
+            o1[q] = f32x4{v0[2], v1[2], v0[3], v1[3]};
+        }
+        if (accu) {
+            f32x4 r0[NP], r1[NP];
+#pragma unroll
+            for (int q = 0; q < NP; ++q) {
+                const unsigned o = (unsigned)(ch0 + h * 32 + q * RSTEP + row0) * out_plane + pix0;
+                r0[q] = *reinterpret_cast<const f32x4*>(ob + o);
+                r1[q] = *reinterpret_cast<const f32x4*>(ob + o + 4);
+            }
+#pragma unroll
+            for (int q = 0; q < NP; ++q) { o0[q] += r0[q]; o1[q] += r1[q]; }
+        }
+#pragma unroll
+        for (int q = 0; q < NP; ++q) {
+            const int co = ch0 + h * 32 + q * RSTEP + row0;
+            const unsigned o = (unsigned)co * out_plane + pix0;
+            float add = 0.f;
+            if (a.bias) add += a.bias[co];
+            if (b2) add += b2[co];
+            o0[q] += add; o1[q] += add;
+            __builtin_nontemporal_store(o0[q], reinterpret_cast<f32x4*>(ob + o));
+            __builtin_nontemporal_store(o1[q], reinterpret_cast<f32x4*>(ob + o + 4));
+            if (tan_st) {
+                const f32x4 va = o0[q], vb = o1[q], xa = xs[q][0], xb = xs[q][1];
+                av[(h * NP + q) * 2] = ((va[0] + va[1]) + (va[2] + va[3])) + ((vb[0] + vb[1]) + (vb[2] + vb[3]));
+                av[(h * NP + q) * 2 + 1] = (fmaf(xa[0], va[0], xa[1] * va[1]) + fmaf(xa[2], va[2], xa[3] * va[3])) +
+                                           (fmaf(xb[0], vb[0], xb[1] * vb[1]) + fmaf(xb[2], vb[2], xb[3] * vb[3]));
+            }
+        }
+    }
+    if (tan_st) {
+        constexpr int STEPS = rs_steps(NV, 64), LEFT = NV >> STEPS;
+        static_assert((NV & (NV - 1)) == 0, "row sums per lane");
+        rs_reduce<NV, 1, 64>(av, lane);
+        if (lane < (1 << STEPS)) {
+            int base = 0;
+#pragma unroll
+            for (int sb = 0; sb < STEPS; ++sb) base += ((lane >> sb) & 1) * (NV >> (sb + 1));
+            const int ntl = (a.Hout * a.Wout) / NT, ntile = 2 * ntl;
+            float* const sp = a.st_part + (long)b * C * ntile * 2;
+#pragma unroll
+            for (int i = 0; i < LEFT; ++i) {
+                const int idx = base + i, hq = idx >> 1;
+                const int h = hq / NP, q = hq - h * NP;
+                const int co = ch0 + h * 32 + q * RSTEP + row0;
+                sp[((long)co * ntile + pa * ntl + tile_id) * 2 + (idx & 1)] = av[i];
+            }
+        }
+    }
+}
+
 template <int PR, int TAPS, int WM, int WN, int TM, int TN, int MODE, int STG, int PHASE = 0>
 __device__ __forceinline__ void conv_lowp_body(const ConvArgs& a, f32x16 (&acc)[TM][TN]) {
     constexpr int NTHR = WM * WN * 64;
@@ -371,9 +473,14 @@
     constexpr int NPC = RB / 16;
     constexpr int MT = WM * TM * 32;
     constexpr int NT = WN * TN * 32;
-    constexpr int KS = (TAPS == 9) ? 3 : 1;
+    constexpr bool POLY = (TAPS == 4 && STG == 0), PIN = (TAPS == 4 && STG == 1);
+    static_assert(TAPS != 4 || POLY || PIN, "4-tap kernels: the two polyphase forms");
+    static_assert(!PIN || (MODE == CM_NONE && PHASE == 0), "polyphase input form: raw");
+    constexpr int KS = (TAPS == 9) ? 3 : (TAPS == 4 ? 2 : 1);
+    constexpr int HK = (TAPS == 1) ? 1 : 3;
     constexpr int NTS = KS;
-    constexpr int NROW = (TAPS == 9) ? 3 : 1;
+    constexpr int NROW = KS;
+    static_assert(!POLY || (WM == 2 && TM == 2 && MODE == CM_NONE && PHASE == 0), "polyphase output form: 128 x 256 tile, raw vector staging");
     constexpr bool NEEDP = (MODE == CM_TAN_SILU || MODE == CM_COT_SILU);
     constexpr bool GEN = (STG == 1 || STG == 2);
     constexpr int NITEM = GEN ? (2 * max_halo(NT, TAPS, STG == 2) + NTHR - 1) / NTHR : 1;
@@ -465,15 +572,21 @@
                 }
         }
     }
-    const int halo_w = (TW - 1) * S + KS;
-    const int halo_h = (TH - 1) * S + KS;
+    const int halo_w = (TW - 1) * S + HK;
+    const int halo_h = (TH - 1) * S + HK;
     const int halo_sz = halo_h * halo_w;
+    int pa_ = 0, pb_ = 0;
+    if constexpr (POLY) {
+        pa_ = __builtin_amdgcn_readfirstlane(idiv_small(cot_id, a.Cout >> 8));
+        pb_ = __builtin_amdgcn_readfirstlane(wm);
+    }
+    int tap0 = pa_ * halo_w + pb_;
     const int HBYTES = (halo_sz + NDUMMY) * HP;
     Hsb = smem_b + NWB * WBYTES;
 
     const int LH = (a.upsample || a.zins) ? a.Hin * 2 : a.Hin;
     const int LW = (a.upsample || a.zins) ? a.Win * 2 : a.Win;
-    const long in_plane = (long)a.Hin * a.Win;
+    const long in_plane = PIN ? 4L * a.Hin * a.Win : (long)a.Hin * a.Win;
 
     int ipos[NITEM], ioct[NITEM];
     unsigned ivoff[NITEM];
@@ -491,7 +604,7 @@
             if (Y >= 0 && Y < LH && X >= 0 && X < LW) {
                 if (a.upsample) off = (Y >> 1) * a.Win + (X >> 1);
                 else if (a.zins) off = ((Y | X) & 1) ? -1 : (Y >> 1) * a.Win + (X >> 1);
-                else off = Y * a.Win + X;
+                else off = PIN ? 4 * Y * a.Win + 2 * X : Y * a.Win + X;
             }
         } else {
             pos = -1; oct = 0;
@@ -587,7 +700,7 @@
     float cA[(MODE == CM_NONE) ? 1 : 16], cB[(MODE == CM_NONE) ? 1 : 16];
     const float* tcb = NEEDP ? a.tc + (long)b * a.tc_bs : nullptr;
 
-    constexpr int NPART = (!GEN && NROW == 3) ? 2 : 1;
+    constexpr int NPART = (!GEN && NROW >= 2) ? 2 : 1;
     constexpr int KP = 4 / NPART;
     struct HaloRegs {
         f32x4 dq[GEN ? 1 : KP];
@@ -695,8 +808,14 @@
         }
     };
     auto load_regs = [&](float (&hvd)[NITEM][8], int chunk) {
-        const int c0 = chunk * BKC;
-        if (c0 + BKC <= a.Cin) {
+        int c0 = chunk * BKC;
+        long poff = 0;
+        if constexpr (PIN) {
+            const int cpp = a.Cin >> 6, ph = __builtin_amdgcn_readfirstlane(idiv_small(chunk, cpp));
+            c0 = (chunk - ph * cpp) * BKC;
+            poff = (long)(ph >> 1) * 2 * a.Win + (ph & 1);
+        }
+        if (PIN || c0 + BKC <= a.Cin) {
             if constexpr (TAPS == 9 && !NEEDP) {
                 const unsigned lm = pf_live ? 0xffffffffu : 0u;
                 const long pb4 = in_plane * 4;
@@ -710,7 +829,7 @@
             } else {
 #pragma unroll
             for (int k = 0; k < 8; ++k) {
-                const float* pk = inb + (long)(c0 + k) * in_plane;
+                const float* pk = inb + (long)(c0 + k) * in_plane + poff;
                 const float2* sk = NEEDP ? sxb + (long)(c0 + k) * in_plane : nullptr;
 #pragma unroll
                 for (int i = 0; i < NITEM; ++i) {
@@ -816,7 +935,7 @@
     constexpr int NLO = PR == PR_BF16X3 ? 1 : 0;
     struct Frag { s16x8 ah[TM], al[NLO ? TM : 1], bh[TN], bl[NLO ? TN : 1]; };
     auto load_frag = [&](Frag& f, int row, int tp) {
-        const int tapoff = (TAPS == 9) ? row * halo_w + tp : 0;
+        const int tapoff = (TAPS == 9) ? row * halo_w + tp : (TAPS == 4 ? tap0 + row * halo_w + tp : 0);
 #pragma unroll
         for (int i = 0; i < TM; ++i) {
             f.ah[i] = *reinterpret_cast<const s16x8*>(Ws + tp * MT * RB + aoff_hi[i]);
@@ -1103,6 +1222,10 @@
     }
     for (int ci = 0; ci < nch; ++ci) {
         const int chunk = cbeg + ci;
+        if constexpr (PIN) {
+            const int ph = __builtin_amdgcn_readfirstlane(idiv_small(chunk, a.Cin >> 6));
+            tap0 = (1 - (ph >> 1)) * halo_w + 1 - (ph & 1);
+        }
 #pragma unroll
         for (int row = 0; row < NROW; ++row) {
             const int s_ = ci * NROW + row;
@@ -1111,7 +1234,7 @@
             unsigned char* const Hcur = Hsb + (ci & 1) * HBYTES;
             unsigned char* const Hnxt = Hsb + ((ci + 1) & 1) * HBYTES;
             constexpr bool one = (NROW == 1);
-            const int st_part = one ? 0 : (NPART == 2 ? (row == 0 ? 0 : row == 1 ? 1 : -1) : (row == 2 ? 0 : -1));
+            const int st_part = one ? 0 : (NPART == 2 ? (row == 0 ? 0 : row == 1 ? 1 : -1) : (row == NROW - 1 ? 0 : -1));
             const int ld_part = one ? 0 : (NPART == 2 ? (row == 0 ? 1 : row == 1 ? 0 : -1) : (row == 0 ? 0 : -1));
             const int ld_chunk = one ? chunk + 2 : ((NPART == 2 && row == 1) ? chunk + 2 : chunk + 1);
             constexpr bool MIDLOAD = !GEN;
@@ -1155,7 +1278,8 @@
         return;
     }
     LP_STAMP(3);
-    conv_lowp_epilogue<WM, WN, TM, TN, (TAPS == 1 && PHASE == 0) ? (EPI_COT1 | EPI_STATS) : EPI_STATS>(a, acc, smem_b, co0, oy0, ox0, TW, tile_id, b, split);
+    if constexpr (POLY) conv_lowp_epilogue_poly<WM, WN, TM, TN>(a, acc, smem_b, cot_id, pa_, oy0, ox0, TW, tile_id, b);
+    else conv_lowp_epilogue<WM, WN, TM, TN, (TAPS == 1 && PHASE == 0) ? (EPI_COT1 | EPI_STATS) : EPI_STATS>(a, acc, smem_b, co0, oy0, ox0, TW, tile_id, b, split);
     LP_STAMP(4);
 #undef LP_STAMP
 }
@@ -1188,10 +1312,10 @@
 template <int PR, int TAPS, int WM, int WN, int TM, int TN, int MODE, int STG>
 static void launch_one_b2(const ConvArgs& a, hipStream_t st) {
     constexpr int MT = WM * TM * 32, NT = WN * TN * 32;
-    constexpr int KS = (TAPS == 9) ? 3 : 1;
+    constexpr int KS = (TAPS == 9) ? 3 : (TAPS == 4 ? 2 : 1), HK = (TAPS == 1) ? 1 : 3;
     int TW = a.Wout < 32 ? a.Wout : 32;
     int TH = NT / TW;
-    int halo_w = (TW - 1) * a.stride + KS, halo_h = (TH - 1) * a.stride + KS;
+    int halo_w = (TW - 1) * a.stride + HK, halo_h = (TH - 1) * a.stride + HK;
     const int nwb = (TAPS == 9 && STG != 2) ? 3 : 2;
     size_t lds = (size_t)nwb * KS * MT * rec_bytes<PR>() + 2 * ((size_t)halo_w * halo_h + NDUMMY) * halo_pitch<PR>();
     const size_t stage_bytes = (size_t)WM * 32 * NT * 4;
@@ -1241,6 +1365,22 @@
     hipLaunchKernelGGL(kern, grid, dim3(WM * WN * 64), lds, st, a);
 }
 
+template <int PR>
+void launch_poly_b(const ConvArgs& a, hipStream_t st) {
+    ConvArgs v = a;
+    v.Cout = 4 * a.Cout; v.Hout = a.Hin; v.Wout = a.Win;
+    v.upsample = 0; v.zins = 0; v.stride = 1; v.pad = 1; v.nsplit = 1;
+    launch_one_b2<PR, 4, 2, 4, 2, 2, CM_NONE, 0>(v, st);
+}
+
+template <int PR>
+void launch_poly_in_b(const ConvArgs& a, hipStream_t st) {
+    ConvArgs v = a;
+    v.Cin = 4 * a.Cin; v.Hin = a.Hin / 2; v.Win = a.Win / 2;
+    v.upsample = 0; v.zins = 0; v.stride = 1; v.pad = 1; v.nsplit = 1;
+    launch_one_b2<PR, 4, 2, 4, 2, 2, CM_NONE, 1>(v, st);
+}
+
 template <int PR, int TAPS, int MODE>
 void launch_tile_b(const ConvArgs& a, hipStream_t st) {
     switch (a.tile) {
diff --git a/loco-edit_amd/csrc/conv_plan.hip b/loco-edit_amd/csrc/conv_plan.hip
--- a/loco-edit_amd/csrc/conv_plan.hip
+++ b/loco-edit_amd/csrc/conv_plan.hip
@@ -52,8 +52,26 @@
 static int tile_for(const ConvArgs& a, int prec, int tile_override) {
     return prec ? bf16_tile_of(a, tile_override) : pick_tile(a.Cout, a.Hout * a.Wout);
 }
-static int conv_bf16_tile_pixels(const ConvArgs& a) { return a.gemm ? 256 : kNT[a.tile]; }
+static int conv_bf16_tile_pixels(const ConvArgs& a) { return a.poly == 1 ? 512 : a.gemm ? 256 : kNT[a.tile]; }
 int conv_bf16_tile_couts(const ConvArgs& a) { return a.gemm ? 64 * a.gemm_tm : kMT[a.tile]; }
+
+static bool conv_poly_ok(const ConvEnv& e, const ConvArgs& a, int taps) {
+    static const bool on = env_int("LOCO_POLYPHASE", 1) != 0;
+    if (!on || e.prec < 1 || taps != 9 || a.mode != CM_NONE || !(a.upsample || a.zins) || a.stride != 1) return false;
+    if (!(e.prec == 2 ? a.wph : a.wpb) || !a.in_padded || a.res || a.Cin2 > 0 || a.cot_d) return false;
+    if (a.upsample ? a.pad != 1 : (a.pad != 1 && a.pad != 2)) return false;
+    if ((a.Cin % BKC) != 0 || (a.Cout % 128) != 0 || a.B < 2) return false;
+    if (a.Hin * a.Win < 4096 || a.Win < 32 || (a.Win % 32) != 0 || (a.Hin % 8) != 0) return false;
+    return a.Hout == 2 * a.Hin && a.Wout == 2 * a.Win;
+}
+static bool conv_poly_in_ok(const ConvEnv& e, const ConvArgs& a, int taps) {
+    static const bool on = env_int("LOCO_POLYPHASE", 1) != 0;
+    if (!on || e.prec < 1 || taps != 9 || a.mode != CM_NONE || !a.pool2 || a.upsample || a.zins || a.stride != 1 || a.pad != 1) return false;
+    if (!(e.prec == 2 ? a.wqh : a.wqb) || a.res || a.bias2 || a.Cin2 > 0 || a.cot_d) return false;
+    if ((a.Cin % BKC) != 0 || (a.Cout % 128) != 0 || a.B < 2 || ((a.Hin | a.Win) & 1)) return false;
+    if (a.Hout * a.Wout < 4096 || a.Wout < 32 || (a.Wout % 32) != 0 || (a.Hout % 8) != 0) return false;
+    return a.Hin == 2 * a.Hout && a.Win == 2 * a.Wout;
+}
 
 static int conv_bf16_pick_nsplit(int Cin, int Cout, int Hout, int Wout, int B, int chip_share, int taps, int lanes) {
     const int HW = Hout * Wout;
@@ -84,7 +102,7 @@
 
 static bool conv_pair_ok(const ConvArgs& a) {
     static const bool on = env_int("LOCO_CONV_PAIR", 1) != 0;
-    if (!on || a.Hout * a.Wout < 16384 || a.taps != 9 || a.Cin2 > 0 || a.nsplit != 1 || a.stride != 1 || a.upsample || a.zins ||
+    if (!on || a.poly || a.Hout * a.Wout < 16384 || a.taps != 9 || a.Cin2 > 0 || a.nsplit != 1 || a.stride != 1 || a.upsample || a.zins ||
         a.pad != 1 || !a.in_padded || (a.Cin % (2 * BKC)) != 0 || (a.Cout % 128) != 0 || (a.Wout % 32) != 0 || (a.Hout % 8) != 0)
         return false;
     if (!(a.mode == CM_NONE || a.mode == CM_GN_SILU || a.mode == CM_TAN_SILU || a.mode == CM_COT_SILU)) return false;
@@ -175,12 +193,12 @@
     const size_t need = (size_t)x.B * x.Cout * ntile * 2;
     const int epi = q->norm ? SR_EPI : SR_KEEP;
     const bool kept = q->keep && s0 == 0 && x.B == B && need <= q->keep_floats;
-    if (q->kind == ST_FWD && conv_lowp_can_fuse_stats(x) && (kept || (q->norm && need <= e.stpart_floats))) {
+    if (q->kind == ST_FWD && x.poly != 1 && conv_lowp_can_fuse_stats(x) && (kept || (q->norm && need <= e.stpart_floats))) {
         x.st_part = kept ? q->keep : e.stpart; x.st_kind = ST_FWD;
         if (kept) *keep_ntile = ntile;
         return epi;
     }
-    const bool cot_cache = q->kind == ST_COT && q->norm && q->sx;
+    const bool cot_cache = q->kind == ST_COT && q->norm && q->sx && x.poly != 1;
     if ((q->kind == ST_TAN || cot_cache) && e.fuse_lin && !x.cot_d && conv_lowp_can_fuse_stats(x)) {
         const size_t lane_off = (size_t)e.lane_s0 * (q->keep_floats / e.max_batch);
         const bool keptl = q->kind == ST_TAN && q->keep && s0 == 0 && x.B == B && lane_off + need <= q->keep_floats;
@@ -210,6 +228,14 @@
     ConvArgs a = a0;
     a.taps = taps;
     a.gemm = 0;
+    a.poly = 0;
+    if (a.pool2) {
+        if (conv_poly_in_ok(e, a, taps)) a.poly = 2;
+        else {
+            p.pool_after = true; p.pool_out = a.out; p.pool_out_bs = a.out_bs; p.pool_acc = a.accumulate;
+            a.out = a.pool_tmp; a.out_bs = a.pool_tmp_bs; a.Hout = a.Hin; a.Wout = a.Win; a.accumulate = 0; a.pool2 = 0;
+        }
+    }
     if (sc) {
         ConvArgs t = a;
         t.nsplit = e.prec >= 1 ? conv_bf16_pick_nsplit(a.Cin, a.Cout, a.Hout, a.Wout, a.B, e.chip_share, 9, e.lanes) : 2;
@@ -240,10 +266,13 @@
     if (a.nsplit < 1) a.nsplit = 1;
     a.partial = e.partial;
     a.partial_floats = e.partial_floats;
+    if (!a.poly && conv_poly_ok(e, a, taps)) a.poly = 1;
+    if (a.poly == 1) { a.nsplit = 1; a.wb = e.prec == 2 ? a.wph : a.wpb; }
+    if (a.poly == 2) { a.nsplit = 1; a.wb = e.prec == 2 ? a.wqh : a.wqb; }
     conv_plan_family(a, e.prec);
     a.tile = tile_for(a, e.prec, -1);
     int split = 1;
-    const int tail = e.prec >= 1 && a.nsplit == 1 && a.B >= 2 && !a.gemm ? tail_split(a, e.partial_floats, &split) : 0;
+    const int tail = e.prec >= 1 && a.nsplit == 1 && a.B >= 2 && !a.gemm && !a.poly ? tail_split(a, e.partial_floats, &split) : 0;
     const bool want = q && q->kind != ST_NONE && e.prec >= 1 && e.fuse_stats;
     if (!tail) {
         p.l[0] = plan_launch(e, q, want, a, 0, a.B, &p.keep_ntile);
@@ -262,6 +291,45 @@
     return p;
 }
 
+void polyphase_fold(int kind, int nin, int nout, const float* w, long so, long si, long st, float* out) {
+    static const int sel[3][2][2][3] = {
+        {{{1, 0, 0}, {0, 1, 1}}, {{1, 1, 0}, {0, 0, 1}}},
+        {{{1, 0, 0}, {0, 0, 1}}, {{0, 1, 0}, {0, 0, 0}}},
+        {{{0, 0, 0}, {0, 1, 0}}, {{1, 0, 0}, {0, 0, 1}}}};
+    const long V = 4L * nout;
+    for (int i = 0; i < nin; ++i)
+        for (int pa = 0; pa < 2; ++pa)
+            for (int pb = 0; pb < 2; ++pb)
+                for (int ty = 0; ty < 2; ++ty)
+                    for (int tx = 0; tx < 2; ++tx)
+                        for (int o = 0; o < nout; ++o) {
+                            double acc = 0.0;
+                            for (int ky = 0; ky < 3; ++ky)
+                                for (int kx = 0; kx < 3; ++kx)
+                                    if (sel[kind][pa][ty][ky] && sel[kind][pb][tx][kx]) acc += (double)w[o * so + i * si + (3 * ky + kx) * st];
+                            out[((long)i * 4 + 2 * ty + tx) * V + polyphase_vcout(nout, pa, pb, o)] = (float)acc;
+                        }
+}
+
+void polyphase_fold_in(int nin, int nout, const float* w, long so, long si, long st, float* out, int noutP) {
+    for (int p = 0; p < 2; ++p)
+        for (int q = 0; q < 2; ++q)
+            for (int i = 0; i < nin; ++i)
+                for (int ty = 0; ty < 2; ++ty)
+                    for (int tx = 0; tx < 2; ++tx) {
+                        const int m = 2 * ty + 1 - p, n = 2 * tx + 1 - q;
+                        for (int o = 0; o < nout; ++o) {
+                            double acc = 0.0;
+                            for (int a = 0; a < 2; ++a)
+                                for (int b = 0; b < 2; ++b) {
+                                    const int ky = m - a, kx = n - b;
+                                    if (ky >= 0 && ky < 3 && kx >= 0 && kx < 3) acc += (double)w[o * so + i * si + (3 * ky + kx) * st];
+                                }
+                            out[((((long)(2 * p + q) * nin + i) * 4) + 2 * ty + tx) * noutP + o] = (float)acc;
+                        }
+                    }
+}
+
 const char* conv_variant_name(const ConvArgs& a, int taps, int prec) {
     static const char* tiles[6] = {"2,2,2,2", "4,1,1,2", "1,4,1,1", "2,2,1,1", "2,2,2,4", "2,4,2,2"};
     static char names[3][2][6][6][56];
@@ -269,6 +337,11 @@
     const int mode = (a.mode < 0 || a.mode > 5) ? 2 : a.mode;
     const char* other = nullptr;
     int k = 0, v = mode;
+    if (prec && taps == 9 && a.poly) {
+        static const char* pn[2][3] = {{"", "conv_mfma_bf16x3<4,2,4,2,2,0>", "conv_mfma_f16<4,2,4,2,2,0>"},
+                                       {"", "conv_mfma_bf16x3<4,2,4,2,2,0>+pool", "conv_mfma_f16<4,2,4,2,2,0>+pool"}};
+        return pn[a.poly == 2][prec];
+    }
     if (prec && taps == 9 && a.Cin2 > 0) other = prec == 1 ? "conv_kcat_bf16x3<2,4,2,2,%d>" : "conv_kcat_f16<2,4,2,2,%d>";
     else if (prec == 1 && taps == 1 && a.gemm) { k = 1; other = "conv_gemm_bf16x3<%d>"; v = a.gemm_tm; }
     else if (prec == 1 && taps == 9 && a.pair) { k = 2; other = "conv_pair_bf16x3<%d>"; }
diff --git a/loco-edit_amd/csrc/engine.hip b/loco-edit_amd/csrc/engine.hip
--- a/loco-edit_amd/csrc/engine.hip
+++ b/loco-edit_amd/csrc/engine.hip
@@ -44,6 +44,11 @@
     float* wbd = nullptr;
     float* whf = nullptr;
     float* whd = nullptr;
+    float* wpb = nullptr;
+    float* wph = nullptr;
+    bool poly_dgrad = false;
+    float* wqb = nullptr;
+    float* wqh = nullptr;
     float* bias = nullptr;
     int cin = 0, cout = 0, taps = 0;
 };
@@ -268,7 +273,7 @@
 }
 
 int make_conv(loco_ctx* c, const std::vector<const HostParam*>& ws, const std::vector<const HostParam*>& bs,
-              ConvP* out, int row_limit = -1) {
+              ConvP* out, int row_limit = -1, int poly_kind = -1, bool poly_dgrad = false) {
     int cin = (int)ws[0]->shape[1], k = ws[0]->shape.size() > 2 ? (int)ws[0]->shape[2] : 1;
     int taps = ws[0]->shape.size() == 4 ? k * k : k;
     int cout = 0;
@@ -304,10 +309,27 @@
     std::vector<float> hf = build_records_f16(cin, cout, taps, fwd);
     std::vector<float> hd = build_records_f16(cout, cin, taps, dgr);
     if (upload(c, &out->whf, hf) || upload(c, &out->whd, hd)) return -1;
-    return 0;
-}
-int make_conv1(loco_ctx* c, const std::string& name, ConvP* out, int row_limit = -1) {
-    return make_conv(c, {&c->params[name + ".weight"]}, {&c->params[name + ".bias"]}, out, row_limit);
+    const int pin = poly_dgrad ? cout : cin, pout = poly_dgrad ? cin : cout;
+    if (poly_kind >= 0 && taps == 9 && pin % 16 == 0 && pout % 128 == 0) {
+        const int poutP = poly_dgrad ? cinP : coutP;
+        std::vector<float> pf((size_t)pin * 16 * pout);
+        polyphase_fold(poly_kind, pin, pout, (poly_dgrad ? wd : wf).data(), 1, 9L * poutP, poutP, pf.data());
+        auto fold = [&](int o, int i, int t) { return pf[((size_t)i * 4 + t) * 4 * pout + o]; };
+        std::vector<float> rp = build_records(pin, 4 * pout, 4, fold), hp = build_records_f16(pin, 4 * pout, 4, fold);
+        if (upload(c, &out->wpb, rp) || upload(c, &out->wph, hp)) return -1;
+        out->poly_dgrad = poly_dgrad;
+    }
+    if (poly_kind == POLY_UP && !poly_dgrad && taps == 9 && cout % 16 == 0 && cin % 128 == 0) {
+        std::vector<float> qf((size_t)4 * cout * 4 * cinP, 0.f);
+        polyphase_fold_in(cout, cin, wd.data(), 1, 9L * cinP, cinP, qf.data(), cinP);
+        auto fold = [&](int o, int i, int t) { return qf[((size_t)i * 4 + t) * cinP + o]; };
+        std::vector<float> rq = build_records(4 * cout, cin, 4, fold), hq = build_records_f16(4 * cout, cin, 4, fold);
+        if (upload(c, &out->wqb, rq) || upload(c, &out->wqh, hq)) return -1;
+    }
+    return 0;
+}
+int make_conv1(loco_ctx* c, const std::string& name, ConvP* out, int row_limit = -1, int poly_kind = -1, bool poly_dgrad = false) {
+    return make_conv(c, {&c->params[name + ".weight"]}, {&c->params[name + ".bias"]}, out, row_limit, poly_kind, poly_dgrad);
 }
 int make_conv1_scaled(loco_ctx* c, const std::string& name, ConvP* out, float s) {
     if (s == 1.f) return make_conv1(c, name, out);
@@ -414,7 +436,11 @@
                 }
                 break;
             }
-            case OP_DOWN: case OP_UP: if (make_conv1(c, op.pn_conv, &ow.conv)) return -1; break;
+            case OP_DOWN: case OP_UP: {
+                const int pk = op.kind == OP_UP ? POLY_UP : (op.sym_down ? POLY_ZINS_PAD1 : POLY_ZINS_PAD2);
+                if (make_conv1(c, op.pn_conv, &ow.conv, -1, pk, op.kind == OP_DOWN)) return -1;
+                break;
+            }
             case OP_XFMR: {
                 const int C = c->tens[op.in].C, NH = op.heads, CH = C / NH;
                 const std::string b = op.name + ".transformer_blocks.0";
@@ -610,6 +636,7 @@
         const ConvArgs& x = l.args;
         double flops = 2.0 * (x.Cin * taps + x.Cin2) * x.Cout * (double)x.Hout * x.Wout * x.B;
         if (x.zins) flops *= 0.25;
+        if (x.poly == 2) flops *= 4.0;
         timed(c->prof_on ? conv_variant_name(x, taps, c->prec) : nullptr, flops, x, [&] {
             if (c->prec == 1) launch_conv_bf16x3(x, taps, st);
             else if (c->prec == 2) launch_conv_f16(x, taps, st);
@@ -640,6 +667,8 @@
         }
     }
     if (p.stats_all) stats_standalone(c, *rq, a.out, a.out_bs, a.B, HWo, 0, st);
+    if (p.pool_after)
+        launch_pool2x2_sum(a.pool_tmp, a.pool_tmp_bs, p.pool_out, p.pool_out_bs, p.pool_acc, a.B, a.Cout, a.Hout, a.Wout, st);
     return p.cot;
 }
 
@@ -647,6 +676,11 @@
     a.w = dgrad ? p.wd : p.wf;
     a.wb = dgrad ? (const void*)p.wbd : (const void*)p.wbf;
     a.wh = dgrad ? (const void*)p.whd : (const void*)p.whf;
+    const bool folded = p.wpb && p.poly_dgrad == dgrad;
+    a.wpb = folded ? p.wpb : nullptr;
+    a.wph = folded ? p.wph : nullptr;
+    a.wqb = dgrad ? p.wqb : nullptr;
+    a.wqh = dgrad ? p.wqh : nullptr;
 }
 
 NormP* consumer_norm(loco_ctx* c, int tid) {
@@ -1332,9 +1366,9 @@
                 ConvArgs a; conv_defaults(a);
                 a.in = TG(op.out); a.in_bs = PS; a.Cin = to.C; a.Hin = to.H; a.Win = to.W;
                 setw(a, op.conv, true);
-                a.out = TG(op.up); a.out_bs = PS; a.Cout = ti.C; a.Hout = to.H; a.Wout = to.W; a.B = B;
+                a.pool2 = 1; a.pool_tmp = TG(op.up); a.pool_tmp_bs = PS;
+                a.out = TG(op.in); a.out_bs = PS; a.Cout = ti.C; a.Hout = ti.H; a.Wout = ti.W; a.B = B;
                 run_conv(c, a, 9, st);
-                launch_pool2x2_sum(TG(op.up), PS, TG(op.in), PS, 0, B, ti.C, ti.H, ti.W, st);
                 break;
             }
             case OP_DOWN: {
@@ -2218,8 +2252,10 @@
     if (finalize_params(c)) return -3;
     hipStream_t st = (hipStream_t)stream;
     const long HW = (long)H * W;
-    const long in_e = (long)cin * HW, out_e = (long)cout * HW;
-    if ((in_e + out_e) * B > (long)c->cfg.max_batch * c->prog->per_sample || 2 * in_e > (long)c->prog->per_sample ||
+    const int geom = (taps == 9 && getenv("LOCO_BENCH_GEOM")) ? atoi(getenv("LOCO_BENCH_GEOM")) : 0;
+    if (geom < 0 || geom > 4 || (geom && ((H | W) & 1))) { c->err = "bench_conv: bad LOCO_BENCH_GEOM"; return -2; }
+    const long in_e = (long)cin * ((geom && geom != 4) ? HW / 4 : HW), out_e = (long)cout * HW;
+    if ((in_e + out_e + (geom == 4 ? out_e / 4 : 0)) * B > (long)c->cfg.max_batch * c->prog->per_sample || 2 * in_e > (long)c->prog->per_sample ||
         in_e > c->prog->sx_total) { c->err = "bench_conv: shape exceeds the arenas"; return -2; }
     float* in = c->arenaT;
     float* out = c->arenaT + in_e * B;
@@ -2230,12 +2266,12 @@
     launch_fill_random(reinterpret_cast<float*>(c->sxcache), 2 * in_e, 3u, zs, st);
     launch_fill_random(c->statsP, c->prog->stats_per_sample, 4u, 1.0f, st);
     launch_fill_random(c->statsT, c->prog->stats_per_sample * B, 5u, 0.01f, st);
-    size_t wfl = (size_t)((cin + 15) / 16) * 16 * taps * ((cout + 31) & ~31);
+    size_t wfl = (size_t)((cin + 15) / 16) * 16 * (geom ? 16 : taps) * ((cout + 31) & ~31);
     if (wfl * 2 > c->partial_floats) { c->err = "bench_conv: weights exceed workspace"; return -2; }
     float* wf = c->partial + c->partial_floats - wfl * 2;
     launch_fill_random(wf, (long)wfl * 2, 6u, 0.05f * zw, st);
     if (c->prec == 1) {
-        const long nrec = (long)((cin + 15) / 16) * taps * ((cout + 31) & ~31);
+        const long nrec = (long)((cin + 15) / 16) * (geom ? 16 : taps) * ((cout + 31) & ~31);
         hipLaunchKernelGGL(diag_fill_records, dim3((unsigned)((nrec + 255) / 256)), dim3(256), 0, st,
                            reinterpret_cast<unsigned char*>(wf), nrec, (cout + 31) & ~31, 7u, 0.05f * zw);
     }
@@ -2245,6 +2281,15 @@
     a.w = wf; a.wb = wf; a.wh = wf;
     a.out = out; a.out_bs = out_e; a.Cout = cout; a.Hout = H; a.Wout = W; a.B = B;
     a.mode = mode; a.pad = taps == 9 ? 1 : 0; a.in_padded = 1; a.taps = taps;
+    if (geom == 4) {
+        a.pool2 = 1; a.pool_tmp = out; a.pool_tmp_bs = out_e;
+        a.out = out + out_e * B; a.out_bs = out_e / 4; a.Hout = H / 2; a.Wout = W / 2;
+        a.wqb = wf; a.wqh = wf;
+    } else if (geom) {
+        a.Hin = H / 2; a.Win = W / 2;
+        if (geom == 1) a.upsample = 1; else { a.zins = 1; a.pad = geom == 2 ? 2 : 1; }
+        a.wpb = wf; a.wph = wf;
+    }
     a.sc = c->statsP; a.sh = c->statsP + cin; a.scsh_bs = 0; a.mr = c->statsP + 2 * cin; a.mr_bs = 0;
     a.gamma_ = c->statsP; a.tst = c->statsT; a.tst_bs = c->prog->stats_per_sample; a.cpg = cin / c->cfg.gn_groups;
     a.tc = c->statsT + 64; a.tc_bs = c->prog->stats_per_sample;
@@ -2262,6 +2307,13 @@
     conv_plan_family(a, c->prec);
     if (const char* e = getenv("LOCO_DUAL_WHATIF")) a.no_deep = atoi(e);
     conv_plan_tile_pair(a, c->prec, tile);
+    if (geom) {
+        ConvEnv e;
+        e.prec = c->prec; e.partial = a.partial; e.partial_floats = a.partial_floats; e.max_batch = c->cfg.max_batch;
+        a.poly = plan_conv(e, a, taps, nullptr, nullptr).l[0].args.poly;
+        if (a.poly) a.nsplit = 1;
+        if (geom == 4 && a.poly != 2) { c->err = "bench_conv: the shape does not take the pooled polyphase launch"; return -2; }
+    }
     auto run = [&]() {
         if (c->prec == 1) launch_conv_bf16x3(a, taps, st);
         else if (c->prec == 2) launch_conv_f16(a, taps, st);
@@ -2312,11 +2364,14 @@
     if (d->cot_d && (!d->cot_prim || !d->cot_sc || !d->cot_sh || !d->cot_mr || !d->cot_tc || d->cot_cpg < 1 || d->Cout % d->cot_cpg)) {
         c->err = "debug_conv: the norm-cotangent term needs cot_prim, cot_sc, cot_sh, cot_mr, cot_tc and cot_cpg"; return -2;
     }
-    const int Hout = d->stride == 2 ? d->Hin / 2 : (d->upsample || d->zins) ? 2 * d->Hin : d->Hin;
-    const int Wout = d->stride == 2 ? d->Win / 2 : (d->upsample || d->zins) ? 2 * d->Win : d->Win;
+    if (d->pool2 && (taps != 9 || d->stride != 1 || d->upsample || d->zins || d->mode != CM_NONE || d->Cin2 > 0 || d->res || d->cot_d ||
+                     ((d->Hin | d->Win) & 1))) { c->err = "debug_conv: pool2 goes with a raw 3x3 stride-1 conv of an even map"; return -2; }
+    const int Hout = (d->stride == 2 || d->pool2) ? d->Hin / 2 : (d->upsample || d->zins) ? 2 * d->Hin : d->Hin;
+    const int Wout = (d->stride == 2 || d->pool2) ? d->Win / 2 : (d->upsample || d->zins) ? 2 * d->Win : d->Win;
     {
         auto pow2 = [](int v) { return v >= 8 && (v & (v - 1)) == 0; };
-        if (!((pow2(Hout) && pow2(Wout)) || (Wout % 32 == 0 && Hout % 8 == 0 && ((long)Hout * Wout) % 256 == 0))) {
+        auto walks = [&](int h, int w) { return (pow2(h) && pow2(w)) || (w % 32 == 0 && h % 8 == 0 && ((long)h * w) % 256 == 0); };
+        if (!walks(Hout, Wout) || (d->pool2 && !walks(d->Hin, d->Win))) {
             c->err = "debug_conv: output map outside the tile geometry of the conv kernels"; return -2;
         }
     }
@@ -2330,7 +2385,12 @@
         need_sx > c->prog->sx_total) { c->err = "debug_conv: shape exceeds the arenas"; return -2; }
     const int G = lin ? d->Cin / d->cpg : 0;
     const long tbs = up64(2L * G) + up64(2L * d->Cin);
-    const long small_n = (lin ? (long)B * tbs : 0) + (d->cot_d ? (long)B * up64(2L * d->Cout) : 0) + 64;
+    const bool st_req = d->st_prim != nullptr;
+    if (st_req && (!d->st_mr || !d->st_out || d->st_cpg < 1 || d->Cout % d->st_cpg || d->cot_d || d->Cin2 > 0)) {
+        c->err = "debug_conv: the statistics request needs st_prim, st_mr, st_out and st_cpg (no second operator, no cot_d)"; return -2;
+    }
+    const long keep_n = st_req ? up64((long)B * d->Cout * ((long)Hout * Wout / 64 + 1) * 2) : 0;
+    const long small_n = (lin ? (long)B * tbs : 0) + (d->cot_d ? (long)B * up64(2L * d->Cout) : 0) + 64 + keep_n + (st_req ? up64(2L * d->Cout) : 0);
     const size_t owned0 = c->owned.size();
     const size_t bytes0 = c->bytes;
     auto release = [&]() {
@@ -2349,7 +2409,10 @@
     HostParam w2 = host_param(d->Cin2 > 0 ? d->w2 : nullptr, {d->Cout, d->Cin2 > 0 ? d->Cin2 : 1, 1, 1}), wb2 = host_param(nullptr, {d->Cout});
     ConvP cp, cp2;
     float *bias_d = nullptr, *bias2nd_d = nullptr, *small = nullptr;
-    int rc = make_conv(c, {&w}, {&wb0}, &cp);
+    const int poly_kind = taps != 9 ? -1 : (d->upsample || d->pool2) ? POLY_UP : d->zins ? ((d->pad >= 0 ? d->pad : 2) == 1 ? POLY_ZINS_PAD1 : POLY_ZINS_PAD2) : -1;
+    int rc = make_conv(c, {&w}, {&wb0}, &cp, -1, poly_kind, d->transposed != 0 && !d->pool2);
+    float* pool_tmp = nullptr;
+    if (!rc && d->pool2) rc = dalloc(c, &pool_tmp, (size_t)B * d->Cout * d->Hin * d->Win);
     if (!rc && d->Cin2 > 0) rc = make_conv(c, {&w2}, {&wb2}, &cp2);
     if (!rc && d->bias) rc = upload(c, &bias_d, std::vector<float>(d->bias, d->bias + d->Cout));
     if (!rc && d->Cin2 > 0 && d->bias2nd) rc = upload(c, &bias2nd_d, std::vector<float>(d->bias2nd, d->bias2nd + d->Cout));
@@ -2369,6 +2432,7 @@
     a.res = d->res; a.res_bs = out_e; a.res_scale = d->res_scale;
     a.mode = d->mode; a.stride = d->stride; a.upsample = d->upsample; a.zins = d->zins; a.accumulate = d->accumulate;
     a.pad = d->pad >= 0 ? d->pad : taps == 1 ? 0 : d->zins ? 2 : d->stride == 2 ? 0 : 1;
+    if (d->pool2) { a.pool2 = 1; a.pool_tmp = pool_tmp; a.pool_tmp_bs = (long)d->Cout * d->Hin * d->Win; }
     a.sc = d->sc; a.sh = d->sh; a.scsh_bs = 0; a.cpg = d->cpg;
     if (lin) {
         if (he == hipSuccess) he = copy(c->arenaP, d->prim, in_e);
@@ -2408,9 +2472,26 @@
     const int act0 = c->cfg.act;
     if (d->mode == CM_GN_GELU) c->cfg.act = ACT_GELU;
     c->plan_log = &text;
-    const bool rode = run_conv(c, a, taps, st, nullptr, d->Cin2 > 0 ? &n2 : nullptr);
+    StatReq srq;
+    int kept_ntile = 0;
+    float* const keep_buf = small + (small_n - keep_n - (st_req ? up64(2L * d->Cout) : 0));
+    if (st_req) {
+        srq.kind = ST_TAN; srq.prim = d->st_prim; srq.keep = keep_buf; srq.keep_floats = (size_t)keep_n; srq.keep_ntile = &kept_ntile;
+    }
+    const bool rode = run_conv(c, a, taps, st, st_req ? &srq : nullptr, d->Cin2 > 0 ? &n2 : nullptr);
     c->plan_log = nullptr;
     c->cfg.act = act0;
+    if (st_req) {
+        const int G2 = d->Cout / d->st_cpg;
+        float* const zero = keep_buf + keep_n;
+        (void)hipMemsetAsync(zero, 0, (size_t)up64(2L * d->Cout) * sizeof(float), st);
+        (void)hipMemsetAsync(d->st_out, 0xff, (size_t)B * G2 * 2 * sizeof(float), st);
+        if (kept_ntile > 0)
+            launch_gn_lin_fused_finalize(ST_TAN, keep_buf, d->Cout, kept_ntile, nullptr, 0, B, d->Cout, Hout * Wout, G2, d->st_mr, d->st_out,
+                                         nullptr, 2L * G2, st);
+        launch_gn_tstats(d->out, out_e, d->st_prim, 0, B, d->Cout, Hout * Wout, G2, zero, zero + d->Cout, d->st_mr, 0, 0, 0,
+                         d->st_out + (long)B * G2 * 2, nullptr, 2L * G2, c->red, st, ACT_SILU);
+    }
     he = hipGetLastError();
     release();
     if (he == hipSuccess) he = hipGetLastError();
diff --git a/loco-edit_amd/csrc/kernels.h b/loco-edit_amd/csrc/kernels.h
--- a/loco-edit_amd/csrc/kernels.h
+++ b/loco-edit_amd/csrc/kernels.h
@@ -75,7 +75,16 @@
     int gemm, gemm_tm;
     size_t partial_floats;
     int tile, pair;
-};
+    const void* wpb; const void* wph;
+    int poly;
+    int pool2; float* pool_tmp; long pool_tmp_bs;
+    const void* wqb; const void* wqh;
+};
+
+enum PolyKind : int { POLY_UP = 0, POLY_ZINS_PAD2 = 1, POLY_ZINS_PAD1 = 2 };
+inline int polyphase_vcout(int C, int a, int b, int co) { return ((a * (C / 64) + co / 64) * 2 + b) * 64 + (co % 64); }
+void polyphase_fold(int kind, int nin, int nout, const float* w, long so, long si, long st, float* out);
+void polyphase_fold_in(int nin, int nout, const float* w, long so, long si, long st, float* out, int noutP);
 
 void launch_conv(const ConvArgs& a, int taps, hipStream_t st);
 void launch_conv_bf16x3(const ConvArgs& a, int taps, hipStream_t st);
@@ -121,6 +130,7 @@
     ConvLaunch l[2];
     bool stats_all = false;
     int keep_ntile = 0;
+    bool pool_after = false; float* pool_out = nullptr; long pool_out_bs = 0; int pool_acc = 0;
     bool cot = false;
 };
 
diff --git a/loco-edit_amd/hip.py b/loco-edit_amd/hip.py
--- a/loco-edit_amd/hip.py
+++ b/loco-edit_amd/hip.py
@@ -55,12 +55,12 @@
 
 class LocoConvDesc(C.Structure):
     _PTRS = ("weight", "bias", "in", "bias2", "res", "prim", "sc", "sh", "mr", "gamma", "tst", "tc", "in2", "w2", "bias2nd",
-             "cot_d", "cot_prim", "cot_sc", "cot_sh", "cot_mr", "cot_tc", "out")
+             "cot_d", "cot_prim", "cot_sc", "cot_sh", "cot_mr", "cot_tc", "out", "st_prim", "st_mr", "st_out")
     _HOST = ("weight", "bias", "w2", "bias2nd")
     _fields_ = ([("struct_size", C.c_int32)] +
                 [(k, C.c_int32) for k in ("Cin", "Cout", "Hin", "Win", "B", "taps", "stride", "upsample", "zins", "mode", "cpg",
                                           "transposed", "accumulate", "in_arena", "pad", "Cin2", "cot_cpg")] +
-                [("res_scale", C.c_float), ("reserved", C.c_int32)] + [(k, C.c_void_p) for k in _PTRS])
+                [("res_scale", C.c_float), ("st_cpg", C.c_int32)] + [(k, C.c_void_p) for k in _PTRS] + [("pool2", C.c_int32)])
 
 
 class LocoTextCfg(C.Structure):
@@ -681,7 +681,7 @@
         d.out = out.data_ptr()
         for k, v in desc.items():
             if k not in LocoConvDesc._PTRS:
-                if not hasattr(d, k) or k in ("struct_size", "reserved"):
+                if not hasattr(d, k) or k == "struct_size":
                     raise TypeError(f"debug_conv: no descriptor field {k!r}")
                 setattr(d, k, v)
             elif v is not None:
```

New measurement: 20.36 edit-directions/s (median of 6 runs). +2.5%, better.
